# LazyLatte/vortex-raytracing

Measured on AMD Instinct MI355X. Metric: Mrays/s (primary+shadow) at 1920x1080, 1M-tri BVH, higher is better.
Workload: dtype f32; 1 GPU; configs[2]: Sponza-class 1048576 tris, 1920x1080, primary + 1 shadow ray per hit; frames_in_flight=2, frames_per_launch_group=5, parallelism=1 GPU: whole frames, 5 per set of launches (vxrt_render_batch), 2 sets in flight, world_size=1, bvh_nodes=726809, bvh_depth=13

## Files before the change

include/vortex_hip.h:

```cpp
#ifndef VORTEX_HIP_H
#define VORTEX_HIP_H

#include <stddef.h>
#include <stdint.h>

#ifdef __cplusplus
extern "C" {
#endif

typedef void* vx_device_h;
typedef void* vx_buffer_h;

typedef struct {
  int (*dev_open)(vx_device_h* hdevice);
  int (*dev_close)(vx_device_h hdevice);
  int (*dev_caps)(vx_device_h hdevice, uint32_t caps_id, uint64_t* value);
  int (*mem_alloc)(vx_device_h hdevice, uint64_t size, int flags, vx_buffer_h* hbuffer);
  int (*mem_reserve)(vx_device_h hdevice, uint64_t address, uint64_t size, int flags, vx_buffer_h* hbuffer);
  int (*mem_free)(vx_buffer_h hbuffer);
  int (*mem_access)(vx_buffer_h hbuffer, uint64_t offset, uint64_t size, int flags);
  int (*mem_address)(vx_buffer_h hbuffer, uint64_t* address);
  int (*mem_info)(vx_device_h hdevice, uint64_t* mem_free, uint64_t* mem_used);
  int (*copy_to_dev)(vx_buffer_h hbuffer, const void* host_ptr, uint64_t dst_offset, uint64_t size);
  int (*copy_from_dev)(void* host_ptr, vx_buffer_h hbuffer, uint64_t src_offset, uint64_t size);
// ... 84 lines not shown
  const void* triEx;
  const void* mat;
  const void* tex;
  uint32_t n_tlas_nodes;
  uint32_t n_blas;
  uint32_t n_bvh_nodes;
  uint32_t n_tris;
  uint32_t n_mats;
  uint32_t reserved;
  uint64_t tex_bytes;
} vxrt_scene_t;

typedef struct {
  float dist, bx, by, bz;
  uint32_t blasIdx, triIdx;
} vxrt_hit_t;

typedef struct {
  float ambient[3], light_color[3], light_pos[3], background[3];
  uint32_t max_depth;
} vxrt_shade_params_t;

#define VXRT_MODE_CLOSEST 0
#define VXRT_MODE_ANY 1

typedef struct vxrt_accel vxrt_accel_t;
int vxrt_accel_build(const vxrt_scene_t* scene, void* stream, vxrt_accel_t** out);
int vxrt_accel_destroy(vxrt_accel_t* accel);
uint64_t vxrt_accel_bytes(const vxrt_accel_t* accel);
int vxrt_accel_info(const vxrt_accel_t* accel, uint32_t which, uint64_t* value);

#define VXRT_REFIT_INSTANCES 1u
#define VXRT_REFIT_GEOMETRY 2u
int vxrt_accel_refit(vxrt_accel_t* accel, uint32_t what, void* stream);
int vxrt_accel_set_transforms(vxrt_accel_t* accel, uint32_t first, uint32_t count, const float* transforms, void* stream);

int vxrt_accel_frames_in_flight(vxrt_accel_t* accel, uint32_t n);

int vxrt_render(vxrt_accel_t* accel, uint32_t width, uint32_t height, uint32_t y0, uint32_t y1,
                const vxrt_shade_params_t* params, int shadow, uint32_t* dst,
                vxrt_hit_t* hits , float* colors ,
                unsigned long long* rays_traced, void* stream);

int vxrt_render_interleaved(vxrt_accel_t* accel, uint32_t width, uint32_t height, uint32_t phase, uint32_t stride,
                            const vxrt_shade_params_t* params, int shadow, uint32_t* dst, vxrt_hit_t* hits,
                            float* colors, unsigned long long* rays_traced, void* stream);

typedef struct vxrt_bvh_info {
  uint32_t n_nodes, n_leaves, max_leaf, max_depth;
  float bounds[6];
} vxrt_bvh_info_t;
int vxrt_bvh_build(void* tri, void* triEx, uint32_t n_tris, uint32_t tri_offset, uint32_t leaf_max,
                   void* nodes, uint32_t node_capacity, vxrt_bvh_info_t* info, void* stream);
int vxrt_tlas_build(const float* instance_boxes, uint32_t n_instances, void* nodes, uint32_t node_capacity,
                    vxrt_bvh_info_t* info, void* stream);
void vxrt_bvh_release_scratch(void);

#define VXRT_MAX_BATCH 32
int vxrt_render_interleaved_batch(vxrt_accel_t* accel, uint32_t width, uint32_t height, uint32_t phase, uint32_t stride, uint32_t n_frames,
                                  const vxrt_shade_params_t* params, int shadow, uint32_t* dst, uint64_t dst_frame_stride,
                                  unsigned long long* rays_traced, void* stream);

int vxrt_render_interleaved_batch_wave_log(vxrt_accel_t* accel, uint32_t width, uint32_t height, uint32_t phase, uint32_t stride, uint32_t n_frames,
                                           const vxrt_shade_params_t* params, int shadow, uint32_t* dst, uint64_t dst_frame_stride,
                                           unsigned long long* counters, unsigned long long* wave_log, void* stream);

int vxrt_wire_pack(const uint32_t* frames, uint64_t frame_stride, uint32_t width, uint32_t tile_rows_per_rank, uint32_t world, uint32_t rank,
                   uint32_t n_frames, uint8_t* wire, void* stream);
int vxrt_wire_unpack(const uint8_t* wire_all, uint64_t wire_stride_bytes, uint32_t width, uint32_t tile_rows_per_rank, uint32_t world,
                     uint32_t n_frames, uint32_t* frames, uint64_t frame_stride, void* stream);

int vxrt_render_rows_batch(vxrt_accel_t* accel, uint32_t width, uint32_t height, uint32_t y0, uint32_t y1, uint32_t n_frames,
                           const vxrt_shade_params_t* params, int shadow, uint32_t* dst, uint64_t dst_frame_stride,
                           unsigned long long* rays_traced, void* stream);

int vxrt_render_batch(vxrt_accel_t* accel, uint32_t width, uint32_t height, uint32_t n_frames, const vxrt_shade_params_t* params, int shadow,
                      uint32_t* dst, uint64_t dst_frame_stride, unsigned long long* rays_traced, void* stream);

typedef struct vxrt_camera {
  float pos[3], forward[3], right[3], up[3], viewplane[2];
} vxrt_camera_t;

int vxrt_render_camera(vxrt_accel_t* accel, const vxrt_camera_t* cam, uint32_t width, uint32_t height, uint32_t y0, uint32_t y1,
                       const vxrt_shade_params_t* params, int shadow, uint32_t* dst, vxrt_hit_t* hits , float* colors ,
                       unsigned long long* rays_traced, void* stream);

int vxrt_render_batch_camera(vxrt_accel_t* accel, uint32_t width, uint32_t height, uint32_t n_frames, const vxrt_camera_t* cams,
                             const vxrt_shade_params_t* params, int shadow, uint32_t* dst, uint64_t dst_frame_stride,
                             unsigned long long* rays_traced, void* stream);

int vxrt_render_stats(vxrt_accel_t* accel, uint32_t width, uint32_t height, uint32_t y0, uint32_t y1,
                      const vxrt_shade_params_t* params, int shadow, uint32_t* dst,
                      unsigned long long* counters, void* stream);

int vxrt_render_stats_timed(vxrt_accel_t* accel, uint32_t width, uint32_t height, uint32_t y0, uint32_t y1,
                            const vxrt_shade_params_t* params, int shadow, uint32_t* dst,
                            unsigned long long* counters, void* stream);

int vxrt_trace_stats(vxrt_accel_t* accel, const float* rays, uint64_t n, const float* tmax,
                     vxrt_hit_t* hits, int mode, unsigned long long* counters, void* stream);

typedef struct vxrt_ao_params {
  uint32_t spp;
  float radius;
  uint32_t seed;
  uint32_t reserved;
} vxrt_ao_params_t;
int vxrt_render_ao(vxrt_accel_t* accel, uint32_t width, uint32_t height, uint32_t y0, uint32_t y1,
                   const vxrt_shade_params_t* params, const vxrt_ao_params_t* ao, uint32_t* dst, float* colors,
                   uint32_t* unoccluded, unsigned long long* rays_traced, void* stream);

int vxrt_render_diffuse_bounce(vxrt_accel_t* accel, uint32_t width, uint32_t height, uint32_t y0, uint32_t y1,
                               const vxrt_shade_params_t* params, uint32_t seed, uint32_t* dst, float* colors,
                               unsigned long long* rays_traced, void* stream);

typedef struct vxrc_scene {
  const void* tlas; const void* blas; const void* bvh; const void* tri; const void* triEx; const void* triIdx; const void* tex;
  uint32_t n_tlas_nodes, n_blas, n_bvh_nodes, n_tris, n_tri_idx, tlas_root;
  uint64_t tex_bytes;
} vxrc_scene_t;
typedef struct vxrc_params {
  float camera_pos[3], camera_forward[3], camera_right[3], camera_up[3], viewplane[2];
  uint32_t samples_per_pixel, max_depth;
  float light_pos[3], light_color[3], ambient_color[3], background_color[3];
} vxrc_params_t;
typedef struct vxrc_accel vxrc_accel_t;
int vxrc_accel_build(const vxrc_scene_t* scene, void* stream, vxrc_accel_t** out);
int vxrc_accel_destroy(vxrc_accel_t* accel);
int vxrc_accel_info(const vxrc_accel_t* accel, uint32_t which, uint64_t* value);
int vxrc_render_accel(vxrc_accel_t* accel, uint32_t width, uint32_t height, uint32_t y0, uint32_t y1,
                      const vxrc_params_t* params, uint32_t* dst, float* colors, void* stream);

int vxrc_render(const vxrc_scene_t* scene, uint32_t width, uint32_t height, uint32_t y0, uint32_t y1,
                const vxrc_params_t* params, uint32_t* dst, float* colors, void* stream);

int vxrt_render_wave_log(vxrt_accel_t* accel, uint32_t width, uint32_t height, uint32_t y0, uint32_t y1,
                         const vxrt_shade_params_t* params, int shadow, uint32_t* dst,
                         unsigned long long* counters, unsigned long long* wave_log, void* stream);

int vxrt_trace(vxrt_accel_t* accel, const float* rays, uint64_t n, const float* tmax,
               vxrt_hit_t* hits, int mode, void* stream);

int vxrt_shade_rays(vxrt_accel_t* accel, const float* rays, const vxrt_hit_t* hits, uint64_t n, const vxrt_shade_params_t* params,
                    float* colors, uint32_t* rgb8, void* stream);

int vxrt_camera_rays(uint32_t width, uint32_t height, uint32_t y0, uint32_t y1, float* rays, void* stream);

int vxrt_pinhole_rays(const vxrt_camera_t* cam, uint32_t width, uint32_t height, uint32_t y0, uint32_t y1, float* rays, void* stream);

int vxrt_trace_reference_quirks(const void* image, uint64_t image_size, uint32_t tlas_off, uint32_t blas_off, uint32_t bvh_off, uint32_t tri_off,
                                const float* rays, uint64_t n, const float* tmax, vxrt_hit_t* hits, int mode, void* stream);

int vxrt_debug_read_control(vxrt_accel_t* accel, uint32_t ctx, uint32_t* out, uint32_t n_dwords, void* stream);
int vxrt_debug_end_log(vxrt_accel_t* accel, unsigned long long* log);
int vxrt_debug_trace_wave_log(vxrt_accel_t* accel, unsigned long long* log);
int vxrt_debug_read_lpt(vxrt_accel_t* accel, uint32_t ctx, uint32_t batch, uint32_t* cost, uint32_t cost_cap, uint32_t* order, uint32_t order_cap,
                        void* stream);

int vxrt_status(void* stream, uint32_t* status);
int vx_hip_buffer_device_ptr(vx_buffer_h hbuffer, void** dev_ptr);

int vx_hip_device_stat(vx_device_h hdevice, uint32_t which, uint64_t* value);

const char* vxrt_version(void);

#ifdef __cplusplus
}
#endif
#endif
```

vortex-raytracing_amd/csrc/rt_accel.hip:

```cpp
#include <algorithm>
#include <cmath>
#include <cstdio>
#include <cstdlib>
#include <cstring>
#include <utility>
#include "rt_internal.h"
#include "bvh_quant.h"

__global__ void accel_nodes_kernel(const uint32_t* __restrict__ ref, uint32_t n_nodes, uint4* __restrict__ out, int is_tlas,
                                   const uint32_t* __restrict__ bases, const uint32_t* __restrict__ ends, uint32_t nb,
                                   uint32_t n_tris, uint32_t n_blas, uint32_t bias, uint32_t* status) {
  const uint32_t i = blockIdx.x * blockDim.x + threadIdx.x;
  if (i >= n_nodes) return;
  const uint32_t* w = ref + (size_t)i * RT_NODE_DWORDS;
  const uint32_t imask = w[3] >> 24, leftFirst = w[4], leafData = w[5];
  uint32_t base = 0, end = n_nodes;
  if (!is_tlas) {
    bool in = false;
    for (uint32_t j = 0; j < nb; ++j) if (i >= bases[j] && i < ends[j]) { base = bases[j]; end = ends[j]; in = true; }
    if (!in) return;
  }
  if (imask != (is_tlas ? 1u : 0u)) return;
  const bool leaf = is_tlas ? (leafData != 0xffffffffu) : (leafData != 0u);
  if (leaf) return;
// ... 224 lines not shown
  bool fin = true;
  if (fbox_bvh) {
    for (int a = 0; a < 3; ++a) { olo[a] = fbox_bvh[(size_t)off * 6 + a]; ohi[a] = fbox_bvh[(size_t)off * 6 + 3 + a]; }
  } else if (r[5] != 0u) {
    fin = refit_tri_box(tri, r[4], r[5], olo, ohi);
  } else {
    const uint8_t* b = (const uint8_t*)r;
    olo[0] = olo[1] = olo[2] = __builtin_inff(); ohi[0] = ohi[1] = ohi[2] = -__builtin_inff();
    for (int k = 0; k < 4; ++k) {
      const uint8_t* c = b + 24 + 7 * k;
      if (c[0] == 0) continue;
      for (int a = 0; a < 3; ++a) {
        const int e = (int)(int8_t)b[12 + a];
        const float o = __uint_as_float(r[a]);
        olo[a] = fminf(olo[a], o + ldexpf((float)c[1 + a], e));
        ohi[a] = fmaxf(ohi[a], o + ldexpf((float)c[4 + a], e));
      }
    }
  }
  const float* m = (const float*)(rec + 17);
  for (int k = 0; k < 12; ++k) fin = fin && isfinite(m[k]);
  float lo[3] = {__builtin_inff(), __builtin_inff(), __builtin_inff()}, hi[3] = {-__builtin_inff(), -__builtin_inff(), -__builtin_inff()};
  for (int c = 0; c < 8; ++c) {
    const float x = (c & 1) ? ohi[0] : olo[0], y = (c & 2) ? ohi[1] : olo[1], z = (c & 4) ? ohi[2] : olo[2];
    for (int a = 0; a < 3; ++a) {
      const float p = refit_row(m + 4 * a, x, y, z);
      fin = fin && isfinite(p);
      lo[a] = fminf(lo[a], p); hi[a] = fmaxf(hi[a], p);
    }
  }
  if (!fin) atomicOr(res + 1, REFIT_ERR_NONFINITE);
  const int e[3] = {bb_pick_exp(hi[0] - lo[0]), bb_pick_exp(hi[1] - lo[1]), bb_pick_exp(hi[2] - lo[2])};
  refit_write_origin(w, lo, hi, e);
  refit_store_box(fbox, i, lo, hi);
}

__global__ __launch_bounds__(256) void refit_level_kernel(uint32_t* __restrict__ nodes, const uint2* __restrict__ items, uint32_t n,
                                                          float* __restrict__ fbox, uint32_t* __restrict__ res) {
  const uint32_t j = blockIdx.x * blockDim.x + threadIdx.x;
  if (j >= n) return;
  const uint2 it = items[j];
  uint32_t* w = nodes + (size_t)it.x * RT_NODE_DWORDS;
  uint32_t cw[7];
#pragma unroll
  for (int v = 0; v < 7; ++v) cw[v] = w[6 + v];
  uint8_t* cb = (uint8_t*)cw;
  uint32_t present = 0;
  float cmin[3][4], cmax[3][4];
  float lo[3] = {__builtin_inff(), __builtin_inff(), __builtin_inff()}, hi[3] = {-__builtin_inff(), -__builtin_inff(), -__builtin_inff()};
#pragma unroll
  for (int k = 0; k < 4; ++k) {
    const bool on = cb[7 * k] != 0;
    present |= on ? (1u << k) : 0u;
    const float* f = fbox + (size_t)(it.y + (on ? (uint32_t)k : 0u)) * 6;
#pragma unroll
    for (int a = 0; a < 3; ++a) {
      cmin[a][k] = on ? f[a] : 0.0f; cmax[a][k] = on ? f[3 + a] : 0.0f;
      if (on) { lo[a] = fminf(lo[a], cmin[a][k]); hi[a] = fmaxf(hi[a], cmax[a][k]); }
    }
  }
  if (!present) return;
  int e[3] = {bb_pick_exp(hi[0] - lo[0]), bb_pick_exp(hi[1] - lo[1]), bb_pick_exp(hi[2] - lo[2])};
  bool ok = true;
#pragma unroll
  for (int a = 0; a < 3; ++a) {
    uint32_t ql[4] = {0, 0, 0, 0}, qh[4] = {0, 0, 0, 0};
    ok = bb_quant_children(lo[a], e[a], cmin[a], cmax[a], present, ql, qh) && ok;
#pragma unroll
    for (int k = 0; k < 4; ++k)
      if ((present >> k) & 1u) { cb[7 * k + 1 + a] = (uint8_t)ql[k]; cb[7 * k + 4 + a] = (uint8_t)qh[k]; }
  }
  if (!ok) atomicOr(res + 1, REFIT_ERR_QUANT);
  refit_write_origin(w, lo, hi, e);
#pragma unroll
  for (int v = 0; v < 7; ++v) w[6 + v] = cw[v];
  refit_store_box(fbox, it.x, lo, hi);
}

__global__ void refit_finish_kernel(const uint32_t* __restrict__ blas, uint32_t troot, const uint32_t* __restrict__ top_roots, uint32_t* __restrict__ res) {
  if (threadIdx.x != 0 || blockIdx.x != 0) return;
  uint32_t id = 0u;
  if (is_inst_desc(troot)) {
    const float* m = (const float*)(blas + (size_t)(troot & PAYLOAD_MASK) * (RT_BLAS_STRIDE / 4) + 1);
    id = 1u;
    for (int i = 0; i < 12; ++i) id = (id && m[i] == ((i % 5 == 0) ? 1.0f : 0.0f)) ? 1u : 0u;
  }
  res[2] = id;
  if (top_roots) { res[3] = top_roots[0]; res[4] = top_roots[1]; }
}

__global__ __launch_bounds__(256) void refit_xform_kernel(const float* __restrict__ in, uint32_t n, float* __restrict__ out, uint32_t* __restrict__ res) {
#pragma clang fp contract(off)
  const uint32_t r = blockIdx.x * blockDim.x + threadIdx.x;
  if (r >= n) return;
  float c[16];
  bool fin = true;
  for (int k = 0; k < 16; ++k) { c[k] = in[(size_t)r * 16 + k]; fin = fin && isfinite(c[k]); }
  const float inv[16] = {
      c[5] * c[10] * c[15] - c[5] * c[11] * c[14] - c[9] * c[6] * c[15] + c[9] * c[7] * c[14] + c[13] * c[6] * c[11] - c[13] * c[7] * c[10],
      -c[1] * c[10] * c[15] + c[1] * c[11] * c[14] + c[9] * c[2] * c[15] - c[9] * c[3] * c[14] - c[13] * c[2] * c[11] + c[13] * c[3] * c[10],
      c[1] * c[6] * c[15] - c[1] * c[7] * c[14] - c[5] * c[2] * c[15] + c[5] * c[3] * c[14] + c[13] * c[2] * c[7] - c[13] * c[3] * c[6],
      -c[1] * c[6] * c[11] + c[1] * c[7] * c[10] + c[5] * c[2] * c[11] - c[5] * c[3] * c[10] - c[9] * c[2] * c[7] + c[9] * c[3] * c[6],
      -c[4] * c[10] * c[15] + c[4] * c[11] * c[14] + c[8] * c[6] * c[15] - c[8] * c[7] * c[14] - c[12] * c[6] * c[11] + c[12] * c[7] * c[10],
      c[0] * c[10] * c[15] - c[0] * c[11] * c[14] - c[8] * c[2] * c[15] + c[8] * c[3] * c[14] + c[12] * c[2] * c[11] - c[12] * c[3] * c[10],
      -c[0] * c[6] * c[15] + c[0] * c[7] * c[14] + c[4] * c[2] * c[15] - c[4] * c[3] * c[14] - c[12] * c[2] * c[7] + c[12] * c[3] * c[6],
      c[0] * c[6] * c[11] - c[0] * c[7] * c[10] - c[4] * c[2] * c[11] + c[4] * c[3] * c[10] + c[8] * c[2] * c[7] - c[8] * c[3] * c[6],
      c[4] * c[9] * c[15] - c[4] * c[11] * c[13] - c[8] * c[5] * c[15] + c[8] * c[7] * c[13] + c[12] * c[5] * c[11] - c[12] * c[7] * c[9],
      -c[0] * c[9] * c[15] + c[0] * c[11] * c[13] + c[8] * c[1] * c[15] - c[8] * c[3] * c[13] - c[12] * c[1] * c[11] + c[12] * c[3] * c[9],
      c[0] * c[5] * c[15] - c[0] * c[7] * c[13] - c[4] * c[1] * c[15] + c[4] * c[3] * c[13] + c[12] * c[1] * c[7] - c[12] * c[3] * c[5],
      -c[0] * c[5] * c[11] + c[0] * c[7] * c[9] + c[4] * c[1] * c[11] - c[4] * c[3] * c[9] - c[8] * c[1] * c[7] + c[8] * c[3] * c[5],
      -c[4] * c[9] * c[14] + c[4] * c[10] * c[13] + c[8] * c[5] * c[14] - c[8] * c[6] * c[13] - c[12] * c[5] * c[10] + c[12] * c[6] * c[9],
      c[0] * c[9] * c[14] - c[0] * c[10] * c[13] - c[8] * c[1] * c[14] + c[8] * c[2] * c[13] + c[12] * c[1] * c[10] - c[12] * c[2] * c[9],
      -c[0] * c[5] * c[14] + c[0] * c[6] * c[13] + c[4] * c[1] * c[14] - c[4] * c[2] * c[13] - c[12] * c[1] * c[6] + c[12] * c[2] * c[5],
      c[0] * c[5] * c[10] - c[0] * c[6] * c[9] - c[4] * c[1] * c[10] + c[4] * c[2] * c[9] + c[8] * c[1] * c[6] - c[8] * c[2] * c[5]};
  const float det = c[0] * inv[0] + c[1] * inv[4] + c[2] * inv[8] + c[3] * inv[12];
  uint32_t err = fin ? 0u : REFIT_ERR_NONFINITE;
  if (det == 0.0f) err |= REFIT_ERR_SINGULAR;
  const float invdet = 1.0f / det;
  float* o = out + (size_t)r * 32;
  for (int k = 0; k < 16; ++k) {
    const float v = inv[k] * invdet;
    if (!isfinite(v)) err |= REFIT_ERR_SINGULAR;
    o[k] = v;
    o[16 + k] = c[k];
  }
  if (err) atomicOr(res + 6, err);
}

__global__ __launch_bounds__(256) void refit_xform_commit_kernel(const float* __restrict__ xf, uint32_t first, uint32_t n, uint32_t* __restrict__ blas,
                                                                 const uint32_t* __restrict__ res) {
  const uint32_t t = blockIdx.x * blockDim.x + threadIdx.x;
  if (t >= n * 32u || res[6] != 0u) return;
  const uint32_t r = t / 32u, k = t % 32u;
  blas[(size_t)(first + r) * (RT_BLAS_STRIDE / 4) + 1 + k] = __float_as_uint(xf[(size_t)r * 32 + k]);
}

struct RefitPlan {
  uint32_t* blas_leaves = nullptr; uint32_t n_blas_leaves = 0;
  uint2* blas_items = nullptr; std::vector<uint32_t> blas_lv;
  uint32_t* tlas_leaves = nullptr; uint32_t n_tlas_leaves = 0;
  uint2* tlas_items = nullptr; std::vector<uint32_t> tlas_lv;
  float* fbox_bvh = nullptr; float* fbox_tlas = nullptr;
  uint32_t* ranges = nullptr; uint32_t nb = 0;
  uint32_t* res = nullptr;
  float* xf = nullptr; uint32_t xf_cap = 0;
};
static void refit_plan_free(RefitPlan* p) {
  if (!p) return;
  (void)hipFree(p->blas_leaves); (void)hipFree(p->blas_items); (void)hipFree(p->tlas_leaves); (void)hipFree(p->tlas_items);
  (void)hipFree(p->fbox_bvh); (void)hipFree(p->fbox_tlas); (void)hipFree(p->ranges); (void)hipFree(p->res); (void)hipFree(p->xf);
  delete p;
}

static void accel_free(vxrt_accel* a) {
  if (!a) return;
  (void)hipDeviceSynchronize();
  (void)hipFree(a->nodes_c); (void)hipFree(a->tri_w); (void)hipFree(a->blas_root);
  (void)hipFree(a->top_img); (void)hipFree(a->top_roots);
  refit_plan_free(a->refit);
  (void)hipFree(a->uvtab); (void)hipFree(a->apriori);
  for (uint32_t k = 0; k <= VXRT_MAX_BATCH; ++k) (void)hipFree(a->batch_order[k]);
  for (FrameCtx& c : a->ctx) {
    (void)hipFree(c.hitbuf); (void)hipFree(c.defer); (void)hipFree(c.ctl); (void)hipFree(c.bcount);
    for (FrameCtx::Lpt& l : c.lpt) { (void)hipFree(l.cost); (void)hipFree(l.order); }
    (void)hipFree(c.ao_geo); (void)hipFree(c.ao_nrm); (void)hipFree(c.ao_col); (void)hipFree(c.ao_cnt); (void)hipFree(c.ao_rays); (void)hipFree(c.ao_tmax); (void)hipFree(c.ao_hits); (void)hipFree(c.ao_list); (void)hipFree(c.ao_hdr);
    (void)hipFree(c.bin_hist); (void)hipFree(c.bin_keys); (void)hipFree(c.bin_order);
    for (FrameCtx::Level& l : c.lv) {
      (void)hipFree(l.rays); (void)hipFree(l.hits); (void)hipFree(l.parent); (void)hipFree(l.term); (void)hipFree(l.col);
      (void)hipFree(l.srays); (void)hipFree(l.stmax); (void)hipFree(l.shits);
    }
    (void)hipFree(c.pbatch); (void)hipFree(c.pool_spill); (void)hipFree(c.cam);
    if (c.side) (void)hipStreamDestroy(c.side);
    if (c.ev_in) (void)hipEventDestroy(c.ev_in);
    if (c.ev_side) (void)hipEventDestroy(c.ev_side);
    if (c.ev_done) (void)hipEventDestroy(c.ev_done);
  }
  delete a;
}

extern "C" {

int vxrt_accel_build(const vxrt_scene_t* s, void* stream, vxrt_accel_t** out) {
  if (!s || !out || !s->tlas || !s->blas || !s->bvh || !s->tri) return -1;
  if (s->n_tlas_nodes == 0 || s->n_blas == 0 || s->n_bvh_nodes == 0 || s->n_tris == 0) return -1;
  if ((uint64_t)s->n_tlas_nodes + s->n_bvh_nodes > PAYLOAD_MASK || s->n_tris >= 0x7fffffffu) return -1;
  hipStream_t st = (hipStream_t)stream;
  std::vector<uint32_t> recs((size_t)s->n_blas * (RT_BLAS_STRIDE / 4));
  if (hipStreamSynchronize(st) != hipSuccess) return -1;
  if (hipMemcpy(recs.data(), s->blas, recs.size() * 4, hipMemcpyDeviceToHost) != hipSuccess) return -1;
  std::vector<uint32_t> bases;
  float max_refl = 0.0f;
  for (uint32_t j = 0; j < s->n_blas; ++j) {
    const uint32_t off = recs[(size_t)j * (RT_BLAS_STRIDE / 4)];
    if (off >= s->n_bvh_nodes) return -1;
    bases.push_back(off);
    float refl;
    memcpy(&refl, &recs[(size_t)j * (RT_BLAS_STRIDE / 4) + 38], sizeof(float));
    if (refl > max_refl) max_refl = refl;
  }
  std::sort(bases.begin(), bases.end());
  bases.erase(std::unique(bases.begin(), bases.end()), bases.end());
  std::vector<uint32_t> ends(bases.size());
  for (size_t j = 0; j < bases.size(); ++j) ends[j] = j + 1 < bases.size() ? bases[j + 1] : s->n_bvh_nodes;

  auto a = new (std::nothrow) vxrt_accel();
  if (!a) return -1;
  a->ref = *s;
  a->max_reflectivity = max_refl;
  (void)hipGetDevice(&a->device);
  uint32_t* d_ranges = nullptr;
  uint32_t* d_status = nullptr;
  uint32_t* d_troot = nullptr;
  constexpr uint32_t TOP_CAP = RT_TOP_NODES;
  const bool stage_top = TOP_CAP > 0 && (uint64_t)s->n_tlas_nodes + s->n_bvh_nodes < DESC_TOP_FLAG;
  bool ok = hipMalloc(&a->nodes_c, ((size_t)s->n_tlas_nodes + s->n_bvh_nodes) * CNODE_VEC4 * 16) == hipSuccess &&
            (!stage_top || (hipMalloc(&a->top_img, (size_t)TOP_CAP * CNODE_VEC4 * 16) == hipSuccess &&
                            hipMalloc((void**)&a->top_roots, ((size_t)s->n_blas + 2) * sizeof(uint32_t)) == hipSuccess)) &&
            hipMalloc(&a->tri_w, (size_t)s->n_tris * WTRI_FLOATS * 4) == hipSuccess &&
            hipMalloc(&a->blas_root, (size_t)s->n_blas * sizeof(uint32_t)) == hipSuccess &&
            hipMalloc((void**)&d_ranges, bases.size() * 8) == hipSuccess &&
            hipMalloc((void**)&d_status, 8) == hipSuccess && hipMalloc((void**)&d_troot, 4) == hipSuccess;
  uint32_t hstatus = 0, troot = DESC_DONE, hstatus2[2] = {0, 0};
  if (ok) {
    ok = hipMemcpy(d_ranges, bases.data(), bases.size() * 4, hipMemcpyHostToDevice) == hipSuccess &&
         hipMemcpy(d_ranges + bases.size(), ends.data(), ends.size() * 4, hipMemcpyHostToDevice) == hipSuccess &&
         hipMemset(d_status, 0, 8) == hipSuccess;
  }
  if (ok) {
    const uint32_t nb = (uint32_t)bases.size();
    hipLaunchKernelGGL(accel_nodes_kernel, dim3((s->n_tlas_nodes + 255) / 256), dim3(256), 0, st, (const uint32_t*)s->tlas, s->n_tlas_nodes,
                       (uint4*)a->nodes_c, 1, (const uint32_t*)nullptr, (const uint32_t*)nullptr, 0u, s->n_tris, s->n_blas, 0u, d_status);
    hipLaunchKernelGGL(accel_nodes_kernel, dim3((s->n_bvh_nodes + 255) / 256), dim3(256), 0, st, (const uint32_t*)s->bvh, s->n_bvh_nodes,
                       (uint4*)a->nodes_c + (size_t)s->n_tlas_nodes * CNODE_VEC4, 0, d_ranges, d_ranges + nb, nb, s->n_tris, s->n_blas, s->n_tlas_nodes, d_status + 1);
    hipLaunchKernelGGL(accel_tris_kernel, dim3((s->n_tris + 255) / 256), dim3(256), 0, st, (const float*)s->tri, s->n_tris, (float4*)a->tri_w);
    hipLaunchKernelGGL(accel_roots_kernel, dim3((s->n_blas + 1 + 255) / 256), dim3(256), 0, st, (const uint32_t*)s->tlas, (const uint32_t*)s->bvh,
                       (const uint32_t*)s->blas, s->n_tlas_nodes, s->n_bvh_nodes, s->n_blas, s->n_tris, d_troot, (uint32_t*)a->blas_root, d_status);
    if (s->triEx && s->mat && s->n_mats) {
      const uint32_t nchk = std::max(s->n_tris, s->n_mats);
      hipLaunchKernelGGL(accel_check_shading_kernel, dim3((nchk + 255) / 256), dim3(256), 0, st, (const rt_triex_t*)s->triEx, s->n_tris,
                         (const rt_material_t*)s->mat, s->n_mats, (uint64_t)s->tex_bytes, s->tex ? 1 : 0, d_status);
    }
    ok = hipGetLastError() == hipSuccess && hipStreamSynchronize(st) == hipSuccess &&
         hipMemcpy(hstatus2, d_status, 8, hipMemcpyDeviceToHost) == hipSuccess &&
         hipMemcpy(&troot, d_troot, 4, hipMemcpyDeviceToHost) == hipSuccess;
    hstatus = hstatus2[0] | hstatus2[1];
    a->blas_status = hstatus2[1] & STATUS_FMA_DECODE_DIFFERS;
  }
  uint32_t n_top = 0, troot_top = troot;
  if (ok && stage_top && (hstatus & (STATUS_BAD_SCENE | STATUS_FMA_DECODE_DIFFERS)) == 0) {
    ok = hipMemsetAsync(a->top_img, 0, (size_t)TOP_CAP * CNODE_VEC4 * 16, st) == hipSuccess;
    hipLaunchKernelGGL(accel_top_kernel, dim3(1), dim3(64), 0, st, (const uint4*)a->nodes_c, troot, (const uint32_t*)a->blas_root, s->n_blas, TOP_CAP,
                       (uint4*)a->top_img, a->top_roots, a->top_roots + 1, a->top_roots + 2);
    uint32_t hdr[2] = {0, DESC_DONE};
    ok = ok && hipGetLastError() == hipSuccess && hipStreamSynchronize(st) == hipSuccess &&
         hipMemcpy(hdr, a->top_roots, sizeof hdr, hipMemcpyDeviceToHost) == hipSuccess;
    n_top = hdr[0]; troot_top = hdr[1];
  }
  uint32_t levels = 0;
  if (ok && (hstatus & STATUS_BAD_SCENE) == 0) {
    const uint32_t nc = s->n_tlas_nodes + s->n_bvh_nodes;
    uint32_t* d_depth = nullptr;
    ok = hipMalloc((void**)&d_depth, ((size_t)nc + 1) * 4) == hipSuccess && hipMemsetAsync(d_depth, 0, ((size_t)nc + 1) * 4, st) == hipSuccess;
    if (ok) {
      for (uint32_t level = 1; level <= RT_SHALLOW_LEVELS + 1u; ++level)
        hipLaunchKernelGGL(accel_depth_kernel, dim3(level == 1u ? 1u : (nc + 255) / 256), dim3(256), 0, st, (const uint4*)a->nodes_c, nc, troot,
                           (const uint32_t*)a->blas_root, level, d_depth, d_depth + nc);
      ok = hipGetLastError() == hipSuccess && hipStreamSynchronize(st) == hipSuccess &&
           hipMemcpy(&levels, d_depth + nc, 4, hipMemcpyDeviceToHost) == hipSuccess;
    }
    (void)hipFree(d_depth);
  }
  (void)hipFree(d_ranges); (void)hipFree(d_status); (void)hipFree(d_troot);
  if (!ok || (hstatus & STATUS_BAD_SCENE) != 0) { accel_free(a); return -1; }
  static const int shallow_env = [] { const char* e = getenv("VXRT_SHALLOW"); return e ? atoi(e) : -1; }();
  a->levels = levels;
  a->shallow = levels <= RT_SHALLOW_LEVELS && shallow_env != 0;
  a->dev.nodes_c = (const uint4*)a->nodes_c; a->dev.ref_tlas = (const uint32_t*)s->tlas; a->dev.n_tlas = s->n_tlas_nodes; a->dev.tri_w = (const float4*)a->tri_w;
  a->dev.blas_root = (const uint32_t*)a->blas_root; a->dev.tlas_root = troot;
  a->dev.ident_root = 0u;
  if (troot >= 0xC0000000u && troot < DESC_IDLE) {
    float m[12];
    static const bool ident_off = [] { const char* e = getenv("VXRT_IDENT_ROOT"); return e && e[0] == '0'; }();
    if (!ident_off && hipMemcpy(m, (const uint32_t*)s->blas + (size_t)(troot & PAYLOAD_MASK) * (RT_BLAS_STRIDE / 4) + 1, sizeof m, hipMemcpyDeviceToHost) == hipSuccess) {
      bool id = true;
      for (int i = 0; i < 12; ++i) id = id && m[i] == ((i % 5 == 0) ? 1.0f : 0.0f);
      a->dev.ident_root = id ? 1u : 0u;
    }
  }
  a->dev.exact_decode = (hstatus & STATUS_FMA_DECODE_DIFFERS) ? 1u : 0u;
  a->dev.ref_bvh = (const uint32_t*)s->bvh;
  a->dev.blas = (const uint32_t*)s->blas; a->dev.triEx = (const rt_triex_t*)s->triEx;
  a->dev.mat = (const rt_material_t*)s->mat; a->dev.tex = (const uint8_t*)s->tex;
  a->dev.top_img = (const uint4*)a->top_img; a->dev.n_top = n_top; a->dev.tlas_root_top = troot_top;
  a->dev.blas_root_top = n_top ? a->top_roots + 2 : (const uint32_t*)a->blas_root;
  if (getenv("VXRT_DEBUG")) fprintf(stderr, "[vxrt] accel: %u top-of-tree nodes staged for LDS (cap %u)\n", n_top, TOP_CAP);
  *out = a;
  return 0;
}

int vxrt_accel_destroy(vxrt_accel_t* a) {
  if (!a) return 0;
  accel_free(a);
  return 0;
}

uint64_t vxrt_accel_bytes(const vxrt_accel_t* a) {
  if (!a) return 0;
  return (uint64_t)a->ref.n_tlas_nodes * CNODE_VEC4 * 16 + (uint64_t)a->ref.n_bvh_nodes * CNODE_VEC4 * 16 +
         (uint64_t)a->ref.n_tris * WTRI_FLOATS * 4 + (uint64_t)a->ref.n_blas * 4;
}

int vxrt_accel_info(const vxrt_accel_t* a, uint32_t which, uint64_t* value) {
  if (!a || !value) return -1;
  switch (which) {
  case 0: *value = a->levels; return 0;
  case 1: *value = a->shallow ? 1u : 0u; return 0;
  case 2: *value = a->dev.ident_root; return 0;
  case 3: *value = a->dev.exact_decode; return 0;
  }
  return -1;
}

int vxrt_accel_frames_in_flight(vxrt_accel_t* a, uint32_t n) {
  if (!a || n < 1 || n > MAX_FRAMES_IN_FLIGHT) return -1;
  if (hipDeviceSynchronize() != hipSuccess) return -1;
  a->n_ctx = n; a->next_ctx = 0;
  return 0;
}

static int refit_fail(const char* where) {
  const hipError_t e = hipGetLastError();
  if (getenv("VXRT_DEBUG")) fprintf(stderr, "[vxrt] refit failed: %s (%s)\n", where, hipGetErrorString(e));
  return -1;
}

static RefitPlan* refit_plan_build(vxrt_accel* a, hipStream_t st) {
  const vxrt_scene_t& s = a->ref;
  std::vector<uint32_t> tl((size_t)s.n_tlas_nodes * RT_NODE_DWORDS), bv((size_t)s.n_bvh_nodes * RT_NODE_DWORDS), recs((size_t)s.n_blas * (RT_BLAS_STRIDE / 4));
  if (hipStreamSynchronize(st) != hipSuccess ||
      hipMemcpy(tl.data(), s.tlas, tl.size() * 4, hipMemcpyDeviceToHost) != hipSuccess ||
      hipMemcpy(bv.data(), s.bvh, bv.size() * 4, hipMemcpyDeviceToHost) != hipSuccess ||
      hipMemcpy(recs.data(), s.blas, recs.size() * 4, hipMemcpyDeviceToHost) != hipSuccess) { refit_fail("plan: node copy"); return nullptr; }
  std::vector<uint32_t> bases;
  for (uint32_t j = 0; j < s.n_blas; ++j) bases.push_back(recs[(size_t)j * (RT_BLAS_STRIDE / 4)]);
  std::sort(bases.begin(), bases.end());
  bases.erase(std::unique(bases.begin(), bases.end()), bases.end());
  std::vector<uint32_t> ends(bases.size());
  for (size_t j = 0; j < bases.size(); ++j) ends[j] = j + 1 < bases.size() ? bases[j + 1] : s.n_bvh_nodes;
  auto walk = [](const std::vector<uint32_t>& w, uint32_t root, uint32_t base, uint32_t end, bool tlas, std::vector<uint32_t>& leaves,
                 std::vector<std::pair<uint32_t, uint2>>& items) -> bool {
    std::vector<std::pair<uint32_t, uint32_t>> q{{root, 0u}};
    for (size_t h = 0; h < q.size(); ++h) {
      const uint32_t i = q[h].first, L = q[h].second;
      const uint32_t* n = w.data() + (size_t)i * RT_NODE_DWORDS;
      if (tlas ? n[5] != 0xffffffffu : n[5] != 0u) { leaves.push_back(i); continue; }
      const uint64_t c0 = (uint64_t)base + n[4];
      items.push_back({L, make_uint2(i, (uint32_t)c0)});
      const uint8_t* b = (const uint8_t*)n;
      bool any = false;
      for (uint32_t k = 0; k < 4; ++k) {
        if (b[24 + 7 * k] == 0) continue;
        if (c0 + k >= end || c0 + k <= i) return false;
        q.push_back({(uint32_t)(c0 + k), L + 1u});
        any = true;
      }
      if (!any) return false;
    }
    return true;
  };
  std::vector<uint32_t> bl, tlv;
  std::vector<std::pair<uint32_t, uint2>> bi, ti;
  for (size_t j = 0; j < bases.size(); ++j)
    if (!walk(bv, bases[j], bases[j], ends[j], false, bl, bi)) { refit_fail("plan: BLAS walk"); return nullptr; }
  if (!walk(tl, 0u, 0u, s.n_tlas_nodes, true, tlv, ti)) { refit_fail("plan: TLAS walk"); return nullptr; }
  for (uint32_t i : tlv) if (tl[(size_t)i * RT_NODE_DWORDS + 5] >= s.n_blas) { refit_fail("plan: instance index"); return nullptr; }
  auto bucket = [](const std::vector<std::pair<uint32_t, uint2>>& it, std::vector<uint2>& out, std::vector<uint32_t>& lv) {
    uint32_t depth = 0;
    for (const auto& x : it) depth = std::max(depth, x.first + 1u);
    lv.assign(depth + 1u, 0u);
    for (const auto& x : it) ++lv[x.first + 1u];
    for (uint32_t L = 0; L < depth; ++L) lv[L + 1u] += lv[L];
    std::vector<uint32_t> pos(lv.begin(), lv.end() - 1);
    out.resize(it.size());
    for (const auto& x : it) out[pos[x.first]++] = x.second;
  };
  std::vector<uint32_t> ranges(bases);
  ranges.insert(ranges.end(), ends.begin(), ends.end());
  std::vector<uint2> bitems, titems;
  auto p = new (std::nothrow) RefitPlan();
  if (!p) return nullptr;
  bucket(bi, bitems, p->blas_lv);
  bucket(ti, titems, p->tlas_lv);
  p->n_blas_leaves = (uint32_t)bl.size(); p->n_tlas_leaves = (uint32_t)tlv.size(); p->nb = (uint32_t)bases.size();
  auto up = [](void** d, const void* h, size_t bytes) {
    return hipMalloc(d, std::max<size_t>(bytes, 16)) == hipSuccess && (bytes == 0 || hipMemcpy(*d, h, bytes, hipMemcpyHostToDevice) == hipSuccess);
  };
  const bool ok = up((void**)&p->blas_leaves, bl.data(), bl.size() * 4) && up((void**)&p->blas_items, bitems.data(), bitems.size() * 8) &&
                  up((void**)&p->tlas_leaves, tlv.data(), tlv.size() * 4) && up((void**)&p->tlas_items, titems.data(), titems.size() * 8) &&
                  up((void**)&p->ranges, ranges.data(), ranges.size() * 4) &&
                  hipMalloc((void**)&p->fbox_bvh, (size_t)s.n_bvh_nodes * 24) == hipSuccess &&
                  hipMalloc((void**)&p->fbox_tlas, (size_t)s.n_tlas_nodes * 24) == hipSuccess &&
                  hipMalloc((void**)&p->res, REFIT_RES_WORDS * 4) == hipSuccess;
  if (!ok) { refit_fail("plan: upload"); refit_plan_free(p); return nullptr; }
  return p;
}

static int refit_run(vxrt_accel* a, uint32_t what, hipStream_t st, const float* xf_in, uint32_t xf_first, uint32_t xf_count) {
  RefitPlan* p = a->refit;
  const vxrt_scene_t& s = a->ref;
  for (uint32_t k = 0; k < MAX_FRAMES_IN_FLIGHT; ++k) {
    FrameCtx& c = a->ctx[k];
    if (!c.busy || c.last_stream == st) continue;
    if (c.done_recorded) { if (hipStreamWaitEvent(st, c.ev_done, 0) != hipSuccess) return refit_fail("ordering"); }
    else if (hipDeviceSynchronize() != hipSuccess) return refit_fail("ordering");
  }
  const bool geom = (what & VXRT_REFIT_GEOMETRY) != 0u;
  auto grid = [](uint64_t n) { return dim3((uint32_t)((n + 255) / 256)); };
  bool ok = hipMemsetAsync(p->res, 0, REFIT_RES_WORDS * 4, st) == hipSuccess;
  if (ok && xf_count) {
    hipLaunchKernelGGL(refit_xform_kernel, grid(xf_count), dim3(256), 0, st, xf_in, xf_count, p->xf, p->res);
    hipLaunchKernelGGL(refit_xform_commit_kernel, grid((uint64_t)xf_count * 32u), dim3(256), 0, st, (const float*)p->xf, xf_first, xf_count,
                       (uint32_t*)s.blas, (const uint32_t*)p->res);
  }
  if (ok && geom) {
    if (p->n_blas_leaves)
      hipLaunchKernelGGL(refit_blas_leaf_kernel, grid(p->n_blas_leaves), dim3(256), 0, st, (uint32_t*)s.bvh, (const float*)s.tri, p->blas_leaves,
                         p->n_blas_leaves, p->fbox_bvh, p->res);
    for (size_t L = p->blas_lv.size() - 1; L-- > 0;) {
      const uint32_t n = p->blas_lv[L + 1] - p->blas_lv[L];
      if (n) hipLaunchKernelGGL(refit_level_kernel, grid(n), dim3(256), 0, st, (uint32_t*)s.bvh, p->blas_items + p->blas_lv[L], n, p->fbox_bvh, p->res);
    }
  }
  if (ok) {
    if (p->n_tlas_leaves)
      hipLaunchKernelGGL(refit_instance_kernel, grid(p->n_tlas_leaves), dim3(256), 0, st, (uint32_t*)s.tlas, p->tlas_leaves, p->n_tlas_leaves,
                         (const uint32_t*)s.blas, (const uint32_t*)s.bvh, (const float*)s.tri, geom ? (const float*)p->fbox_bvh : (const float*)nullptr,
                         p->fbox_tlas, p->res);
    for (size_t L = p->tlas_lv.size() - 1; L-- > 0;) {
      const uint32_t n = p->tlas_lv[L + 1] - p->tlas_lv[L];
      if (n) hipLaunchKernelGGL(refit_level_kernel, grid(n), dim3(256), 0, st, (uint32_t*)s.tlas, p->tlas_items + p->tlas_lv[L], n, p->fbox_tlas, p->res);
    }
    hipLaunchKernelGGL(accel_nodes_kernel, grid(s.n_tlas_nodes), dim3(256), 0, st, (const uint32_t*)s.tlas, s.n_tlas_nodes,
                       (uint4*)a->nodes_c, 1, (const uint32_t*)nullptr, (const uint32_t*)nullptr, 0u, s.n_tris, s.n_blas, 0u, p->res);
    if (geom) {
      hipLaunchKernelGGL(accel_nodes_kernel, grid(s.n_bvh_nodes), dim3(256), 0, st, (const uint32_t*)s.bvh, s.n_bvh_nodes,
                         (uint4*)a->nodes_c + (size_t)s.n_tlas_nodes * CNODE_VEC4, 0, p->ranges, p->ranges + p->nb, p->nb, s.n_tris, s.n_blas, s.n_tlas_nodes,
                         p->res + 5);
      hipLaunchKernelGGL(accel_tris_kernel, grid(s.n_tris), dim3(256), 0, st, (const float*)s.tri, s.n_tris, (float4*)a->tri_w);
    }
    if (a->top_img) {
      ok = hipMemsetAsync(a->top_img, 0, (size_t)RT_TOP_NODES * CNODE_VEC4 * 16, st) == hipSuccess;
      hipLaunchKernelGGL(accel_top_kernel, dim3(1), dim3(64), 0, st, (const uint4*)a->nodes_c, a->dev.tlas_root, (const uint32_t*)a->blas_root, s.n_blas,
                         (uint32_t)RT_TOP_NODES, (uint4*)a->top_img, a->top_roots, a->top_roots + 1, a->top_roots + 2);
    }
    hipLaunchKernelGGL(refit_finish_kernel, dim3(1), dim3(64), 0, st, (const uint32_t*)s.blas, a->dev.tlas_root, (const uint32_t*)a->top_roots, p->res);
  }
  uint32_t res[REFIT_RES_WORDS] = {0};
  ok = ok && hipGetLastError() == hipSuccess && hipStreamSynchronize(st) == hipSuccess &&
       hipMemcpy(res, p->res, sizeof res, hipMemcpyDeviceToHost) == hipSuccess;
  if (!ok || res[1] != 0u || ((res[0] | res[5]) & STATUS_BAD_SCENE) != 0u) {
    a->stale = true;
    if (getenv("VXRT_DEBUG")) fprintf(stderr, "[vxrt] refit: ok %d, errors %u, status %u / %u\n", (int)ok, res[1], res[0], res[5]);
    return refit_fail("boxes");
  }
  if (geom) a->blas_status = res[5] & STATUS_FMA_DECODE_DIFFERS;
  const uint32_t st_all = (res[0] & STATUS_FMA_DECODE_DIFFERS) | a->blas_status;
  a->dev.exact_decode = st_all ? 1u : 0u;
  static const bool ident_off = [] { const char* e = getenv("VXRT_IDENT_ROOT"); return e && e[0] == '0'; }();
  a->dev.ident_root = ident_off ? 0u : res[2];
  if (a->top_img && !st_all) {
    a->dev.n_top = res[3]; a->dev.tlas_root_top = res[4]; a->dev.blas_root_top = a->top_roots + 2;
  } else {
    a->dev.n_top = 0; a->dev.tlas_root_top = a->dev.tlas_root; a->dev.blas_root_top = (const uint32_t*)a->blas_root;
// ... 35 lines not shown
```

vortex-raytracing_amd/csrc/rt_internal.h:

```cpp
#pragma once
#include <hip/hip_runtime.h>
#include <stdint.h>
#include <vector>
#include "rt_types.h"
#include "../../include/vortex_hip.h"

#define STATUS_STACK_OVERFLOW 1u
#define STATUS_ITER_LIMIT 2u
#define STATUS_BAD_SCENE 4u
#define STATUS_FMA_DECODE_DIFFERS 8u

struct SceneDev {
  const uint4* nodes_c;
  const uint32_t* ref_tlas;
  uint32_t n_tlas;
  const float4* tri_w;
  const uint32_t* blas_root;
  uint32_t tlas_root;
  uint32_t exact_decode;
  const uint32_t* ref_bvh;
  const uint32_t* blas;
  const rt_triex_t* triEx;
  const rt_material_t* mat;
  const uint8_t* tex;
  const uint4* top_img;
  uint32_t n_top;
  uint32_t tlas_root_top;
  const uint32_t* blas_root_top;
  uint32_t ident_root;
};

struct HitRec { float dist, bx, by, bz; uint32_t blasIdx, triIdx; };

struct ShadeParams { float amb[3], lcol[3], lpos[3], bg[3]; uint32_t max_depth; };

#define MAX_FRAMES_IN_FLIGHT 8
struct FrameCtx {
  void* hitbuf = nullptr;
  uint64_t hitbuf_pixels = 0;
  uint32_t* defer = nullptr;
  uint64_t defer_cap = 0;
  uint32_t* ctl = nullptr;
  ShadeParams* pbatch = nullptr;
  float* cam = nullptr; uint64_t cam_floats = 0;
  bool ctl_dirty = false;
  struct Level {
    float* rays = nullptr; HitRec* hits = nullptr; uint32_t* parent = nullptr; float4* term = nullptr; float* col = nullptr;
    float* srays = nullptr; float* stmax = nullptr; HitRec* shits = nullptr;
    uint64_t cap = 0; uint32_t n = 0;
  };
  std::vector<Level> lv;
  uint32_t* bcount = nullptr;
  struct Lpt { uint32_t* cost = nullptr; uint32_t* order = nullptr; uint32_t cap = 0; uint32_t key[6] = {0, 0, 0, 0, 0, 0}; bool valid = false; };
  Lpt lpt[VXRT_MAX_BATCH + 1];
  float4* ao_geo = nullptr; float4* ao_nrm = nullptr; float4* ao_col = nullptr; uint32_t* ao_cnt = nullptr;
  uint32_t* ao_list = nullptr; uint32_t* ao_hdr = nullptr;
  float* ao_rays = nullptr; float* ao_tmax = nullptr; HitRec* ao_hits = nullptr; uint64_t ao_cap = 0, ao_ray_cap = 0;
  uint32_t* bin_hist = nullptr; uint32_t* bin_keys = nullptr; uint32_t* bin_order = nullptr; uint64_t bin_cap = 0, bin_ray_cap = 0;
  void* pool_spill = nullptr; uint64_t pool_spill_bytes = 0;
  hipStream_t side = nullptr;
  hipEvent_t ev_in = nullptr, ev_side = nullptr, ev_done = nullptr;
  bool busy = false, inited = false, done_recorded = false;
  hipStream_t last_stream = nullptr;
};

struct vxrt_accel {
  SceneDev dev{};
  vxrt_scene_t ref{};
  void* nodes_c = nullptr; void* tri_w = nullptr; void* blas_root = nullptr;
  void* top_img = nullptr; uint32_t* top_roots = nullptr;
  FrameCtx ctx[MAX_FRAMES_IN_FLIGHT];
  uint32_t n_ctx = 1, next_ctx = 0;
  bool stream_seen = false, multi_stream = false; hipStream_t first_stream = nullptr;
  float* uvtab = nullptr;
  uint32_t uv_w = 0, uv_h = 0;
  uint32_t* apriori = nullptr;
  uint32_t* batch_order[VXRT_MAX_BATCH + 1] = {}; uint32_t bo_tiles = 0;
  uint32_t ap_count = 0, ap_key[6] = {0, 0, 0, 0, 0, 0};
  uint64_t ap_cap = 0;
  float max_reflectivity = 0.0f;
  unsigned long long* trace_wave_log = nullptr;
  unsigned long long* end_log = nullptr;
  uint32_t levels = 0;
  bool shallow = false;
  int device = 0;
  struct RefitPlan* refit = nullptr;
  uint32_t blas_status = 0;
  bool stale = false;
};
```

vortex-raytracing_amd/csrc/rt_kernels.hip:

```cpp
#include <hip/hip_runtime.h>
#include <stdint.h>
#include "rt_internal.h"
#include "pinhole.h"

__device__ __forceinline__ float std_min(float a, float b) { return (b < a) ? b : a; }
__device__ __forceinline__ float std_max(float a, float b) { return (a < b) ? b : a; }

template <bool EXACT>
__device__ __forceinline__ float slab_interval(float tx1, float tx2, float ty1, float ty2, float tz1, float tz2) {
  float tmin, tmax;
  if (EXACT) {
    tmin = std_min(tx1, tx2);
    tmax = std_max(tx1, tx2);
    tmin = std_max(tmin, std_min(ty1, ty2));
    tmax = std_min(tmax, std_max(ty1, ty2));
    tmin = std_max(tmin, std_min(tz1, tz2));
    tmax = std_min(tmax, std_max(tz1, tz2));
  } else {
    tmin = fmaxf(fmaxf(fminf(tx1, tx2), fminf(ty1, ty2)), fminf(tz1, tz2));
    tmax = fminf(fminf(fmaxf(tx1, tx2), fmaxf(ty1, ty2)), fmaxf(tz1, tz2));
  }
  return (tmax < tmin || tmax <= 0) ? RT_LARGE_FLOAT : tmin;
}

// ... 253 lines not shown
__device__ __forceinline__ float random_float(uint32_t& s) {
  s ^= s << 13; s ^= s >> 17; s ^= s << 5;
  return (float)s * 2.3283064365387e-10f;
}

__device__ __forceinline__ void ao_sample_ray(uint32_t x, uint32_t y, uint32_t W, uint32_t spp, uint32_t smp, uint32_t user_seed,
                                              float Ix, float Iy, float Iz, float nx, float ny, float nz, float vdx, float vdy, float vdz, float* o6) {
  uint32_t seed = wang_hash((x + y * W) * spp + smp + 1u + user_seed * 0x9E3779B9u);
  if (seed == 0u) seed = 1u;
  float u = 0.0f, v = 0.0f, r2 = 0.0f;
  bool ok = false;
  for (int k = 0; k < 8 && !ok; ++k) {
    const float a = 2.0f * random_float(seed) - 1.0f;
    const float b = 2.0f * random_float(seed) - 1.0f;
    const float q = a * a + b * b;
    if (q < 1.0f) { u = a; v = b; r2 = q; ok = true; }
  }
  const float z = sqrtf(1.0f - r2);
  if (nx * vdx + ny * vdy + nz * vdz > 0.0f) { nx = -nx; ny = -ny; nz = -nz; }
  const float sign = nz >= 0.0f ? 1.0f : -1.0f;
  const float a = -1.0f / (sign + nz);
  const float b = nx * ny * a;
  const float tx = 1.0f + sign * nx * nx * a, ty = sign * b, tz = -sign * nx;
  const float bx = b, by = sign + ny * ny * a, bz = -ny;
  o6[0] = Ix + nx * 0.001f; o6[1] = Iy + ny * 0.001f; o6[2] = Iz + nz * 0.001f;
  o6[3] = tx * u + bx * v + nx * z;
  o6[4] = ty * u + by * v + ny * z;
  o6[5] = tz * u + bz * v + nz * z;
}

#ifndef RT_TRI_PREFETCH
#define RT_TRI_PREFETCH 1
#endif
#ifndef RT_WAVES_PER_EU
#define RT_WAVES_PER_EU 6
#endif

#ifndef RT_DEAD_MAX
#define RT_DEAD_MAX 64
#endif
#ifndef RT_LEAF_MIN
#define RT_LEAF_MIN 1
#endif
#ifndef RT_TRACE_LEAF_MIN
#define RT_TRACE_LEAF_MIN 24
#endif
#ifndef RT_TRI_LDS
#define RT_TRI_LDS 0
#endif
#ifndef RT_TRI_LDS_MIN
#define RT_TRI_LDS_MIN 8
#endif
#ifndef RT_UNORDERED_OCCLUSION
#define RT_UNORDERED_OCCLUSION 1
#endif
#ifndef RT_SHADOW_FINISH_MIN
#define RT_SHADOW_FINISH_MIN 65
#endif
#ifndef RT_TRACE_DEAD_MAX
#define RT_TRACE_DEAD_MAX 16
#endif
#ifndef RT_CHUNK
#define RT_CHUNK 64
#endif
#ifndef RT_TRACE_NT
#define RT_TRACE_NT 0
#endif
#ifndef RT_TRACE_CHUNK
#define RT_TRACE_CHUNK 64
#endif
#ifndef RT_XCC_HOME
#define RT_XCC_HOME 1
#endif
#ifndef RT_QUEUE_DRY_MASK
#define RT_QUEUE_DRY_MASK 1
#endif
#ifndef RT_STEAL_SPREAD
#define RT_STEAL_SPREAD 0
#endif
#ifndef QUEUE_SHARDS
#define QUEUE_SHARDS 8u
#endif
#define QUEUE_STRIDE 32u
#define CTL_QUEUE_DWORDS (QUEUE_SHARDS * QUEUE_STRIDE)
#define CTL_DWORDS (32u + 3u * CTL_QUEUE_DWORDS)
#ifndef RT_WAVES_TRACE
#define RT_WAVES_TRACE 7
#endif
#ifndef RT_LDS_STACK_TRACE
#define RT_LDS_STACK_TRACE 7
#endif
#ifndef RT_WAVES_RENDER
#define RT_WAVES_RENDER 7
#endif
#ifndef RT_LDS_STACK_RENDER
#define RT_LDS_STACK_RENDER 6
#endif
#ifndef RT_WAVES_RENDER_PACKED
#define RT_WAVES_RENDER_PACKED 8
#endif
#ifndef RT_LDS_STACK_RENDER_PACKED
#define RT_LDS_STACK_RENDER_PACKED 5
#endif
#ifndef LDS_STACK
#define LDS_STACK 8
#endif
#ifndef RT_WG_WAVES
#define RT_WG_WAVES 4
#endif
#define RT_WG_THREADS (64 * RT_WG_WAVES)

enum { JOB_RENDER = 0, JOB_RENDER_SHADOW = 1, JOB_TRACE = 2, JOB_RENDER_GI = 3, JOB_TRACE_UNORDERED = 4 };
__host__ __device__ constexpr bool is_trace_job(int job) { return job == JOB_TRACE || job == JOB_TRACE_UNORDERED; }
enum { JOB_CAM = 8 };
__host__ __device__ constexpr int job_base(int job) { return job & ~JOB_CAM; }
__host__ __device__ constexpr bool is_cam_job(int job) { return (job & JOB_CAM) != 0; }
#ifndef RT_WAVES_GI
#define RT_WAVES_GI 7
#endif
#ifndef RT_LDS_STACK_GI
#define RT_LDS_STACK_GI 6
#endif
#ifndef RT_GI_DEAD_MAX
#define RT_GI_DEAD_MAX 64
#endif

#ifdef RT_ISA_MARKS
#define RT_MARK(name) asm volatile("; RTMARK " name)
#else
#define RT_MARK(name)
#endif

__device__ __forceinline__ size_t hit_index(uint32_t x, uint32_t lr, uint32_t tiles_x) {
  return ((size_t)(lr >> 3) * tiles_x + (x >> 3)) * 64u + ((lr & 7u) << 3) + (x & 7u);
}
__device__ __forceinline__ uint32_t frame_row(uint32_t lr, uint32_t y0, uint32_t row_step) { return y0 + (lr >> 3) * row_step + (lr & 7u); }

struct FastDiv { uint32_t d, m, s; };
static FastDiv fast_div_make(uint32_t d) {
  FastDiv f{d ? d : 1u, 1u, 0u};
  while ((1ull << f.s) < f.d) ++f.s;
  f.m = (uint32_t)((((1ull << f.s) - f.d) << 32) / f.d) + 1u;
  return f;
}
__device__ __forceinline__ uint32_t fast_div(uint32_t x, const FastDiv& f) { return (__umulhi(x, f.m) + x) >> f.s; }

struct PersistArgs {
  uint32_t W, H, y0, y1, tiles_x;
  FastDiv div_tiles_x, div_frame_tiles;
  uint32_t row_step;
  uint32_t total;
  const uint32_t* total_dev;
  HitRec* hits;
  const float* rays; const float* tmax; int any_hit;
  const uint32_t* order;
  unsigned long long* counters;
  uint32_t* status;
  uint32_t* queue;
  uint32_t per_shard;
  const float* utab; const float* vtab;
  uint32_t* defer_count; uint32_t* defer_list; uint32_t defer_cap;
  const uint32_t* tile_order; uint32_t* tile_cost;
  uint32_t shard_rot;
  unsigned long long* wave_log;
  unsigned long long* end_log;
  const ShadeParams* pbatch; uint32_t frame_tiles;
  uint32_t* dst; float* colors; uint32_t gi_seed;
};

#define RT_FAST_INV_MAX 0x1p+64f
#define RT_FAST_POS_MAX 0x1p+60f
__device__ __forceinline__ bool ray_in_fast_domain(float ox, float oy, float oz, float ix, float iy, float iz) {
  return fabsf(ix) <= RT_FAST_INV_MAX && fabsf(iy) <= RT_FAST_INV_MAX && fabsf(iz) <= RT_FAST_INV_MAX && ix != 0.0f && iy != 0.0f && iz != 0.0f &&
         fabsf(ox) <= RT_FAST_POS_MAX && fabsf(oy) <= RT_FAST_POS_MAX && fabsf(oz) <= RT_FAST_POS_MAX;
}

__device__ __forceinline__ float vmax_nonan(float a, float b) { float r; asm("v_max_f32 %0, %1, %2" : "=v"(r) : "v"(a), "v"(b)); return r; }

#define F_FOUND 1u
#define F_ANYHIT 2u
#define F_SHADOW 8u
#define F_WORLD 16u
#define F_RESUMED 32u

template <int JOB, int STATS, bool LDEXP, bool EXACT, bool PACKED = false, bool SHALLOW = false>
__global__ __launch_bounds__(EXACT ? 256 : RT_WG_THREADS, EXACT ? 4 : (is_trace_job(JOB) ? RT_WAVES_TRACE : (JOB == JOB_RENDER_GI ? RT_WAVES_GI : (PACKED ? RT_WAVES_RENDER_PACKED : RT_WAVES_RENDER)))) void rt_persistent_kernel(SceneDev sc, ShadeParams p, PersistArgs A) {
  constexpr int LSTK = EXACT ? LDS_STACK : (is_trace_job(JOB) ? RT_LDS_STACK_TRACE : (JOB == JOB_RENDER_GI ? RT_LDS_STACK_GI : (PACKED ? RT_LDS_STACK_RENDER_PACKED : RT_LDS_STACK_RENDER)));
  constexpr int WG_WAVES = EXACT ? 4 : RT_WG_WAVES;
  constexpr bool USE_TOP = RT_TOP_NODES > 0 && !EXACT && !LDEXP;
  constexpr uint32_t DEAD_MAX = is_trace_job(JOB) ? RT_TRACE_DEAD_MAX : (JOB == JOB_RENDER_GI ? RT_GI_DEAD_MAX : RT_DEAD_MAX);
  constexpr uint32_t FINISH_MIN = job_base(JOB) == JOB_RENDER_SHADOW ? RT_SHADOW_FINISH_MIN : 65u;
  const uint32_t lane = threadIdx.x & 63u;
  const uint32_t n_jobs = EXACT ? min(*A.defer_count, A.defer_cap) : (A.total_dev ? min(*A.total_dev, A.total) : A.total);
  const uint32_t per_shard = (EXACT || A.total_dev) ? (((n_jobs + QUEUE_SHARDS - 1) / QUEUE_SHARDS + 63u) & ~63u) : A.per_shard;

  __shared__ uint2 s_stk[WG_WAVES][LSTK][64];
  constexpr int NCTX = (!EXACT && is_trace_job(JOB)) ? 8 : 9;
  __shared__ uint32_t s_ctx[WG_WAVES][NCTX][64];
  __shared__ uint32_t s_dry;
  if (threadIdx.x == 0) s_dry = 0u;
  float* s_cam = nullptr;
  if constexpr (is_cam_job(JOB)) {
    s_cam = cam_lds<CAM_TAB>();
    for (uint32_t i = threadIdx.x; i < (uint32_t)CAM_TAB; i += blockDim.x) s_cam[i] = A.utab[i];
  }
  __syncthreads();
  uint2* const lstk = &s_stk[threadIdx.x >> 6][0][lane];
  uint32_t* const ctx = &s_ctx[threadIdx.x >> 6][0][lane];
#define CTX(i) ctx[((NCTX == 8 && (i) > 5) ? (i) - 1 : (i)) * 64]
  __shared__ uint4 s_top[USE_TOP ? 4 : 1][USE_TOP ? RT_TOP_NODES : 1];
  constexpr bool TRI_LDS = RT_TRI_LDS > 0 && !EXACT && !is_trace_job(JOB);
  __shared__ float4 s_tri[TRI_LDS ? WG_WAVES : 1][TRI_LDS ? 3 * RT_TRI_LDS : 1];
  const uint32_t n_top = USE_TOP ? min(sc.n_top, (uint32_t)RT_TOP_NODES) : 0u;
  if (USE_TOP && n_top) {
    for (uint32_t i = threadIdx.x; i < 4u * n_top; i += (uint32_t)(64 * WG_WAVES)) s_top[i / n_top][i % n_top] = sc.top_img[(size_t)(i / n_top) * RT_TOP_NODES + (i % n_top)];
    __syncthreads();
  }
  const uint32_t root_desc = (USE_TOP && n_top) ? sc.tlas_root_top : sc.tlas_root;
  const uint32_t* const blas_roots = (USE_TOP && n_top) ? sc.blas_root_top : sc.blas_root;
  const uint32_t root_blas_desc = is_inst_desc(root_desc) ? blas_roots[root_desc & PAYLOAD_MASK] : DESC_DONE;

  float arx = 0, ary = 0, arz = 0, aix = 0, aiy = 0, aiz = 0;
  float hitd = 0, path_m = 0, tos_m = 0;
  uint32_t cur = DESC_IDLE, tos_d = DESC_DONE, job = 0, flags = 0;
  float g_col[3] = {0.f, 0.f, 0.f}, g_alb[3] = {0.f, 0.f, 0.f}, g_ray[6] = {0.f, 0.f, 0.f, 0.f, 0.f, 0.f};
  int sp = 0;
  constexpr int STACK_CAP = SHALLOW ? 3 * RT_SHALLOW_LEVELS : LSTK + RT_STACK_ENTRIES;
  static_assert(STACK_CAP > LSTK, "stack");
  uint32_t ovf_d[STACK_CAP - LSTK];
  float ovf_m[STACK_CAP - LSTK];
  bool queue_empty = false;
  const uint32_t xcc_id = RT_XCC_HOME ? (uint32_t)__builtin_amdgcn_s_getreg((3 << 11) | (0 << 6) | 20) : blockIdx.x;
  const uint32_t shard = (xcc_id + A.shard_rot) % QUEUE_SHARDS;
  uint32_t tries = 0, loc_next = 0, loc_end = 0;
  uint32_t loc_off = 0;
  uint32_t lpt_tile = 0xFFFFFFFFu, lpt_work = 0; unsigned long long lpt_t0 = 0;
  Fetches fx;
  unsigned nrays = 0, nhit = 0;
  unsigned long long t_first = 0;
  unsigned long long wl_tn = 0, wl_tl = 0, wl_t0 = 0;
  unsigned wl_no23 = 0, wl_no3 = 0, wl_iter = 0, wl_node_x = 0, wl_node_l = 0, wl_leaf_x = 0, wl_leaf_l = 0;
  unsigned long long wl_tstart = 0, wl_tf = 0, wl_tfin = 0, wl_tmark = 0;
  unsigned long long wl_tq = 0;
  if (STATS && A.wave_log) { t_first = wall_clock64(); wl_tstart = __builtin_readcyclecounter(); }

  auto pixel_of = [&](uint32_t r, uint32_t& x, uint32_t& y) {
    asm volatile("" : "+v"(r));
    uint32_t tile = r >> 6;
    const uint32_t l = r & 63u;
    if (A.pbatch) tile -= fast_div(tile, A.div_frame_tiles) * A.frame_tiles;
    const uint32_t ty = fast_div(tile, A.div_tiles_x);
    x = (tile - ty * A.tiles_x) * 8u + (l & 7u);
    y = A.y0 + ty * A.row_step + (l >> 3);
  };
  auto hit_slot = [&]() -> HitRec* {
    uint32_t j = job;
    asm volatile("" : "+v"(j));
    return A.hits + j;
  };
  auto pixel_ray = [&](uint32_t x, uint32_t y, float& ox, float& oy, float& oz, float& dx, float& dy, float& dz) {
    if constexpr (is_cam_job(JOB)) {
      const uint32_t f = A.pbatch ? fast_div(job >> 6, A.div_frame_tiles) : 0u;
      camera_ray(s_cam + f * CAM_HDR, A.vtab + (size_t)f * (A.W + A.H), A.W, x, y, ox, oy, oz, dx, dy, dz);
    } else generate_ray(A.utab[x], A.vtab[y], ox, oy, oz, dx, dy, dz);
  };
  auto world_ray = [&](float& ox, float& oy, float& oz, float& dx, float& dy, float& dz, float& tmax_) {
    tmax_ = RT_LARGE_FLOAT;
    if (is_trace_job(JOB)) {
      const float* rp = A.rays + (size_t)job * 6;
      if (RT_TRACE_NT) {
        ox = __builtin_nontemporal_load(rp); oy = __builtin_nontemporal_load(rp + 1); oz = __builtin_nontemporal_load(rp + 2);
        dx = __builtin_nontemporal_load(rp + 3); dy = __builtin_nontemporal_load(rp + 4); dz = __builtin_nontemporal_load(rp + 5);
      } else { ox = rp[0]; oy = rp[1]; oz = rp[2]; dx = rp[3]; dy = rp[4]; dz = rp[5]; }
      if (A.tmax) tmax_ = A.tmax[job];
    } else {
      uint32_t x, y;
      pixel_of(job, x, y);
      pixel_ray(x, y, ox, oy, oz, dx, dy, dz);
      if (JOB == JOB_RENDER_GI && (flags & F_SHADOW)) {
        ox = g_ray[0]; oy = g_ray[1]; oz = g_ray[2]; dx = g_ray[3]; dy = g_ray[4]; dz = g_ray[5];
      }
      if (job_base(JOB) == JOB_RENDER_SHADOW && (flags & F_SHADOW)) {
        const float pd = __uint_as_float(CTX(5));
        float sox, soy, soz, sdx, sdy, sdz, sdist;
        float lpx = p.lpos[0], lpy = p.lpos[1], lpz = p.lpos[2];
        if (A.pbatch) { const ShadeParams* q = A.pbatch + fast_div(job >> 6, A.div_frame_tiles); lpx = q->lpos[0]; lpy = q->lpos[1]; lpz = q->lpos[2]; }
        shadow_ray(lpx, lpy, lpz, ox, oy, oz, dx, dy, dz, pd, sox, soy, soz, sdx, sdy, sdz, sdist);
        ox = sox; oy = soy; oz = soz; dx = sdx; dy = sdy; dz = sdz;
        tmax_ = sdist;
      }
    }
  };
  auto defer = [&](bool counted) {
    const uint32_t slot = atomicAdd(A.defer_count, 1u);
    if (JOB == JOB_RENDER_GI && (flags & F_SHADOW)) nrays--;
    if (slot < A.defer_cap) A.defer_list[slot] = job | ((flags & F_SHADOW) && JOB != JOB_RENDER_GI ? 0x80000000u : 0u);
    if (job_base(JOB) == JOB_RENDER_SHADOW && (flags & F_SHADOW)) {
      HitRec h;
      h.bx = __uint_as_float(CTX(3)); h.by = __uint_as_float(CTX(4)); h.bz = 1 - h.bx - h.by;
      h.dist = __uint_as_float(CTX(5)); h.blasIdx = CTX(6); h.triIdx = CTX(7);
      *hit_slot() = h;
    }
    if (counted) nrays--;
    cur = DESC_IDLE;
  };
  auto enter_instance = [&](uint32_t blasIdx, float ox, float oy, float oz, float dx, float dy, float dz) {
    const uint32_t* bp = sc.blas + (size_t)blasIdx * (RT_BLAS_STRIDE / 4);
    uint32_t bw[13];
#pragma unroll
    for (int i = 0; i < 13; ++i) bw[i] = bp[i];
    if (STATS) { fx.node++; fx.inst++; }
    const float m00 = __uint_as_float(bw[1]), m01 = __uint_as_float(bw[2]), m02 = __uint_as_float(bw[3]), m03 = __uint_as_float(bw[4]);
    const float m10 = __uint_as_float(bw[5]), m11 = __uint_as_float(bw[6]), m12 = __uint_as_float(bw[7]), m13 = __uint_as_float(bw[8]);
    const float m20 = __uint_as_float(bw[9]), m21 = __uint_as_float(bw[10]), m22 = __uint_as_float(bw[11]), m23 = __uint_as_float(bw[12]);
    arx = m00 * ox + m01 * oy + m02 * oz + m03;
    ary = m10 * ox + m11 * oy + m12 * oz + m13;
    arz = m20 * ox + m21 * oy + m22 * oz + m23;
    const float cdx = m00 * dx + m01 * dy + m02 * dz;
    const float cdy = m10 * dx + m11 * dy + m12 * dz;
    const float cdz = m20 * dx + m21 * dy + m22 * dz;
    aix = 1.0f / cdx; aiy = 1.0f / cdy; aiz = 1.0f / cdz;
    const bool s2 = ray_in_fast_domain(arx, ary, arz, aix, aiy, aiz);
    if (!EXACT && !s2) { defer(true); return; }
    flags &= ~F_WORLD;
    CTX(0) = __float_as_uint(cdx); CTX(1) = __float_as_uint(cdy); CTX(2) = __float_as_uint(cdz);
    CTX(8) = blasIdx;
    cur = blas_roots[blasIdx];
  };
  auto start_ray = [&](float ox, float oy, float oz, float dx, float dy, float dz, float tmax_, bool any_) {
    arx = ox; ary = oy; arz = oz;
    aix = 1.0f / dx; aiy = 1.0f / dy; aiz = 1.0f / dz;
    const bool safe = ray_in_fast_domain(ox, oy, oz, aix, aiy, aiz);
    flags = (flags & (F_SHADOW | F_RESUMED)) | F_WORLD | (any_ ? F_ANYHIT : 0u);
    if (!EXACT && !safe) {
      if (!is_trace_job(JOB) && !is_cam_job(JOB) && !(flags & F_SHADOW)) cur = DESC_IDLE; else defer(false);
      return;
    }
    hitd = tmax_ > RT_LARGE_FLOAT ? RT_LARGE_FLOAT : tmax_;
    path_m = -__builtin_inff(); sp = 0; tos_d = DESC_DONE;
    cur = root_desc;
    nrays++;
    if (is_inst_desc(root_desc)) {
      const bool no_neg_zero = __float_as_uint(ox) != 0x80000000u && __float_as_uint(oy) != 0x80000000u && __float_as_uint(oz) != 0x80000000u;
      if (sc.ident_root && safe && no_neg_zero) {
        if (STATS) { fx.node++; fx.inst++; }
        flags &= ~F_WORLD;
        CTX(0) = __float_as_uint(dx); CTX(1) = __float_as_uint(dy); CTX(2) = __float_as_uint(dz);
        CTX(8) = root_desc & PAYLOAD_MASK;
        cur = root_blas_desc;
      } else enter_instance(root_desc & PAYLOAD_MASK, ox, oy, oz, dx, dy, dz);
    }
  };
  volatile uint32_t* const vovf_d = ovf_d;
  volatile float* const vovf_m = ovf_m;
  auto push = [&](uint32_t d, float m) {
    if (tos_d != DESC_DONE) {
      if (sp < LSTK) lstk[sp * 64] = make_uint2(tos_d, __float_as_uint(tos_m));
      else { ovf_d[sp - LSTK] = tos_d; ovf_m[sp - LSTK] = tos_m; }
      ++sp;
    }
    tos_d = d; tos_m = m;
  };
  auto pop_next = [&]() {
    cur = DESC_DONE;
    while (tos_d != DESC_DONE) {
      const uint32_t d = tos_d;
      const float m = tos_m;
      if (sp > 0) {
        --sp;
        if (sp < LSTK) { const uint2 e = lstk[sp * 64]; tos_d = e.x; tos_m = __uint_as_float(e.y); }
        else { tos_d = ovf_d[sp - LSTK]; tos_m = ovf_m[sp - LSTK]; }
      } else {
        tos_d = DESC_DONE;
      }
      if (m < hitd) { cur = d; path_m = m; break; }
    }
  };

  for (;;) {
    RT_MARK("fetch");
    if (STATS && A.wave_log) wl_tmark = __builtin_readcyclecounter();
    {
      const unsigned long long idle = __ballot(cur == DESC_IDLE);
      if (!queue_empty && idle != 0ull && (is_trace_job(JOB) || FINISH_MIN > 64u || idle == ~0ull || RT_DEAD_MAX < 64)) {
        const uint32_t wl_tries0 = tries; const unsigned long long wl_tpoll0 = (STATS && A.wave_log) ? __builtin_readcyclecounter() : 0ull;
        if (loc_next == loc_end) {
          uint32_t dry = RT_QUEUE_DRY_MASK ? *(volatile uint32_t*)&s_dry : 0u;
          while (tries < QUEUE_SHARDS) {
            const uint32_t step = RT_STEAL_SPREAD ? (((tries & 1u) << 2) | (tries & 2u) | ((tries >> 2) & 1u)) : tries;
            const uint32_t sid = (shard + step) % QUEUE_SHARDS;
            if (RT_QUEUE_DRY_MASK && ((dry >> sid) & 1u)) { ++tries; continue; }
            const uint32_t s_lo = sid * per_shard;
            uint32_t in_range;
            asm volatile("s_cmp_lt_u32 %1, %2\n\ts_cselect_b32 %0, 1, 0 ; RTGUARD shard_range" : "=s"(in_range)
                         : "s"(__builtin_amdgcn_readfirstlane(s_lo)), "s"(__builtin_amdgcn_readfirstlane(n_jobs)) : "scc");
            if (!in_range) { ++tries; continue; }
            const uint32_t s_n = min(per_shard, n_jobs - s_lo);
            uint32_t base = 0;
            constexpr uint32_t CHUNK = (is_trace_job(JOB) && !EXACT) ? (uint32_t)RT_TRACE_CHUNK : (uint32_t)RT_CHUNK;
            if (lane == 0) base = atomicAdd(A.queue + sid * QUEUE_STRIDE, CHUNK);
            base = __shfl(base, 0);
            if (base < s_n) {
              loc_next = s_lo + base; loc_end = s_lo + min(base + CHUNK, s_n);
              break;
            }
            if (RT_QUEUE_DRY_MASK) {
              if (lane == 0) atomicOr(&s_dry, 1u << sid);
              dry |= 1u << sid;
            }
            ++tries;
          }
          if (tries >= QUEUE_SHARDS) { queue_empty = true; if (STATS && A.wave_log && !wl_tq) wl_tq = wall_clock64(); }
          if (STATS && A.wave_log && !USE_TOP && tries != wl_tries0 && lane == 0) wl_no23 += (unsigned)(__builtin_readcyclecounter() - wl_tpoll0);
        }
        uint32_t avail = loc_end - loc_next;
        if (!is_trace_job(JOB) && !EXACT) {
          avail = min(avail, 64u - (loc_next & 63u));
          if (avail != 0u && (A.tile_order || A.tile_cost)) {
            const uint32_t pos = loc_next >> 6;
            const uint32_t tile = A.tile_order ? A.tile_order[pos] : pos;
            loc_off = __builtin_amdgcn_readfirstlane((tile << 6) - (loc_next & ~63u));
            if (A.tile_cost && tile != lpt_tile) {
              if (lane == 0 && lpt_tile != 0xFFFFFFFFu) A.tile_cost[lpt_tile] = lpt_work;
              if (STATS && A.wave_log) {
                const unsigned long long now = wall_clock64();
                if (lane == 0) {
                  if (lpt_tile != 0xFFFFFFFFu) A.tile_cost[2u * (A.total >> 6) + lpt_tile] = (uint32_t)min(now - lpt_t0, 0xFFFFFFFFull);
                  A.tile_cost[(A.total >> 6) + tile] = (uint32_t)now;
                  A.tile_cost[3u * (A.total >> 6) + tile] = tries;
                }
                lpt_t0 = now;
              }
              lpt_tile = tile; lpt_work = 0;
            }
          }
        }
        if (avail != 0u && cur == DESC_IDLE) {
          const uint32_t rank = (uint32_t)__popcll(idle & ((1ull << lane) - 1ull));
          if (rank < avail) {
            job = loc_next + rank + loc_off;
            flags = 0;
            if (!EXACT && is_trace_job(JOB) && A.order) job = A.order[job];
            if (EXACT) {
              const uint32_t wd = A.defer_list[job];
              job = wd & 0x7fffffffu;
              if (wd >> 31) { flags = F_SHADOW | F_RESUMED; if (job_base(JOB) == JOB_RENDER_SHADOW) CTX(5) = __float_as_uint(hit_slot()->dist); }
            }
            float ox, oy, oz, dx, dy, dz, tm;
            if (is_trace_job(JOB)) {
              world_ray(ox, oy, oz, dx, dy, dz, tm);
              start_ray(ox, oy, oz, dx, dy, dz, tm, A.any_hit != 0);
            } else {
              uint32_t x, y;
              pixel_of(job, x, y);
              if (x < A.W && y < A.y1) {
                world_ray(ox, oy, oz, dx, dy, dz, tm);
                start_ray(ox, oy, oz, dx, dy, dz, tm, (flags & F_SHADOW) != 0u);
              }
            }
          }
        }
        loc_next += min(avail, (uint32_t)__popcll(idle));
      }
      if (__ballot(cur != DESC_IDLE) == 0ull) {
        if (queue_empty && loc_next == loc_end) {
          if (!is_trace_job(JOB) && !EXACT && A.tile_cost && lane == 0 && lpt_tile != 0xFFFFFFFFu) {
            A.tile_cost[lpt_tile] = lpt_work;
            if (STATS && A.wave_log) A.tile_cost[2u * (A.total >> 6) + lpt_tile] = (uint32_t)min(wall_clock64() - lpt_t0, 0xFFFFFFFFull);
          }
          break;
        }
        if (STATS && A.wave_log) wl_tf += __builtin_readcyclecounter() - wl_tmark;
        continue;
      }
    }
    if (STATS && A.wave_log) wl_tf += __builtin_readcyclecounter() - wl_tmark;

    for (;;) {
      RT_MARK("loop_top");
      if (!is_trace_job(JOB) && !EXACT) ++lpt_work;
      if (STATS && A.wave_log) {
        const unsigned long long nm = __ballot(is_node_desc(cur));
        ++wl_iter;
        if (nm) {
          ++wl_node_x; wl_node_l += (unsigned)__popcll(nm);
          const uint32_t c0 = __shfl(cur, __ffsll((long long)nm) - 1);
          if (__ballot(is_node_desc(cur) && cur == c0) == nm) ++wl_no3;
        }
      }
      if (STATS && A.wave_log) wl_t0 = __builtin_readcyclecounter();
      RT_MARK("node");
      if (is_node_desc(cur)) {
        const bool top = (cur >> 30) == DK_TLAS;
        if (top && !(flags & F_WORLD)) {
          float ox, oy, oz, dx, dy, dz, tm;
          world_ray(ox, oy, oz, dx, dy, dz, tm);
          arx = ox; ary = oy; arz = oz; aix = 1.0f / dx; aiy = 1.0f / dy; aiz = 1.0f / dz;
          flags |= F_WORLD;
        }
        const uint32_t ni = cur & PAYLOAD_MASK;
        uint4 q0, q1, q2, q3;
        if (USE_TOP && (cur & DESC_TOP_FLAG)) {
          typedef uint32_t u32x4_t __attribute__((ext_vector_type(4)));
          typedef __attribute__((address_space(3))) const volatile u32x4_t lds_u32x4_t;
          lds_u32x4_t* tp = (lds_u32x4_t*)&s_top[0][0] + (cur & DESC_TOP_SLOT);
          const u32x4_t t0 = tp[0], t1 = tp[RT_TOP_NODES], t2 = tp[2 * RT_TOP_NODES], t3 = tp[3 * RT_TOP_NODES];
          q0 = make_uint4(t0.x, t0.y, t0.z, t0.w); q1 = make_uint4(t1.x, t1.y, t1.z, t1.w);
          q2 = make_uint4(t2.x, t2.y, t2.z, t2.w); q3 = make_uint4(t3.x, t3.y, t3.z, t3.w);
          if (STATS && A.wave_log) ++wl_no23;
        } else {
          const uint4* np = sc.nodes_c + (size_t)ni * CNODE_VEC4;
          q0 = np[0]; q1 = np[1]; q2 = np[2]; q3 = np[3];
        }
        const uint32_t* ref_node = nullptr;
        if (LDEXP) ref_node = top ? sc.ref_tlas + (size_t)ni * RT_NODE_DWORDS : sc.ref_bvh + (size_t)(ni - sc.n_tlas) * RT_NODE_DWORDS;
        if (STATS) fx.node++;
        Cand c[4];
        eval_children<EXACT, LDEXP>(q0, q1, q2, q3, ref_node, arx, ary, arz, aix, aiy, aiz, hitd, c);
        if (((job_base(JOB) == JOB_RENDER_SHADOW && RT_UNORDERED_OCCLUSION) || JOB == JOB_TRACE_UNORDERED) && STATS != 1 && __all((flags & F_ANYHIT) != 0u)) {
          const bool v0 = c[0].d < __builtin_inff(), v1 = c[1].d < __builtin_inff(), v2 = c[2].d < __builtin_inff(), v3 = c[3].d < __builtin_inff();
          if (v0 || v1 || v2 || v3) {
            bool more = true;
            if (sp + 4 > STACK_CAP) { atomicOr(A.status, STATUS_STACK_OVERFLOW); more = false; }
            cur = v0 ? c[0].desc : (v1 ? c[1].desc : (v2 ? c[2].desc : c[3].desc));
            if (more) {
              if (v1 && v0) push(c[1].desc, c[1].d);
              if (v2 && (v0 || v1)) push(c[2].desc, c[2].d);
              if (v3 && (v0 || v1 || v2)) push(c[3].desc, c[3].d);
            }
          } else {
            pop_next();
          }
        } else {
          order_children(c);
          if (c[0].d < __builtin_inff()) {
            bool more = true;
            if (sp + 4 > STACK_CAP) { atomicOr(A.status, STATUS_STACK_OVERFLOW); more = false; }
            if (more && c[3].d < __builtin_inff()) push(c[3].desc, vmax_nonan(path_m, c[3].d));
            if (more && c[2].d < __builtin_inff()) push(c[2].desc, vmax_nonan(path_m, c[2].d));
            if (more && c[1].d < __builtin_inff()) push(c[1].desc, vmax_nonan(path_m, c[1].d));
            cur = c[0].desc;
            path_m = vmax_nonan(path_m, c[0].d);
          } else {
            pop_next();
          }
        }
      }
      if (STATS && A.wave_log) { const unsigned long long t1 = __builtin_readcyclecounter(); wl_tn += t1 - wl_t0; wl_t0 = t1; }
      RT_MARK("inst");
      if (__any(is_inst_desc(cur))) {
        if (is_inst_desc(cur)) {
          float ox, oy, oz, dx, dy, dz, tm;
          world_ray(ox, oy, oz, dx, dy, dz, tm);
          enter_instance(cur & PAYLOAD_MASK, ox, oy, oz, dx, dy, dz);
        }
      }
      RT_MARK("leaf");
      const unsigned long long leafm = __ballot(is_leaf_desc(cur));
      if (leafm != 0ull && ((uint32_t)__popcll(leafm) >= (is_trace_job(JOB) ? RT_TRACE_LEAF_MIN : RT_LEAF_MIN) || __ballot(is_node_desc(cur) || is_inst_desc(cur)) == 0ull)) {
        if (STATS && A.wave_log) { ++wl_leaf_x; wl_leaf_l += (unsigned)__popcll(leafm); }
        if (!is_trace_job(JOB) && !EXACT) lpt_work += 2u;
        {
          bool tri_from_lds = false;
          if (TRI_LDS) {
            const uint32_t L0 = __shfl(cur, __ffsll((long long)leafm) - 1);
            const uint32_t c0 = (L0 >> LEAF_FIRST_BITS) & LEAF_MAX_INLINE;
            const unsigned long long same = __ballot(cur == L0);
            if (c0 != 0u && c0 <= (uint32_t)RT_TRI_LDS && (uint32_t)__popcll(same) >= (uint32_t)RT_TRI_LDS_MIN) {
              if (lane < 3u * c0) s_tri[threadIdx.x >> 6][lane] = sc.tri_w[(size_t)(L0 & LEAF_FIRST_MASK) * 3 + lane];
              tri_from_lds = cur == L0;
              if (STATS && A.wave_log) wl_no23 += (unsigned)__popcll(same);
            }
          }
          if (is_leaf_desc(cur)) {
            if (STATS) fx.node++;
            uint32_t leftFirst = cur & LEAF_FIRST_MASK, triCount = (cur >> LEAF_FIRST_BITS) & LEAF_MAX_INLINE;
            if (triCount == 0u) {
              const uint32_t* rn = sc.ref_bvh + (size_t)leftFirst * RT_NODE_DWORDS;
              leftFirst = rn[4]; triCount = rn[5];
            }
            const float cdx = __uint_as_float(CTX(0)), cdy = __uint_as_float(CTX(1)), cdz = __uint_as_float(CTX(2));
            bool stop = false;
            constexpr bool PREFETCH = is_trace_job(JOB) && RT_TRI_PREFETCH;
            float4 n0 = make_float4(0.f, 0.f, 0.f, 0.f), n1 = n0, n2 = n0;
            if (PREFETCH) { const float4* tp0 = sc.tri_w + (size_t)leftFirst * 3; n0 = tp0[0]; n1 = tp0[1]; n2 = tp0[2]; }
            for (uint32_t i = 0; i < triCount; ++i) {
              const uint32_t triIdx = leftFirst + i;
              float4 t0, t1, t2;
              if (TRI_LDS && tri_from_lds) {
                typedef float f32x4_t __attribute__((ext_vector_type(4)));
                typedef __attribute__((address_space(3))) const volatile f32x4_t lds_f32x4_t;
                lds_f32x4_t* lp = (lds_f32x4_t*)&s_tri[threadIdx.x >> 6][0] + 3u * i;
                const f32x4_t a0 = lp[0], a1 = lp[1], a2 = lp[2];
                t0 = make_float4(a0.x, a0.y, a0.z, a0.w); t1 = make_float4(a1.x, a1.y, a1.z, a1.w); t2 = make_float4(a2.x, a2.y, a2.z, a2.w);
              } else
              if (PREFETCH) {
                t0 = n0; t1 = n1; t2 = n2;
                if (i + 1u < triCount) { const float4* tn = sc.tri_w + (size_t)(triIdx + 1u) * 3; n0 = tn[0]; n1 = tn[1]; n2 = tn[2]; }
              } else {
                const float4* tp = sc.tri_w + (size_t)triIdx * 3;
                t0 = tp[0]; t1 = tp[1]; t2 = tp[2];
              }
              if (STATS) fx.tri++;
              float bx, by, bz;
              const float d = ray_tri(arx, ary, arz, cdx, cdy, cdz, t0, t1, t2, bx, by, bz);
              if (d < hitd) {
                hitd = d;
                flags |= F_FOUND;
                if (!(job_base(JOB) == JOB_RENDER_SHADOW && (flags & F_SHADOW))) { CTX(3) = __float_as_uint(bx); CTX(4) = __float_as_uint(by); CTX(6) = CTX(8); CTX(7) = triIdx; }
                if (flags & F_ANYHIT) { stop = true; break; }
                if (!(path_m < hitd)) break;
              }
            }
            if (stop) { sp = 0; tos_d = DESC_DONE; cur = DESC_DONE; }
            else pop_next();
          }
        }
      }
      if (STATS && A.wave_log) { const unsigned long long t1 = __builtin_readcyclecounter(); wl_tl += t1 - wl_t0; }
      RT_MARK("loop_exit");
      const unsigned long long work = __ballot(is_work_desc(cur));
      if (work == 0ull) break;
      const unsigned long long done = __ballot(cur == DESC_DONE);
      const uint32_t n_done = (uint32_t)__popcll(done);
      const uint32_t n_idle = queue_empty && loc_next == loc_end ? 0u : 64u - (uint32_t)__popcll(work | done);
      if (n_done + n_idle >= DEAD_MAX || n_done >= FINISH_MIN) break;
    }

    RT_MARK("finish");
    if (STATS && A.wave_log) wl_tmark = __builtin_readcyclecounter();
    if (cur == DESC_DONE) {
      const bool found = (flags & F_FOUND) != 0u;
      HitRec h; h.dist = RT_LARGE_FLOAT; h.bx = 0; h.by = 0; h.bz = 0; h.blasIdx = 0; h.triIdx = 0;
      if (is_trace_job(JOB)) {
        if (found) {
          h.dist = hitd; h.bx = __uint_as_float(CTX(3)); h.by = __uint_as_float(CTX(4)); h.bz = 1 - h.bx - h.by;
          h.blasIdx = CTX(6); h.triIdx = CTX(7);
        }
        if (RT_TRACE_NT) {
          uint32_t* hp = (uint32_t*)hit_slot();
          __builtin_nontemporal_store(__float_as_uint(h.dist), hp); __builtin_nontemporal_store(__float_as_uint(h.bx), hp + 1);
          __builtin_nontemporal_store(__float_as_uint(h.by), hp + 2); __builtin_nontemporal_store(__float_as_uint(h.bz), hp + 3);
          __builtin_nontemporal_store(h.blasIdx, hp + 4); __builtin_nontemporal_store(h.triIdx, hp + 5);
        } else *hit_slot() = h;
        cur = DESC_IDLE;
      } else if (JOB == JOB_RENDER_GI) {
        uint32_t x, y;
        pixel_of(job, x, y);
        const size_t e = (size_t)x + (size_t)y * A.W;
        bool write = false;
        float cr = 0.f, cg = 0.f, cb = 0.f;
        if (found) {
          h.dist = hitd; h.bx = __uint_as_float(CTX(3)); h.by = __uint_as_float(CTX(4)); h.bz = 1 - h.bx - h.by;
          h.blasIdx = CTX(6); h.triIdx = CTX(7);
        }
        if (!(flags & F_SHADOW)) {
          float ox, oy, oz, dx, dy, dz;
          generate_ray(A.utab[x], A.vtab[y], ox, oy, oz, dx, dy, dz);
          if (!found) {
            cr = p.bg[0]; cg = p.bg[1]; cb = p.bg[2];
            write = true;
          } else {
            float r, g, b, refl, Ix, Iy, Iz, Nx, Ny, Nz, a3[3];
            shade_terms<false>(sc, p, ox, oy, oz, dx, dy, dz, h, false, r, g, b, refl, Ix, Iy, Iz, Nx, Ny, Nz, nullptr, a3);
            float thr = 1.0f;
            thr *= refl;
            g_col[0] = r + p.bg[0] * thr; g_col[1] = g + p.bg[1] * thr; g_col[2] = b + p.bg[2] * thr;
            g_alb[0] = a3[0]; g_alb[1] = a3[1]; g_alb[2] = a3[2];
            ao_sample_ray(x, y, A.W, 1u, 0u, A.gi_seed, Ix, Iy, Iz, Nx, Ny, Nz, dx, dy, dz, g_ray);
            flags = F_SHADOW;
            start_ray(g_ray[0], g_ray[1], g_ray[2], g_ray[3], g_ray[4], g_ray[5], RT_LARGE_FLOAT, false);
          }
        } else {
          float r, g, b;
          shade_eval<false>(sc, p, g_ray[0], g_ray[1], g_ray[2], g_ray[3], g_ray[4], g_ray[5], h, found, false, r, g, b);
          cr = g_col[0] + g_alb[0] * r; cg = g_col[1] + g_alb[1] * g; cb = g_col[2] + g_alb[2] * b;
          write = true;
        }
        if (write) {
          A.dst[e] = pack_rgb8(cr, cg, cb);
          if (A.colors) { A.colors[3 * e] = cr; A.colors[3 * e + 1] = cg; A.colors[3 * e + 2] = cb; }
          cur = DESC_IDLE;
        }
      } else if (!(flags & F_SHADOW)) {
        if (STATS && found) nhit++;
        if (job_base(JOB) == JOB_RENDER_SHADOW && found) {
          uint32_t x, y;
          pixel_of(job, x, y);
          float ox, oy, oz, dx, dy, dz, sox, soy, soz, sdx, sdy, sdz, sdist;
          pixel_ray(x, y, ox, oy, oz, dx, dy, dz);
          float lpx = p.lpos[0], lpy = p.lpos[1], lpz = p.lpos[2];
          if (A.pbatch) { const ShadeParams* q = A.pbatch + fast_div(job >> 6, A.div_frame_tiles); lpx = q->lpos[0]; lpy = q->lpos[1]; lpz = q->lpos[2]; }
          shadow_ray(lpx, lpy, lpz, ox, oy, oz, dx, dy, dz, hitd, sox, soy, soz, sdx, sdy, sdz, sdist);
          CTX(5) = __float_as_uint(hitd);
          flags = F_SHADOW;
          start_ray(sox, soy, soz, sdx, sdy, sdz, sdist, true);
        } else {
          if (found) {
            h.dist = hitd; h.bx = __uint_as_float(CTX(3)); h.by = __uint_as_float(CTX(4)); h.bz = 1 - h.bx - h.by;
            h.blasIdx = CTX(6); h.triIdx = CTX(7);
          }
          *hit_slot() = h;
          cur = DESC_IDLE;
        }
      } else if (EXACT && (flags & F_RESUMED)) {
        if (found) hit_slot()->blasIdx |= 0x80000000u;
        cur = DESC_IDLE;
      } else {
        h.bx = __uint_as_float(CTX(3)); h.by = __uint_as_float(CTX(4)); h.bz = 1 - h.bx - h.by;
        h.dist = __uint_as_float(CTX(5)); h.blasIdx = CTX(6) | (found ? 0x80000000u : 0u); h.triIdx = CTX(7);
        *hit_slot() = h;
        cur = DESC_IDLE;
      }
    }
    if (STATS && A.wave_log) wl_tfin += __builtin_readcyclecounter() - wl_tmark;
  }
#undef CTX

  if (STATS && A.wave_log && !EXACT) {
    unsigned s = nrays;
    for (int o = 32; o > 0; o >>= 1) s += __shfl_down(s, o);
    for (int o = 32; o > 0; o >>= 1) wl_no23 += __shfl_down(wl_no23, o);
    if (lane == 0) {
      unsigned long long* w = A.wave_log + 16ull * (blockIdx.x * (uint32_t)WG_WAVES + (threadIdx.x >> 6));
      w[13] = wl_tf; w[14] = wl_tfin; w[15] = wl_tq;
      w[0] = t_first; w[1] = wall_clock64(); w[2] = s; w[8] = wl_no23;
      w[9] = (unsigned long long)wl_no3 | ((unsigned long long)(uint32_t)__builtin_amdgcn_s_getreg((3 << 11) | (0 << 6) | 20) << 56);
      w[10] = wl_tn; w[11] = wl_tl; w[12] = __builtin_readcyclecounter() - wl_tstart;
      w[3] = wl_iter; w[4] = wl_node_x; w[5] = wl_node_l; w[6] = wl_leaf_x; w[7] = wl_leaf_l;
    }
  }
  if (!EXACT && A.end_log) {
    unsigned s = nrays;
    for (int o = 32; o > 0; o >>= 1) s += __shfl_down(s, o);
    if (lane == 0) {
      unsigned long long* w = A.end_log + 2ull * (blockIdx.x * (uint32_t)WG_WAVES + (threadIdx.x >> 6));
      w[0] = wall_clock64();
      w[1] = (unsigned long long)s | ((unsigned long long)(uint32_t)__builtin_amdgcn_s_getreg((3 << 11) | (0 << 6) | 20) << 56);
    }
  }
  if (A.counters) {
    __shared__ unsigned s_cnt[5];
    if (threadIdx.x < 5u) s_cnt[threadIdx.x] = 0u;
    __syncthreads();
    unsigned v[5] = {nrays, fx.node, fx.inst, fx.tri, nhit};
#pragma unroll
    for (int k = 0; k < (STATS ? 5 : 1); ++k) {
      unsigned s = v[k];
      for (int o = 32; o > 0; o >>= 1) s += __shfl_down(s, o);
      if (lane == 0 && s) atomicAdd(&s_cnt[k], s);
    }
    __syncthreads();
    if (threadIdx.x < (STATS ? 5u : 1u) && s_cnt[threadIdx.x]) atomicAdd(A.counters + threadIdx.x, (unsigned long long)s_cnt[threadIdx.x]);
  }
}

__device__ __forceinline__ uint32_t lpt_cls(uint32_t c) {
  if (c < 64u) return c;
  const uint32_t e = 31u - (uint32_t)__clz((int)c);
  return ((e - 5u) << 6) | ((c >> (e - 6u)) & 63u);
}
__device__ void lpt_order_block(uint32_t shard, const uint32_t* __restrict__ cost, uint32_t* __restrict__ order,
                                uint32_t n_tiles, uint32_t tiles_per_shard, uint32_t* hist ,
                                const uint32_t* __restrict__ base_order = nullptr) {
  const uint32_t lo = shard * tiles_per_shard;
  const uint32_t hi = min(lo + tiles_per_shard, n_tiles);
  if (lo >= hi) return;
  const uint32_t lane = threadIdx.x & 63u, wave = threadIdx.x >> 6;
  for (uint32_t i = threadIdx.x; i < 2048u; i += 256u) hist[i] = 0u;
  __syncthreads();
  for (uint32_t t = lo + threadIdx.x; t < hi; t += 256u) atomicAdd(&hist[2047u - lpt_cls(cost[base_order ? base_order[t] : t])], 1u);
  __syncthreads();
  uint32_t v[8], sum = 0;
#pragma unroll
  for (int k = 0; k < 8; ++k) { v[k] = hist[threadIdx.x * 8u + k]; sum += v[k]; }
  uint32_t inc = sum;
  for (int o = 1; o < 64; o <<= 1) { const uint32_t y = __shfl_up(inc, o); if (lane >= (uint32_t)o) inc += y; }
  if (lane == 63u) hist[2048u + wave] = inc;
  __syncthreads();
  uint32_t base = inc - sum;
  for (uint32_t w = 0; w < wave; ++w) base += hist[2048u + w];
#pragma unroll
  for (int k = 0; k < 8; ++k) { hist[threadIdx.x * 8u + k] = base; base += v[k]; }
  __syncthreads();
  for (uint32_t t = lo + threadIdx.x; t < hi; t += 256u) {
    const uint32_t tile = base_order ? base_order[t] : t;
    order[lo + atomicAdd(&hist[2047u - lpt_cls(cost[tile])], 1u)] = tile;
  }
}

template <bool STATS, bool CAM>
__device__ __forceinline__ void shade_pass(SceneDev sc, ShadeParams p, uint32_t W, uint32_t H, uint32_t y0, uint32_t y1, uint32_t row_step,
                                           uint32_t n_rows, const float* __restrict__ utab, const float* __restrict__ vtab,
                                           const HitRec* __restrict__ hb, uint32_t* __restrict__ dst,
                                           HitRec* __restrict__ hits, float* __restrict__ colors,
                                           unsigned long long* counters, uint32_t* __restrict__ ctl_reset,
                                           uint32_t lpt_blocks, const uint32_t* __restrict__ lpt_cost, uint32_t* __restrict__ lpt_order,
                                           uint32_t lpt_tiles, uint32_t lpt_per_shard,
                                           uint32_t batch, const ShadeParams* __restrict__ pbatch, uint64_t dst_frame_stride,
                                           const uint32_t* __restrict__ lpt_base) {
  __shared__ uint32_t s_hist[2048 + 8];
  if (blockIdx.x < lpt_blocks) { lpt_order_block(blockIdx.x, lpt_cost, lpt_order, lpt_tiles, lpt_per_shard, s_hist, lpt_base); return; }
  const uint32_t blk = blockIdx.x - lpt_blocks;
  if (ctl_reset && blk == 0)
    for (uint32_t i = threadIdx.x; i < CTL_DWORDS; i += 256u) ctl_reset[i] = 0u;
  const uint64_t t = (uint64_t)blk * 256u + threadIdx.x;
  const uint64_t n = (uint64_t)W * n_rows * batch;
  unsigned ntex = 0, npix = 0;
  const uint32_t x = (uint32_t)(t % W), vr = (uint32_t)(t / W);
  const uint32_t frame = batch > 1 ? vr / n_rows : 0u, lr = vr - frame * n_rows, y = frame_row(lr, y0, row_step);
  if (batch > 1 && t < n) { p = pbatch[frame]; dst += (size_t)frame * dst_frame_stride; }
  if (t < n && y < y1) {
    const size_t idx = (size_t)x + (size_t)y * W;
    HitRec h = hb[hit_index(x, vr, (W + 7u) >> 3)];
    const uint32_t occ_bit = h.blasIdx & 0x80000000u;
    const bool occ = occ_bit != 0u;
    h.blasIdx &= 0x7fffffffu;
    const bool found = h.dist != RT_LARGE_FLOAT;
    float ox, oy, oz, dx, dy, dz;
    frame_pixel_ray<CAM>(utab, vtab, W, H, frame, x, y, ox, oy, oz, dx, dy, dz);
    float r, g, b;
    shade_eval<STATS>(sc, p, ox, oy, oz, dx, dy, dz, h, found, occ, r, g, b, &ntex);
    dst[idx] = pack_rgb8(r, g, b);
    if (hits) { HitRec o = h; o.blasIdx |= occ_bit; hits[idx] = o; }
    if (colors) { colors[3 * idx] = r; colors[3 * idx + 1] = g; colors[3 * idx + 2] = b; }
    npix = 1;
  }
  if (STATS && counters) {
    const uint32_t lane = threadIdx.x & 63u;
    unsigned v[2] = {ntex, npix};
#pragma unroll
    for (int k = 0; k < 2; ++k) {
      unsigned s = v[k];
      for (int o = 32; o > 0; o >>= 1) s += __shfl_down(s, o);
      if (lane == 0 && s) atomicAdd(counters + 5 + k, (unsigned long long)s);
    }
  }
}
template <bool STATS>
__global__ __launch_bounds__(256) void rt_shade_kernel(SceneDev sc, ShadeParams p, uint32_t W, uint32_t H, uint32_t y0, uint32_t y1, uint32_t row_step,
                                                      uint32_t n_rows, const float* __restrict__ utab, const float* __restrict__ vtab,
                                                      const HitRec* __restrict__ hb, uint32_t* __restrict__ dst,
                                                      HitRec* __restrict__ hits, float* __restrict__ colors,
                                                      unsigned long long* counters, uint32_t* __restrict__ ctl_reset,
                                                      uint32_t lpt_blocks, const uint32_t* __restrict__ lpt_cost, uint32_t* __restrict__ lpt_order,
                                                      uint32_t lpt_tiles, uint32_t lpt_per_shard,
                                                      uint32_t batch = 1, const ShadeParams* __restrict__ pbatch = nullptr, uint64_t dst_frame_stride = 0,
                                                      const uint32_t* __restrict__ lpt_base = nullptr) {
  shade_pass<STATS, false>(sc, p, W, H, y0, y1, row_step, n_rows, utab, vtab, hb, dst, hits, colors, counters, ctl_reset, lpt_blocks, lpt_cost, lpt_order,
                           lpt_tiles, lpt_per_shard, batch, pbatch, dst_frame_stride, lpt_base);
}
template <bool BATCH>
__global__ __launch_bounds__(256) void rt_shade_camera_kernel(SceneDev sc, ShadeParams p, uint32_t W, uint32_t H, uint32_t y0, uint32_t y1, uint32_t row_step,
                                                             uint32_t n_rows, const float* __restrict__ cam,
                                                             const HitRec* __restrict__ hb, uint32_t* __restrict__ dst,
                                                             HitRec* __restrict__ hits, float* __restrict__ colors, uint32_t* __restrict__ ctl_reset,
                                                             uint32_t lpt_blocks, const uint32_t* __restrict__ lpt_cost, uint32_t* __restrict__ lpt_order,
                                                             uint32_t lpt_tiles, uint32_t lpt_per_shard,
                                                             uint32_t batch, const ShadeParams* __restrict__ pbatch, uint64_t dst_frame_stride,
                                                             const uint32_t* __restrict__ lpt_base) {
  shade_pass<false, true>(sc, p, W, H, y0, y1, row_step, n_rows, cam, cam + CAM_TAB, hb, dst, hits, colors, nullptr, ctl_reset, lpt_blocks, lpt_cost, lpt_order,
                          lpt_tiles, lpt_per_shard, BATCH ? batch : 1u, pbatch, dst_frame_stride, lpt_base);
}

__global__ __launch_bounds__(256) void rt_shade_rays_kernel(SceneDev sc, ShadeParams p, uint64_t n, const float* __restrict__ rays,
                                                           const HitRec* __restrict__ hits, float* __restrict__ colors, uint32_t* __restrict__ rgb8) {
  const uint64_t i = (uint64_t)blockIdx.x * 256u + threadIdx.x;
  if (i >= n) return;
  const float* rp = rays + i * 6;
  HitRec h = hits[i];
  h.blasIdx &= 0x7fffffffu;
  float r, g, b;
  shade_eval<false>(sc, p, rp[0], rp[1], rp[2], rp[3], rp[4], rp[5], h, h.dist != RT_LARGE_FLOAT, false, r, g, b);
  if (colors) { colors[3 * i] = r; colors[3 * i + 1] = g; colors[3 * i + 2] = b; }
  if (rgb8) rgb8[i] = pack_rgb8(r, g, b);
}

template <bool LEVEL0, bool CAM>
__device__ __forceinline__ void shade_bounce_pass(SceneDev sc, ShadeParams p, uint32_t level, uint64_t n,
    uint32_t W, uint32_t H, uint32_t y0, const float* __restrict__ utab, const float* __restrict__ vtab,
    const HitRec* __restrict__ hb, const float* __restrict__ rays, const HitRec* __restrict__ shits,
    float4* __restrict__ term, float* __restrict__ col, uint32_t* __restrict__ dst, HitRec* __restrict__ hits_out,
    float* __restrict__ colors_out, uint32_t* next_count, float* __restrict__ next_rays, uint32_t* __restrict__ next_parent,
    uint32_t* __restrict__ ctl_reset) {
  if (ctl_reset && blockIdx.x == 0)
    for (uint32_t i = threadIdx.x; i < CTL_DWORDS; i += 256u) ctl_reset[i] = 0u;
  const uint64_t t = (uint64_t)blockIdx.x * 256u + threadIdx.x;
  if (t >= n) return;
  size_t e = (size_t)t;
  float ox, oy, oz, dx, dy, dz;
  HitRec h;
  bool occ;
  if (LEVEL0) {
    const uint32_t x = (uint32_t)(t % W), y = y0 + (uint32_t)(t / W);
    e = (size_t)x + (size_t)y * W;
    h = hb[hit_index(x, y - y0, (W + 7u) >> 3)];
    occ = (h.blasIdx & 0x80000000u) != 0u;
    if (hits_out) hits_out[e] = h;
    h.blasIdx &= 0x7fffffffu;
    frame_pixel_ray<CAM>(utab, vtab, W, H, 0u, x, y, ox, oy, oz, dx, dy, dz);
  } else {
    const float* rp = rays + e * 6;
    ox = rp[0]; oy = rp[1]; oz = rp[2]; dx = rp[3]; dy = rp[4]; dz = rp[5];
    h = hb[e];
    occ = shits != nullptr && shits[e].dist != RT_LARGE_FLOAT;
  }
  float r, g, b;
  bool final_ = true;
  if (h.dist == RT_LARGE_FLOAT) {
    r = p.bg[0]; g = p.bg[1]; b = p.bg[2];
  } else {
    float refl, Ix, Iy, Iz, Nx, Ny, Nz;
    shade_terms<false>(sc, p, ox, oy, oz, dx, dy, dz, h, occ, r, g, b, refl, Ix, Iy, Iz, Nx, Ny, Nz);
    if (refl > 0.0f && level + 1u < p.max_depth) {
      final_ = false;
      term[e] = make_float4(r, g, b, refl);
      const uint32_t slot = atomicAdd(next_count, 1u);
      mirror_ray(dx, dy, dz, Ix, Iy, Iz, Nx, Ny, Nz, next_rays + (size_t)slot * 6);
      next_parent[slot] = (uint32_t)e;
    } else {
      float thr = 1.0f;
      thr *= refl;
      r = r + p.bg[0] * thr;
      g = g + p.bg[1] * thr;
      b = b + p.bg[2] * thr;
    }
  }
  if (final_) {
    if (LEVEL0) {
      dst[e] = pack_rgb8(r, g, b);
      if (colors_out) { colors_out[3 * e] = r; colors_out[3 * e + 1] = g; colors_out[3 * e + 2] = b; }
    } else {
      col[3 * e] = r; col[3 * e + 1] = g; col[3 * e + 2] = b;
    }
  }
}
template <bool LEVEL0>
__global__ __launch_bounds__(256) void rt_shade_bounce_kernel(SceneDev sc, ShadeParams p, uint32_t level, uint64_t n,
    uint32_t W, uint32_t y0, const float* __restrict__ utab, const float* __restrict__ vtab,
    const HitRec* __restrict__ hb, const float* __restrict__ rays, const HitRec* __restrict__ shits,
    float4* __restrict__ term, float* __restrict__ col, uint32_t* __restrict__ dst, HitRec* __restrict__ hits_out,
    float* __restrict__ colors_out, uint32_t* next_count, float* __restrict__ next_rays, uint32_t* __restrict__ next_parent,
    uint32_t* __restrict__ ctl_reset) {
  shade_bounce_pass<LEVEL0, false>(sc, p, level, n, W, 0u, y0, utab, vtab, hb, rays, shits, term, col, dst, hits_out, colors_out, next_count, next_rays,
                                   next_parent, ctl_reset);
}
__global__ __launch_bounds__(256) void rt_shade_bounce_camera_kernel(SceneDev sc, ShadeParams p, uint64_t n, uint32_t W, uint32_t H, uint32_t y0,
    const float* __restrict__ cam, const HitRec* __restrict__ hb, float4* __restrict__ term, uint32_t* __restrict__ dst, HitRec* __restrict__ hits_out,
    float* __restrict__ colors_out, uint32_t* next_count, float* __restrict__ next_rays, uint32_t* __restrict__ next_parent, uint32_t* __restrict__ ctl_reset) {
  shade_bounce_pass<true, true>(sc, p, 0u, n, W, H, y0, cam, cam + CAM_TAB, hb, nullptr, nullptr, term, nullptr, dst, hits_out, colors_out, next_count,
                                next_rays, next_parent, ctl_reset);
}

__global__ __launch_bounds__(256) void rt_bounce_shadow_rays_kernel(ShadeParams p, uint32_t n, const float* __restrict__ rays,
    const HitRec* __restrict__ hits, float* __restrict__ srays, float* __restrict__ stmax, unsigned long long* rays_traced) {
  const uint32_t i = blockIdx.x * 256u + threadIdx.x;
  bool real = false;
  if (i < n) {
    const float* rp = rays + (size_t)i * 6;
    float* sp = srays + (size_t)i * 6;
    const float d = hits[i].dist;
    if (d == RT_LARGE_FLOAT) {
      sp[0] = 0.f; sp[1] = 0.f; sp[2] = 0.f; sp[3] = 1.f; sp[4] = 1.f; sp[5] = 1.f;
      stmax[i] = -1.0f;
    } else {
      float sdist;
      shadow_ray(p, rp[0], rp[1], rp[2], rp[3], rp[4], rp[5], d, sp[0], sp[1], sp[2], sp[3], sp[4], sp[5], sdist);
      stmax[i] = sdist;
      real = true;
    }
  }
  const unsigned long long m = __ballot(real);
  if (rays_traced && (threadIdx.x & 63u) == 0u && m) atomicAdd(rays_traced, (unsigned long long)__popcll(m));
}

template <bool TO_PIXELS>
__global__ __launch_bounds__(256) void rt_bounce_unwind_kernel(uint32_t n, const uint32_t* __restrict__ parent, const float* __restrict__ col_k,
    const float4* __restrict__ term_prev, float* __restrict__ col_prev, uint32_t* __restrict__ dst, float* __restrict__ colors_out) {
  const uint32_t i = blockIdx.x * 256u + threadIdx.x;
  if (i >= n) return;
  const size_t q = parent[i];
  const float4 t = term_prev[q];
  float thr = 1.0f;
  thr *= t.w;
  const float r = t.x + col_k[3 * (size_t)i] * thr, g = t.y + col_k[3 * (size_t)i + 1] * thr, b = t.z + col_k[3 * (size_t)i + 2] * thr;
  if (TO_PIXELS) {
    dst[q] = pack_rgb8(r, g, b);
    if (colors_out) { colors_out[3 * q] = r; colors_out[3 * q + 1] = g; colors_out[3 * q + 2] = b; }
  } else {
    col_prev[3 * q] = r; col_prev[3 * q + 1] = g; col_prev[3 * q + 2] = b;
  }
}

#define AO_PREP_CHUNKS 4
__global__ __launch_bounds__(256) void rt_ao_prepare_kernel(SceneDev sc, ShadeParams p, uint64_t n, uint32_t W, uint32_t y0,
    const float* __restrict__ utab, const float* __restrict__ vtab, const HitRec* __restrict__ hb,
    float4* __restrict__ geo, float4* __restrict__ nrm, float4* __restrict__ col, uint32_t* __restrict__ cnt,
    uint32_t* __restrict__ list, uint32_t* hdr, uint32_t* ctl_reset, float4* __restrict__ alb ) {
  if (ctl_reset && blockIdx.x == 0)
    for (uint32_t i = threadIdx.x; i < CTL_DWORDS; i += 256u) ctl_reset[i] = 0u;
  __shared__ uint32_t s_cnt[AO_PREP_CHUNKS][4];
  const uint32_t lane = threadIdx.x & 63u, wv = threadIdx.x >> 6;
  bool hit_c[AO_PREP_CHUNKS];
  uint32_t off_c[AO_PREP_CHUNKS];
#pragma unroll
  for (int c = 0; c < AO_PREP_CHUNKS; ++c) {
    const uint64_t t = ((uint64_t)blockIdx.x * AO_PREP_CHUNKS + c) * 256u + threadIdx.x;
    bool hit = false;
    if (t < n) {
      const uint32_t x = (uint32_t)(t % W), y = y0 + (uint32_t)(t / W);
      HitRec h = hb[hit_index(x, y - y0, (W + 7u) >> 3)];
      h.blasIdx &= 0x7fffffffu;
      float ox, oy, oz, dx, dy, dz;
      generate_ray(utab[x], vtab[y], ox, oy, oz, dx, dy, dz);
      float r, g, b;
// ... 585 lines not shown
  uint32_t batch = 1;
  int shadow = 0;
  uint32_t* dst = nullptr; uint64_t dst_frame_stride = 0;
  vxrt_hit_t* hits = nullptr; float* colors = nullptr;
  unsigned long long* counters = nullptr;
  uint32_t* unoccluded = nullptr;
  unsigned long long* wave_log = nullptr;
  const vxrt_ao_params_t* ao = nullptr;
  const vxrt_camera_t* cams = nullptr;
  void* stream = nullptr;
  Counting counting = Counting::TIMED;
};

static int render_bounce_tail(vxrt_accel_t* a, FrameCtx* c, const RenderRequest& r, const ShadeParams& p, const float* utab, const float* vtab) {
  const SceneDev& sc = a->dev;
  const uint32_t width = r.width, y0 = r.y0, y1 = r.y1;
  const bool shadow = r.shadow != 0;
  uint32_t* dst = r.dst; float* colors = r.colors;
  unsigned long long* rays_traced = r.counters;
  hipStream_t s = (hipStream_t)r.stream;
  const uint64_t npix = (uint64_t)width * (y1 - y0);
  const uint64_t pix_span = (uint64_t)width * y1;
  if (npix > 0x7fffffffull) return -1;
  if (!c->bcount && hipMalloc((void**)&c->bcount, sizeof(uint32_t)) != hipSuccess) return -1;
  if (c->lv.size() < 2) c->lv.resize(2);
  if (!level_reserve(c->lv[0], pix_span, false, true)) return -1;
  if (!level_reserve(c->lv[1], npix, shadow, false)) return -1;
  dim3 block(256);
  if (hipMemsetAsync(c->bcount, 0, sizeof(uint32_t), s) != hipSuccess) return -1;
  if (r.cams) hipLaunchKernelGGL(rt_shade_bounce_camera_kernel, dim3((uint32_t)((npix + 255) / 256)), block, 0, s, sc, p, npix, width, r.height, y0, utab,
                                 (const HitRec*)c->hitbuf, c->lv[0].term, dst, (HitRec*)r.hits, colors, c->bcount, c->lv[1].rays, c->lv[1].parent, c->ctl);
  else hipLaunchKernelGGL(rt_shade_bounce_kernel<true>, dim3((uint32_t)((npix + 255) / 256)), block, 0, s, sc, p, 0u, npix, width, y0, utab, vtab,
                          (const HitRec*)c->hitbuf, (const float*)nullptr, (const HitRec*)nullptr, c->lv[0].term, (float*)nullptr, dst, (HitRec*)r.hits, colors,
                          c->bcount, c->lv[1].rays, c->lv[1].parent, c->ctl);
  if (hipGetLastError() != hipSuccess) return -1;
  c->ctl_dirty = false;
  uint32_t depth = 0;
  for (uint32_t k = 1; k < p.max_depth; ++k) {
    uint32_t n = 0;
    if (hipMemcpyAsync(&n, c->bcount, sizeof(uint32_t), hipMemcpyDeviceToHost, s) != hipSuccess) return -1;
    if (hipStreamSynchronize(s) != hipSuccess) return -1;
    if (n == 0) break;
    FrameCtx::Level& L = c->lv[k];
    L.n = n;
    depth = k;
    if (rays_traced) hipLaunchKernelGGL(add_counter_kernel, dim3(1), dim3(64), 0, s, rays_traced, (unsigned long long)n);
    if (trace_on_ctx(a, c, L.rays, n, nullptr, L.hits, VXRT_MODE_CLOSEST, s) != 0) return -1;
    const dim3 grid((n + 255u) / 256u);
    if (shadow) {
      hipLaunchKernelGGL(rt_bounce_shadow_rays_kernel, grid, block, 0, s, p, n, (const float*)L.rays, (const HitRec*)L.hits, L.srays, L.stmax, rays_traced);
      if (trace_on_ctx(a, c, L.srays, n, L.stmax, L.shits, MODE_ANY_UNORDERED, s) != 0) return -1;
    }
    if (c->lv.size() < (size_t)k + 2) c->lv.resize((size_t)k + 2);
    FrameCtx::Level& Nx = c->lv[k + 1];
    const bool more = k + 1 < p.max_depth;
    if (more && !level_reserve(Nx, n, shadow, false)) return -1;
    FrameCtx::Level& Lk = c->lv[k];
    if (hipMemsetAsync(c->bcount, 0, sizeof(uint32_t), s) != hipSuccess) return -1;
    hipLaunchKernelGGL(rt_shade_bounce_kernel<false>, grid, block, 0, s, sc, p, k, (uint64_t)n, width, y0, utab, vtab,
                       (const HitRec*)Lk.hits, (const float*)Lk.rays, shadow ? (const HitRec*)Lk.shits : (const HitRec*)nullptr, Lk.term, Lk.col,
                       (uint32_t*)nullptr, (HitRec*)nullptr, (float*)nullptr, c->bcount, more ? Nx.rays : (float*)nullptr, more ? Nx.parent : (uint32_t*)nullptr,
                       (uint32_t*)nullptr);
    if (hipGetLastError() != hipSuccess) return -1;
    if (!more) break;
  }
  for (uint32_t k = depth; k >= 1; --k) {
    FrameCtx::Level& L = c->lv[k];
    const dim3 grid((L.n + 255u) / 256u);
    if (k == 1) hipLaunchKernelGGL(rt_bounce_unwind_kernel<true>, grid, block, 0, s, L.n, (const uint32_t*)L.parent, (const float*)L.col, (const float4*)c->lv[0].term, (float*)nullptr, dst, colors);
    else        hipLaunchKernelGGL(rt_bounce_unwind_kernel<false>, grid, block, 0, s, L.n, (const uint32_t*)L.parent, (const float*)L.col, (const float4*)c->lv[k - 1].term, c->lv[k - 1].col, (uint32_t*)nullptr, (float*)nullptr);
  }
  return hipGetLastError() == hipSuccess ? 0 : -1;
}

#define AO_BATCH_RAYS (32ull << 20)
#define VXRT_AO_MODE_DIFFUSE_BOUNCE 1u
static int render_ao_tail(vxrt_accel_t* a, FrameCtx* c, const RenderRequest& r, const ShadeParams& p, const float* utab, const float* vtab) {
  const SceneDev& sc = a->dev;
  const vxrt_ao_params_t* ao = r.ao;
  const uint32_t width = r.width, y0 = r.y0, y1 = r.y1;
  hipStream_t s = (hipStream_t)r.stream;
  const uint64_t n = (uint64_t)width * (y1 - y0);
  if (ao->reserved == VXRT_AO_MODE_DIFFUSE_BOUNCE) return -1;
  if (n > 0x7fffffffull || ao->spp == 0) return -1;
  uint32_t ns = (uint32_t)std::min<uint64_t>(ao->spp, std::max<uint64_t>(1, AO_BATCH_RAYS / n));
  const uint64_t ray_cap = n * ns;
  if (ray_cap > 0x7fffffffull) return -1;
  if (c->ao_cap < n || c->ao_ray_cap < ray_cap) {
    if (hipStreamSynchronize(s) != hipSuccess) return -1;
    const uint64_t have = c->ao_cap, rhave = c->ao_ray_cap;
    bool ok = grow_buf((void**)&c->ao_geo, have, n, 16) && grow_buf((void**)&c->ao_nrm, have, n, 16) && grow_buf((void**)&c->ao_col, have, n, 16) &&
              grow_buf((void**)&c->ao_cnt, have, n, 4) && grow_buf((void**)&c->ao_list, have, n, 4) && grow_buf((void**)&c->ao_hdr, c->ao_hdr ? 1 : 0, 1, 8) &&
              grow_buf((void**)&c->ao_rays, rhave, ray_cap, 24) && grow_buf((void**)&c->ao_tmax, rhave, ray_cap, 4) &&
              grow_buf((void**)&c->ao_hits, rhave, ray_cap, sizeof(HitRec));
    if (!ok) return -1;
    c->ao_cap = std::max(have, n); c->ao_ray_cap = std::max(rhave, ray_cap);
  }
  const dim3 block(256), grid((uint32_t)((n + 255) / 256)), rgrid((uint32_t)((ray_cap + 255) / 256));
  static const bool sort_on = [] { const char* e = getenv("VXRT_SORT_SECONDARY"); return e && e[0] == '1'; }();
  const uint32_t cells_x = (width + (1u << BIN_CELL_SHIFT) - 1) >> BIN_CELL_SHIFT, cells_y = (y1 - y0 + (1u << BIN_CELL_SHIFT) - 1) >> BIN_CELL_SHIFT;
  const uint32_t n_cells = cells_x * cells_y, n_bins = 8u * n_cells;
  if (sort_on && (c->bin_cap < n_bins || c->bin_ray_cap < ray_cap)) {
    if (hipStreamSynchronize(s) != hipSuccess) return -1;
    bool ok = grow_buf((void**)&c->bin_hist, c->bin_cap, n_bins, 4) && grow_buf((void**)&c->bin_keys, c->bin_ray_cap, ray_cap, 4) &&
              grow_buf((void**)&c->bin_order, c->bin_ray_cap, ray_cap, 4);
    if (!ok) return -1;
    c->bin_cap = std::max<uint64_t>(c->bin_cap, n_bins); c->bin_ray_cap = std::max(c->bin_ray_cap, ray_cap);
  }
  auto bin_rays = [&](uint32_t ns_batch) -> const uint32_t* {
    if (!sort_on) return nullptr;
    if (hipMemsetAsync(c->bin_hist, 0, (size_t)n_bins * 4, s) != hipSuccess) return nullptr;
    hipLaunchKernelGGL(rt_bin_count_kernel, rgrid, block, 0, s, ray_cap, (const uint32_t*)c->ao_hdr, (const float*)c->ao_rays, (const uint32_t*)c->ao_list, ns_batch,
                       width, cells_x, n_cells, c->bin_hist, c->bin_keys);
    hipLaunchKernelGGL(rt_bin_scan_kernel, dim3(1), dim3(1024), 0, s, c->bin_hist, n_bins, (n_bins + 1023u) / 1024u);
    hipLaunchKernelGGL(rt_bin_scatter_kernel, rgrid, block, 0, s, ray_cap, (const uint32_t*)c->ao_hdr, (const uint32_t*)c->bin_keys, c->bin_hist, c->bin_order);
    return c->bin_order;
  };
  if (hipMemsetAsync(c->ao_hdr, 0, 8, s) != hipSuccess) return -1;
  hipLaunchKernelGGL(rt_ao_prepare_kernel, dim3((uint32_t)((n + 256u * AO_PREP_CHUNKS - 1u) / (256u * AO_PREP_CHUNKS))), block, 0, s, sc, p, n, width, y0, utab, vtab, (const HitRec*)c->hitbuf,
                     c->ao_geo, c->ao_nrm, c->ao_col, c->ao_cnt, c->ao_list, c->ao_hdr, c->ctl, (float4*)nullptr);
  if (hipGetLastError() != hipSuccess) return -1;
  c->ctl_dirty = false;
  for (uint32_t s0 = 0; s0 < ao->spp; s0 += ns) {
    const uint32_t k = std::min(ns, ao->spp - s0);
    hipLaunchKernelGGL(rt_ao_rays_kernel, rgrid, block, 0, s, ray_cap, width, y0, utab, vtab, (const float4*)c->ao_geo, (const float4*)c->ao_nrm,
                       (const uint32_t*)c->ao_list, c->ao_hdr, ao->spp, s0, k, ao->seed, ao->radius, c->ao_rays, c->ao_tmax);
    if (trace_on_ctx(a, c, c->ao_rays, n * k, c->ao_tmax, c->ao_hits, MODE_ANY_UNORDERED, s, c->ao_hdr + 1, nullptr, bin_rays(k)) != 0) return -1;
    hipLaunchKernelGGL(rt_ao_accumulate_kernel, rgrid, block, 0, s, ray_cap, (const uint32_t*)c->ao_list, (const uint32_t*)c->ao_hdr, k,
                       (const HitRec*)c->ao_hits, c->ao_cnt);
  }
  hipLaunchKernelGGL(rt_ao_final_kernel, grid, block, 0, s, n, width, y0, (const float4*)c->ao_geo, (const float4*)c->ao_col, (const uint32_t*)c->ao_cnt,
                     ao->spp, r.dst, r.colors, r.unoccluded, r.counters);
  return hipGetLastError() == hipSuccess ? 0 : -1;
}


struct Tiles {
  uint32_t x, y;
  uint32_t row_step;
  uint32_t per_frame;
  uint64_t total;
};
static Tiles window_tiles(const RenderRequest& r) {
  Tiles t;
  t.x = (r.width + 7) / 8; t.y = ((r.y1 - r.y0 + 7) / 8 + r.stride - 1) / r.stride;
  t.row_step = 8u * r.stride;
  t.per_frame = t.x * t.y;
  t.total = (uint64_t)t.x * t.y * r.batch;
  return t;
}

static bool mirror_frame(const vxrt_accel* a, const vxrt_shade_params_t& params) { return params.max_depth > 1 && a->max_reflectivity > 0.0f; }
static bool gi_fused_frame(const RenderRequest& r) { return r.ao && r.ao->reserved == VXRT_AO_MODE_DIFFUSE_BOUNCE; }

static int check_request(const vxrt_accel* a, const RenderRequest& r) {
  const bool stats = r.counting != Counting::TIMED;
  if (!a || a->stale || !r.params || !r.dst) return -1;
  if (r.cams && (r.stride != 1 || r.ao || stats || r.wave_log || r.unoccluded)) return -1;
  if (r.batch == 0 || r.batch > VXRT_MAX_BATCH) return -1;
  if (r.batch > 1 && (r.hits || r.colors || r.ao || ((stats || r.wave_log) && !(r.counting == Counting::TIMED_TRAVERSAL && r.wave_log)))) return -1;
  if (r.ao && (stats || r.shadow)) return -1;
  if (r.stride == 0 || (r.stride > 1 && ((r.y0 & 7u) != 0 || r.ao))) return -1;
  if (!a->ref.triEx || !a->ref.mat || a->ref.n_mats == 0) return -1;
  if (r.width == 0 || r.height == 0 || r.y0 > r.y1 || r.y1 > r.height) return -1;
  if (stats && !r.counters) return -1;
  if (r.y0 == r.y1) return 0;
  if (window_tiles(r).total > 0x1ffffffull) return -1;
  if (mirror_frame(a, r.params[0]) && (stats || r.stride > 1 || r.batch > 1)) return -1;
  if (r.batch > 1)
    for (uint32_t f = 0; f < r.batch; ++f)
      if (mirror_frame(a, r.params[f])) return -1;
  if (gi_fused_frame(r) && (stats || r.shadow || r.unoccluded)) return -1;
  return 1;
}

static bool lpt_wanted(const vxrt_accel* a, const RenderRequest& r, uint32_t n_tiles) {
  const HostKnobs& k = host_knobs();
  if (!k.lpt || !(r.counting == Counting::TIMED || r.wave_log)) return false;
  if (n_tiles < LPT_MIN_TILES) return false;
  if (r.batch == 1) return a->n_ctx == 1;
  if (!k.lpt_batch) return false;
  if (n_tiles <= k.lpt_batch_max) return true;
  return k.lpt_batch_alone && a->n_ctx == 1;
}

static bool ensure_uv_tables(vxrt_accel* a, uint32_t width, uint32_t height, hipStream_t s) {
  if (a->uv_w == width && a->uv_h == height) return true;
  std::vector<float> tab((size_t)width + height);
  for (uint32_t x = 0; x < width; ++x) tab[x] = (float)(((double)x * 2.0 - (double)width) / (double)height);
  for (uint32_t y = 0; y < height; ++y) tab[width + y] = (float)(((double)y * 2.0 - (double)height) / (double)height);
  a->uv_w = a->uv_h = 0;
  uint64_t none = 0;
  if (!grow_device({{(void**)&a->uvtab, sizeof(float)}}, &none, tab.size(), GrowSync::DEVICE, s)) return false;
  if (hipMemcpy(a->uvtab, tab.data(), tab.size() * sizeof(float), hipMemcpyHostToDevice) != hipSuccess) return false;
  a->uv_w = width; a->uv_h = height;
  return true;
}

static bool upload_cameras(FrameCtx* c, const RenderRequest& r, hipStream_t s) {
  const uint64_t need = CAM_TAB + (uint64_t)r.batch * (r.width + r.height);
  if (!grow_device({{(void**)&c->cam, sizeof(float)}}, &c->cam_floats, need, GrowSync::STREAM, s)) return false;
  CamBatch cb;
  for (uint32_t f = 0; f < VXRT_MAX_BATCH; ++f) cb.c[f] = r.cams[f < r.batch ? f : 0];
  const uint32_t g = (uint32_t)std::min<uint64_t>((need + 255) / 256, 1024);
  hipLaunchKernelGGL(rt_camera_prep_kernel, dim3(g), dim3(256), 0, s, cb, r.batch, r.width, r.height, c->cam);
  return hipGetLastError() == hipSuccess;
}

static bool upload_batch(vxrt_accel* a, FrameCtx* c, const RenderRequest& r, const Tiles& t, hipStream_t s) {
  if (!c->pbatch && hipMalloc((void**)&c->pbatch, VXRT_MAX_BATCH * sizeof(ShadeParams)) != hipSuccess) return false;
  ShadeBatch sb;
  for (uint32_t f = 0; f < VXRT_MAX_BATCH; ++f) sb.p[f] = shade_params(r.params[f < r.batch ? f : 0]);
  hipLaunchKernelGGL(set_batch_params_kernel, dim3(1), dim3(64), 0, s, sb, r.batch, c->pbatch);
  if (a->bo_tiles != t.per_frame) {
    if (hipDeviceSynchronize() != hipSuccess) return false;
    for (uint32_t k = 0; k <= VXRT_MAX_BATCH; ++k) { (void)hipFree(a->batch_order[k]); a->batch_order[k] = nullptr; }
    a->bo_tiles = t.per_frame;
  }
  if (!a->batch_order[r.batch]) {
    std::vector<uint32_t> ord;
    ord.reserve(t.total);
    const uint32_t band = (t.per_frame + QUEUE_SHARDS - 1) / QUEUE_SHARDS;
    for (uint32_t sh = 0; sh < QUEUE_SHARDS; ++sh)
      for (uint32_t f = 0; f < r.batch; ++f)
        for (uint32_t k = sh * band; k < std::min(t.per_frame, (sh + 1) * band); ++k) ord.push_back(f * t.per_frame + k);
    if (hipMalloc((void**)&a->batch_order[r.batch], ord.size() * sizeof(uint32_t)) != hipSuccess) return false;
    if (hipMemcpy(a->batch_order[r.batch], ord.data(), ord.size() * sizeof(uint32_t), hipMemcpyHostToDevice) != hipSuccess) return false;
  }
  return true;
}

static bool ensure_lpt_tables(FrameCtx* c, const RenderRequest& r, uint32_t n_tiles, PersistArgs& A, hipStream_t s) {
  FrameCtx::Lpt& L = c->lpt[r.batch];
  const bool grows = L.cap < n_tiles;
  if (!grow_device({{(void**)&L.cost, 4 * 4}, {(void**)&L.order, 4}}, &L.cap, n_tiles, GrowSync::STREAM, s)) return false;
  if (grows) L.valid = false;
  const uint32_t key[6] = {r.width, r.height, r.y0, r.y1, (uint32_t)r.shadow | (r.stride << 1), (r.ao ? 1u : 0u) | (r.batch << 1) | (r.cams ? 0x80000000u : 0u)};
  if (memcmp(key, L.key, sizeof key) != 0) { L.valid = false; memcpy(L.key, key, sizeof key); }
  if (!L.cost || !L.order) return false;
  A.tile_cost = L.cost;
  if (L.valid) A.tile_order = L.order;
  else if (r.batch == 1) A.tile_order = nullptr;
  return true;
}

static bool ensure_apriori(vxrt_accel* a, const RenderRequest& r, const Tiles& t, hipStream_t s) {
  if (a->ap_key[0] == r.width && a->ap_key[1] == r.height && a->ap_key[2] == r.y0 && a->ap_key[3] == r.y1 && a->ap_key[4] == r.stride && a->ap_key[5] >= r.batch && a->apriori) return true;
  std::vector<uint32_t> list(1, 0u);
  for (uint32_t k = 0; k < t.per_frame; ++k)
    for (uint32_t l = 0; l < 64; ++l) {
      const uint32_t x = (k % t.x) * 8u + (l & 7u), y = r.y0 + (k / t.x) * t.row_step + (l >> 3);
      if (x >= r.width || y >= r.y1) continue;
      const float u = (float)(((double)x * 2.0 - (double)r.width) / (double)r.height);
      const float v = (float)(((double)y * 2.0 - (double)r.height) / (double)r.height);
      if (u == 0.0f || v == 0.0f) list.push_back(k * 64u + l);
    }
  const size_t per_frame = list.size() - 1;
  for (uint32_t f = 1; f < r.batch; ++f)
    for (size_t i = 0; i < per_frame; ++i) list.push_back(list[1 + i] + f * t.per_frame * 64u);
  list[0] = (uint32_t)(list.size() - 1);
  if (hipDeviceSynchronize() != hipSuccess) return false;
  if (!grow_device({{(void**)&a->apriori, sizeof(uint32_t)}}, &a->ap_cap, list.size(), GrowSync::NONE, s)) return false;
  if (hipMemcpy(a->apriori, list.data(), list.size() * sizeof(uint32_t), hipMemcpyHostToDevice) != hipSuccess) return false;
  a->ap_count = (uint32_t)per_frame;
  a->ap_key[0] = r.width; a->ap_key[1] = r.height; a->ap_key[2] = r.y0; a->ap_key[3] = r.y1; a->ap_key[4] = r.stride; a->ap_key[5] = r.batch;
  return true;
}

static bool frame_resources(vxrt_accel* a, FrameCtx* c, const RenderRequest& r, const Tiles& t, bool lpt, PersistArgs& A, hipStream_t s) {
  const uint32_t n_tiles = (uint32_t)t.total;
  const uint64_t pixels = r.batch > 1 ? (uint64_t)n_tiles * 64u : (uint64_t)t.x * ((r.height + 7) / 8 + 1) * 64u;
  if (!grow_device({{&c->hitbuf, sizeof(HitRec)}}, &c->hitbuf_pixels, pixels, GrowSync::STREAM, s)) return false;
  if (!r.cams && !ensure_uv_tables(a, r.width, r.height, s)) return false;
  A.W = r.width; A.H = r.height; A.y0 = r.y0; A.y1 = r.y1; A.tiles_x = t.x; A.row_step = t.row_step; A.total = n_tiles * 64u;
  A.div_tiles_x = fast_div_make(t.x); A.div_frame_tiles = fast_div_make(t.per_frame); A.frame_tiles = t.per_frame;
  A.hits = (HitRec*)c->hitbuf; A.counters = r.counters; A.wave_log = r.wave_log; A.end_log = a->end_log;
  A.utab = a->uvtab; A.vtab = a->uvtab + r.width;
  if (r.cams) {
    if (!upload_cameras(c, r, s)) return false;
    A.utab = c->cam; A.vtab = c->cam + CAM_TAB;
  }
  if (r.batch > 1) {
    if (!upload_batch(a, c, r, t, s)) return false;
    A.pbatch = c->pbatch; A.tile_order = a->batch_order[r.batch];
  }
  if (!grow_device({{(void**)&c->defer, sizeof(uint32_t)}}, &c->defer_cap, A.total, GrowSync::STREAM, s)) return false;
  A.defer_count = c->ctl; A.defer_list = c->defer; A.defer_cap = A.total;
  A.queue = c->ctl + 32;
  A.per_shard = ((A.total + QUEUE_SHARDS - 1) / QUEUE_SHARDS + 63u) & ~63u;
  A.shard_rot = host_knobs().shard_rot;
  if (lpt && !ensure_lpt_tables(c, r, n_tiles, A, s)) return false;
  return r.cams || ensure_apriori(a, r, t, s);
}

struct LaunchPlan {
  bool lpt;
  bool packed;
  bool side_launch;
  uint32_t side_wgs;
  bool side_reserve;
  uint32_t grid_div;
  bool grid_div_small;
};
static LaunchPlan launch_plan(const vxrt_accel* a, const RenderRequest& r, uint32_t n_tiles, bool lpt, uint32_t ap_count) {
  const HostKnobs& k = host_knobs();
  LaunchPlan plan;
  plan.lpt = lpt;
  plan.packed = k.packed >= 0 ? k.packed != 0 : ((a->n_ctx > 1 || (k.packed_batch && r.batch > 1)) && n_tiles >= LPT_MIN_TILES);
  plan.side_launch = ap_count != 0;
  plan.side_wgs = plan.side_launch ? std::min<uint32_t>(EXACT_GRID, (ap_count + 255u) / 256u) : 0u;
  plan.side_reserve = k.side_reserve >= 0 ? k.side_reserve != 0 : a->n_ctx == 1;
  plan.grid_div = k.grid_div > 0 ? (uint32_t)k.grid_div : ((k.grid_div == 0 && a->n_ctx > 1) ? a->n_ctx : 1u);
  plan.grid_div_small = k.grid_div == 0;
  return plan;
}

template <class K>
static uint32_t main_grid(K kernel, const LaunchPlan& plan, uint32_t total) {
  const uint32_t side_wgs_r = plan.side_reserve ? plan.side_wgs : 0u;
  uint32_t g = persistent_grid(kernel, total + (uint64_t)side_wgs_r * RT_WG_THREADS);
  const uint32_t cap = persistent_grid(kernel, ~0ull >> 8);
  const uint32_t div = (plan.grid_div_small && (uint64_t)total >= 2ull * 64ull * RT_WG_WAVES * cap) ? 1u : plan.grid_div;
  if (div > 1u) g = std::min<uint32_t>(g, std::max<uint32_t>(cap / div, 1u));
  return std::max<uint32_t>(1u, g > side_wgs_r ? g - side_wgs_r : 1u);
}

struct FrameLaunch {
  const vxrt_accel* a; FrameCtx* c; const LaunchPlan& plan; const ShadeParams& p; hipStream_t s;
  PersistArgs A, X, X0;
};

template <int JOB, int STATS, bool PACKED>
static void launch_traversal(const FrameLaunch& l) {
  static_assert(!(PACKED && (JOB == JOB_RENDER_GI || STATS != 0)), "only the timed render jobs have a packed form");
  with_decode_and_depth<STATS == 0>(l.a, [&](auto ld, auto sh) {
    const auto k_main = rt_persistent_kernel<JOB, STATS, decltype(ld)::value, false, PACKED, decltype(sh)::value>;
    const auto k_exact = rt_persistent_kernel<JOB, STATS, decltype(ld)::value, true>;
    if (l.plan.side_launch) hipLaunchKernelGGL(k_exact, dim3(l.plan.side_wgs), dim3(256), 0, l.c->side, l.a->dev, l.p, l.X0);
    hipLaunchKernelGGL(k_main, dim3(main_grid(k_main, l.plan, l.A.total)), dim3(RT_WG_THREADS), 0, l.s, l.a->dev, l.p, l.A);
    hipLaunchKernelGGL(k_exact, dim3(EXACT_GRID), dim3(256), 0, l.s, l.a->dev, l.p, l.X);
  });
}
template <int STATS, bool PACKED, int CAM = 0>
static void launch_render(bool shadow, const FrameLaunch& l) {
  if (shadow) launch_traversal<JOB_RENDER_SHADOW | CAM, STATS, PACKED>(l); else launch_traversal<JOB_RENDER | CAM, STATS, PACKED>(l);
}

static bool traverse_frame(vxrt_accel* a, FrameCtx* c, const RenderRequest& r, const LaunchPlan& plan, const ShadeParams& p, const PersistArgs& A, hipStream_t s) {
  FrameLaunch l{a, c, plan, p, s, A, A, A};
  l.X.queue = c->ctl + 32 + CTL_QUEUE_DWORDS;
  c->ctl_dirty = true;
  if (plan.side_launch) {
    const bool drained = hipStreamQuery(s) == hipSuccess;
    if (!drained && (hipEventRecord(c->ev_in, s) != hipSuccess || hipStreamWaitEvent(c->side, c->ev_in, 0) != hipSuccess)) return false;
    const uint32_t ap_count = a->ap_count * r.batch;
    l.X0.queue = c->ctl + 32 + 2 * CTL_QUEUE_DWORDS;
    l.X0.defer_count = a->apriori; l.X0.defer_list = a->apriori + 1; l.X0.defer_cap = ap_count;
  }
  if (gi_fused_frame(r)) {
    for (PersistArgs* g : {&l.A, &l.X, &l.X0}) { g->dst = r.dst; g->colors = r.colors; g->gi_seed = r.ao->seed; }
    launch_traversal<JOB_RENDER_GI, 0, false>(l);
  }
  else if (r.counting == Counting::TIMED_TRAVERSAL) launch_render<2, false>(r.shadow != 0, l);
  else if (r.counting == Counting::REFERENCE_ORDER) launch_render<1, false>(r.shadow != 0, l);
  else if (r.cams)      launch_render<0, false, JOB_CAM>(r.shadow != 0, l);
  else if (plan.packed) launch_render<0, true>(r.shadow != 0, l);
  else                  launch_render<0, false>(r.shadow != 0, l);
  return !plan.side_launch || (hipEventRecord(c->ev_side, c->side) == hipSuccess && hipStreamWaitEvent(s, c->ev_side, 0) == hipSuccess);
}

static bool shade_frame(vxrt_accel* a, FrameCtx* c, const RenderRequest& r, const Tiles& t, bool lpt_sort, const ShadeParams& p, const PersistArgs& A, hipStream_t s) {
  const FrameCtx::Lpt& L = c->lpt[r.batch];
  const uint32_t n_tiles = (uint32_t)t.total, n_rows = t.y * 8u;
  const uint64_t npx = (uint64_t)r.width * n_rows * r.batch;
  const uint32_t lpt_blocks = lpt_sort ? QUEUE_SHARDS : 0u;
  const dim3 sgrid((uint32_t)((npx + 255) / 256) + lpt_blocks), block(256);
  const uint32_t* base_order = r.batch > 1 ? (const uint32_t*)a->batch_order[r.batch] : (const uint32_t*)nullptr;
  if (r.cams) {
    hipLaunchKernelGGL(r.batch > 1 ? rt_shade_camera_kernel<true> : rt_shade_camera_kernel<false>, sgrid, block, 0, s, a->dev, p, r.width, r.height, r.y0, r.y1, t.row_step,
                       n_rows, (const float*)A.utab, (const HitRec*)c->hitbuf, r.dst, (HitRec*)r.hits, r.colors, c->ctl, lpt_blocks, (const uint32_t*)L.cost,
                       L.order, n_tiles, A.per_shard >> 6, r.batch, (const ShadeParams*)c->pbatch, r.dst_frame_stride, base_order);
  } else {
    const bool stats = r.counting != Counting::TIMED;
    hipLaunchKernelGGL(stats ? rt_shade_kernel<true> : rt_shade_kernel<false>, sgrid, block, 0, s, a->dev, p, r.width, r.height, r.y0, r.y1, t.row_step,
                       n_rows, A.utab, A.vtab, (const HitRec*)c->hitbuf, r.dst, (HitRec*)r.hits, r.colors, r.counters, c->ctl, lpt_blocks, (const uint32_t*)L.cost,
                       L.order, n_tiles, A.per_shard >> 6, stats ? 1u : r.batch, stats ? (const ShadeParams*)nullptr : (const ShadeParams*)c->pbatch,
                       stats ? (uint64_t)0 : r.dst_frame_stride, base_order);
  }
  return hipGetLastError() == hipSuccess;
}

static int render_common(vxrt_accel_t* a, const RenderRequest& r) {
  const int go = check_request(a, r);
  if (go <= 0) return go;
  uint32_t* st = status_word();
  if (!st) return -1;
  const ShadeParams p = shade_params(r.params[0]);
  const Tiles t = window_tiles(r);
  hipStream_t s = (hipStream_t)r.stream;
  FrameCtx* c = acquire_ctx(a, s);
  if (!c) return -1;
  auto fail = [&]() -> int { c->ctl_dirty = true; (void)release_ctx(a, c, s); return -1; };
  const bool lpt = lpt_wanted(a, r, (uint32_t)t.total);
  PersistArgs A{};
  A.status = st;
  if (!frame_resources(a, c, r, t, lpt, A, s)) return fail();
  const LaunchPlan plan = launch_plan(a, r, (uint32_t)t.total, lpt, r.cams ? 0u : a->ap_count * r.batch);
  if (!traverse_frame(a, c, r, plan, p, A, s)) return fail();
  const bool mirror = mirror_frame(a, r.params[0]);
  const bool lpt_sort = plan.lpt && !r.ao && !mirror;
  if (plan.lpt && !lpt_sort) c->lpt[r.batch].valid = false;
  if (gi_fused_frame(r)) {
    if (hipGetLastError() != hipSuccess) return fail();
  } else if (r.ao) {
    if (render_ao_tail(a, c, r, p, A.utab, A.vtab) != 0) return fail();
  } else if (mirror) {
    if (render_bounce_tail(a, c, r, p, A.utab, A.vtab) != 0) return fail();
  } else {
    if (!shade_frame(a, c, r, t, lpt_sort, p, A, s)) return fail();
    if (lpt_sort) c->lpt[r.batch].valid = true;
    c->ctl_dirty = false;
  }
  return release_ctx(a, c, s);
}

extern "C" {

const char* vxrt_version(void) { return "vortex-rt-mi355x 0.3 (gfx950, compact 64-byte nodes, persistent wavefronts)"; }

int vxrt_render(vxrt_accel_t* accel, uint32_t width, uint32_t height, uint32_t y0, uint32_t y1,
                const vxrt_shade_params_t* params, int shadow, uint32_t* dst, vxrt_hit_t* hits,
                float* colors, unsigned long long* rays_traced, void* stream) {
  RenderRequest r;
  r.width = width; r.height = height; r.y0 = y0; r.y1 = y1; r.params = params; r.shadow = shadow;
  r.dst = dst; r.hits = hits; r.colors = colors; r.counters = rays_traced; r.stream = stream;
  return render_common(accel, r);
}

int vxrt_render_interleaved(vxrt_accel_t* accel, uint32_t width, uint32_t height, uint32_t phase, uint32_t stride,
                            const vxrt_shade_params_t* params, int shadow, uint32_t* dst, vxrt_hit_t* hits,
                            float* colors, unsigned long long* rays_traced, void* stream) {
  if (stride == 0 || phase >= stride) return -1;
  if ((uint64_t)phase * 8u >= height) return 0;
  RenderRequest r;
  r.width = width; r.height = height; r.y0 = phase * 8u; r.y1 = height; r.stride = stride; r.params = params; r.shadow = shadow;
  r.dst = dst; r.hits = hits; r.colors = colors; r.counters = rays_traced; r.stream = stream;
  return render_common(accel, r);
}

int vxrt_render_interleaved_batch(vxrt_accel_t* accel, uint32_t width, uint32_t height, uint32_t phase, uint32_t stride, uint32_t n_frames,
                                  const vxrt_shade_params_t* params, int shadow, uint32_t* dst, uint64_t dst_frame_stride,
                                  unsigned long long* rays_traced, void* stream) {
  if (stride == 0 || phase >= stride || n_frames == 0) return -1;
  if ((uint64_t)phase * 8u >= height) return 0;
  RenderRequest r;
  r.width = width; r.height = height; r.y0 = phase * 8u; r.y1 = height; r.stride = stride; r.params = params; r.batch = n_frames; r.shadow = shadow;
  r.dst = dst; r.dst_frame_stride = dst_frame_stride; r.counters = rays_traced; r.stream = stream;
  return render_common(accel, r);
}

int vxrt_render_rows_batch(vxrt_accel_t* accel, uint32_t width, uint32_t height, uint32_t y0, uint32_t y1, uint32_t n_frames,
                           const vxrt_shade_params_t* params, int shadow, uint32_t* dst, uint64_t dst_frame_stride,
                           unsigned long long* rays_traced, void* stream) {
  if (n_frames == 0) return -1;
  RenderRequest r;
  r.width = width; r.height = height; r.y0 = y0; r.y1 = y1; r.params = params; r.batch = n_frames; r.shadow = shadow;
  r.dst = dst; r.dst_frame_stride = dst_frame_stride; r.counters = rays_traced; r.stream = stream;
  return render_common(accel, r);
}

int vxrt_render_interleaved_batch_wave_log(vxrt_accel_t* accel, uint32_t width, uint32_t height, uint32_t phase, uint32_t stride, uint32_t n_frames,
                                           const vxrt_shade_params_t* params, int shadow, uint32_t* dst, uint64_t dst_frame_stride,
                                           unsigned long long* counters, unsigned long long* wave_log, void* stream) {
  if (stride == 0 || phase >= stride || n_frames == 0 || !wave_log || !counters) return -1;
  RenderRequest r;
  r.width = width; r.height = height; r.y0 = phase * 8u; r.y1 = height; r.stride = stride; r.params = params; r.batch = n_frames; r.shadow = shadow;
  r.dst = dst; r.dst_frame_stride = dst_frame_stride; r.counters = counters; r.wave_log = wave_log; r.stream = stream;
  r.counting = Counting::TIMED_TRAVERSAL;
  return render_common(accel, r);
}

int vxrt_render_batch(vxrt_accel_t* accel, uint32_t width, uint32_t height, uint32_t n_frames, const vxrt_shade_params_t* params, int shadow,
                      uint32_t* dst, uint64_t dst_frame_stride, unsigned long long* rays_traced, void* stream) {
  return vxrt_render_interleaved_batch(accel, width, height, 0, 1, n_frames, params, shadow, dst, dst_frame_stride, rays_traced, stream);
}

static bool camera_ok(const vxrt_camera_t* c) {
  if (!c) return false;
  const float* f = &c->pos[0];
  for (int i = 0; i < 14; ++i) if (!std::isfinite(f[i])) return false;
  return true;
}

int vxrt_render_camera(vxrt_accel_t* accel, const vxrt_camera_t* cam, uint32_t width, uint32_t height, uint32_t y0, uint32_t y1,
                       const vxrt_shade_params_t* params, int shadow, uint32_t* dst, vxrt_hit_t* hits, float* colors,
                       unsigned long long* rays_traced, void* stream) {
  if (!camera_ok(cam)) return -1;
  RenderRequest r;
  r.width = width; r.height = height; r.y0 = y0; r.y1 = y1; r.params = params; r.shadow = shadow; r.cams = cam;
  r.dst = dst; r.hits = hits; r.colors = colors; r.counters = rays_traced; r.stream = stream;
  return render_common(accel, r);
}

int vxrt_render_batch_camera(vxrt_accel_t* accel, uint32_t width, uint32_t height, uint32_t n_frames, const vxrt_camera_t* cams,
                             const vxrt_shade_params_t* params, int shadow, uint32_t* dst, uint64_t dst_frame_stride,
                             unsigned long long* rays_traced, void* stream) {
  if (!cams || n_frames == 0 || n_frames > VXRT_MAX_BATCH) return -1;
  for (uint32_t f = 0; f < n_frames; ++f) if (!camera_ok(cams + f)) return -1;
  if (!accel || accel->stale || !params || !dst) return -1;
  if (height == 0) return 0;
  RenderRequest r;
  r.width = width; r.height = height; r.y0 = 0; r.y1 = height; r.params = params; r.batch = n_frames; r.shadow = shadow; r.cams = cams;
  r.dst = dst; r.dst_frame_stride = dst_frame_stride; r.counters = rays_traced; r.stream = stream;
  return render_common(accel, r);
}

int vxrt_render_stats(vxrt_accel_t* accel, uint32_t width, uint32_t height, uint32_t y0, uint32_t y1,
                      const vxrt_shade_params_t* params, int shadow, uint32_t* dst,
                      unsigned long long* counters, void* stream) {
  RenderRequest r;
  r.width = width; r.height = height; r.y0 = y0; r.y1 = y1; r.params = params; r.shadow = shadow;
  r.dst = dst; r.counters = counters; r.stream = stream; r.counting = Counting::REFERENCE_ORDER;
  return render_common(accel, r);
}

int vxrt_render_stats_timed(vxrt_accel_t* accel, uint32_t width, uint32_t height, uint32_t y0, uint32_t y1,
                            const vxrt_shade_params_t* params, int shadow, uint32_t* dst,
                            unsigned long long* counters, void* stream) {
  RenderRequest r;
  r.width = width; r.height = height; r.y0 = y0; r.y1 = y1; r.params = params; r.shadow = shadow;
  r.dst = dst; r.counters = counters; r.stream = stream; r.counting = Counting::TIMED_TRAVERSAL;
  return render_common(accel, r);
}

int vxrt_render_wave_log(vxrt_accel_t* accel, uint32_t width, uint32_t height, uint32_t y0, uint32_t y1,
                         const vxrt_shade_params_t* params, int shadow, uint32_t* dst,
                         unsigned long long* counters, unsigned long long* wave_log, void* stream) {
  RenderRequest r;
  r.width = width; r.height = height; r.y0 = y0; r.y1 = y1; r.params = params; r.shadow = shadow;
  r.dst = dst; r.counters = counters; r.wave_log = wave_log; r.stream = stream; r.counting = Counting::TIMED_TRAVERSAL;
// ... 154 lines not shown
```

vortex-raytracing_amd/csrc/rt_types.h:

```cpp
#pragma once
#include <stdint.h>

#define RT_LARGE_FLOAT 1e30f
#define RT_EPSILON 1e-6f
#define RT_BVH_WIDTH 4
#define RT_NODE_BYTES 52
#define RT_NODE_DWORDS 13
#define RT_BLAS_STRIDE 160
#define RT_TRI_BYTES 36
#define RT_MAX_TRAIL 32
#define RT_TRIEX_BYTES 64
#define RT_MAT_BYTES 88
#define RT_MAX_LEVELS 32
#define RT_STACK_ENTRIES (3 * RT_MAX_LEVELS)

#pragma pack(push, 1)
struct rt_child_t { uint8_t meta; uint8_t qaabb[6]; };
#pragma pack(pop)

struct rt_qnode_t {
  float origin[3];
  int8_t ex, ey, ez;
  uint8_t imask;
  uint32_t leftFirst;
  uint32_t leafData;
  rt_child_t children[RT_BVH_WIDTH];
};
static_assert(sizeof(rt_qnode_t) == RT_NODE_BYTES, "node layout");

struct rt_blas_t {
  uint32_t bvh_offset;
  float invTransform[16];
  float transform[16];
  uint64_t mat_offset;
  uint32_t tex_width, tex_height;
  float reflectivity;
  uint32_t _pad;
};
static_assert(sizeof(rt_blas_t) == RT_BLAS_STRIDE, "blas layout");

struct rt_tri_t { float v0[3], v1[3], v2[3]; };
static_assert(sizeof(rt_tri_t) == RT_TRI_BYTES, "tri layout");

struct rt_triex_t {
  float N0[3], N1[3], N2[3];
  float uv0[2], uv1[2], uv2[2];
  uint32_t texId;
};
static_assert(sizeof(rt_triex_t) == RT_TRIEX_BYTES, "triEx layout");

struct rt_material_t {
  float ambient[3], diffuse[3], specular[3], emissive[3];
  float shininess, ior, dissolve, reflectivity;
  int32_t diffuse_tex_id, illum;
  uint32_t tex_width, tex_height;
  uint64_t tex_offset;
};
static_assert(sizeof(rt_material_t) == RT_MAT_BYTES, "material layout");

#define DK_TLAS 0u
#define DK_BLAS 1u
#define DK_LEAF 2u
#define DK_INST 3u
#define DESC(kind, payload) (((kind) << 30) | (payload))
#define DESC_DONE 0xFFFFFFFEu
#define DESC_IDLE 0xFFFFFFFDu
#define DESC_NONE 0xFFFFFFFFu
#define PAYLOAD_MASK 0x3FFFFFFFu
#define DESC_TOP_FLAG 0x20000000u
#define DESC_TOP_SLOT 0x0000FFFFu
#define LEAF_FIRST_BITS 26
#define LEAF_FIRST_MASK 0x03FFFFFFu
#define LEAF_MAX_INLINE 15u
#define CNODE_VEC4 4
#define WTRI_FLOATS 12
#ifndef RT_SHALLOW_LEVELS
#define RT_SHALLOW_LEVELS 16
#endif
#ifndef RT_TOP_NODES
#define RT_TOP_NODES 0
#endif
#define RT_TOP_MAX 1024
static_assert(RT_TOP_NODES <= RT_TOP_MAX, "top-of-tree image");
#ifdef __HIPCC__
__device__ __forceinline__ bool is_node_desc(uint32_t d) { return d < 0x80000000u; }
__device__ __forceinline__ bool is_leaf_desc(uint32_t d) { return (d >> 30) == DK_LEAF; }
__device__ __forceinline__ bool is_inst_desc(uint32_t d) { return d >= 0xC0000000u && d < DESC_IDLE; }
__device__ __forceinline__ bool is_work_desc(uint32_t d) { return d < DESC_IDLE; }
#endif
```

vortex-raytracing_amd/rtapi.py:

```python
import ctypes as C

from .runtime import hip_lib, check

MODE_CLOSEST, MODE_ANY = 0, 1


class VxrtScene(C.Structure):
    _fields_ = [("tlas", C.c_void_p), ("blas", C.c_void_p), ("bvh", C.c_void_p), ("tri", C.c_void_p),
                ("triEx", C.c_void_p), ("mat", C.c_void_p), ("tex", C.c_void_p),
                ("n_tlas_nodes", C.c_uint32), ("n_blas", C.c_uint32), ("n_bvh_nodes", C.c_uint32),
                ("n_tris", C.c_uint32), ("n_mats", C.c_uint32), ("reserved", C.c_uint32), ("tex_bytes", C.c_uint64)]


class ShadeParams(C.Structure):
    _fields_ = [("ambient", C.c_float * 3), ("light_color", C.c_float * 3), ("light_pos", C.c_float * 3),
                ("background", C.c_float * 3), ("max_depth", C.c_uint32)]


def default_shade_params():
    p = ShadeParams()
    p.ambient[:] = (0.4, 0.4, 0.4)
    p.light_color[:] = (1.0, 1.0, 1.0)
    p.light_pos[:] = (0.0, 10.0, -10.0)
    p.background[:] = (0.4, 0.35, 0.25)
# ... 64 lines not shown
def tlas_build(boxes_ptr, n_instances, nodes_ptr, node_capacity, stream=None):
    L = _lib()
    L.vxrt_tlas_build.restype = C.c_int
    L.vxrt_tlas_build.argtypes = [C.c_void_p, C.c_uint32, C.c_void_p, C.c_uint32, C.POINTER(BvhInfo), C.c_void_p]
    info = BvhInfo()
    rc = L.vxrt_tlas_build(boxes_ptr, n_instances, nodes_ptr, node_capacity, C.byref(info), stream)
    if rc == -2:
        raise BvhTooDeep("vxrt_tlas_build: tree depth %d exceeds the reference's 32 levels" % info.max_depth)
    check(rc, "vxrt_tlas_build")
    return info


REFIT_INSTANCES, REFIT_GEOMETRY = 1, 2


def accel_refit(accel, what, stream=None):
    L = _lib()
    L.vxrt_accel_refit.restype = C.c_int
    L.vxrt_accel_refit.argtypes = [C.c_void_p, C.c_uint32, C.c_void_p]
    check(L.vxrt_accel_refit(accel, int(what), stream), "vxrt_accel_refit")


def accel_set_transforms(accel, first, count, ptr, stream=None):
    L = _lib()
    L.vxrt_accel_set_transforms.restype = C.c_int
    L.vxrt_accel_set_transforms.argtypes = [C.c_void_p, C.c_uint32, C.c_uint32, C.c_void_p, C.c_void_p]
    check(L.vxrt_accel_set_transforms(accel, int(first), int(count), ptr, stream), "vxrt_accel_set_transforms")


def accel_destroy(accel):
    if accel:
        check(_lib().vxrt_accel_destroy(accel), "vxrt_accel_destroy")


def accel_frames_in_flight(accel, n):
    if _lib().vxrt_accel_frames_in_flight(accel, int(n)) != 0:
        raise RuntimeError("vxrt_accel_frames_in_flight(%r) failed" % (n,))


def trace_reference_quirks(image_ptr, image_size, offsets, rays_ptr, n, hits_ptr, mode=MODE_CLOSEST, tmax_ptr=None, stream=None):
    L = _lib()
    L.vxrt_trace_reference_quirks.restype = C.c_int
    L.vxrt_trace_reference_quirks.argtypes = [C.c_void_p, C.c_uint64, C.c_uint32, C.c_uint32, C.c_uint32, C.c_uint32, C.c_void_p, C.c_uint64,
                                              C.c_void_p, C.c_void_p, C.c_int, C.c_void_p]
    check(L.vxrt_trace_reference_quirks(image_ptr, image_size, offsets[0], offsets[1], offsets[2], offsets[3], rays_ptr, n, tmax_ptr, hits_ptr, mode, stream),
          "vxrt_trace_reference_quirks")


def debug_read_control(accel, ctx=0, n_dwords=800, stream=None):
    import numpy as np
    L = _lib()
    L.vxrt_debug_read_control.restype = C.c_int
    L.vxrt_debug_read_control.argtypes = [C.c_void_p, C.c_uint32, C.c_void_p, C.c_uint32, C.c_void_p]
    out = np.zeros(n_dwords, np.uint32)
    check(L.vxrt_debug_read_control(accel, ctx, out.ctypes.data, n_dwords, stream), "vxrt_debug_read_control")
    return out


def accel_bytes(accel):
    return int(_lib().vxrt_accel_bytes(accel))


def render(accel, width, height, y0, y1, params, dst_ptr, shadow=0, hits_ptr=None, colors_ptr=None, rays_ptr=None, stream=None):
    check(_lib().vxrt_render(accel, width, height, y0, y1, C.byref(params), int(shadow), dst_ptr, hits_ptr,
                             colors_ptr, rays_ptr, stream), "vxrt_render")


def render_interleaved(accel, width, height, phase, stride, params, dst_ptr, shadow=0, hits_ptr=None, colors_ptr=None, rays_ptr=None, stream=None):
    L = _lib()
    L.vxrt_render_interleaved.restype = C.c_int
    L.vxrt_render_interleaved.argtypes = [C.c_void_p, C.c_uint32, C.c_uint32, C.c_uint32, C.c_uint32, C.POINTER(ShadeParams), C.c_int,
                                          C.c_void_p, C.c_void_p, C.c_void_p, C.c_void_p, C.c_void_p]
    check(L.vxrt_render_interleaved(accel, width, height, int(phase), int(stride), C.byref(params), int(shadow), dst_ptr, hits_ptr,
                                    colors_ptr, rays_ptr, stream), "vxrt_render_interleaved")


def trace_stats(accel, rays_ptr, n, hits_ptr, mode=0, tmax_ptr=None, stream=None):
    import torch
    cnt = torch.zeros(8, dtype=torch.int64, device="cuda:%d" % torch.cuda.current_device())
    L = _lib()
    L.vxrt_trace_stats.restype = C.c_int
    L.vxrt_trace_stats.argtypes = [C.c_void_p, C.c_void_p, C.c_uint64, C.c_void_p, C.c_void_p, C.c_int, C.c_void_p, C.c_void_p]
    check(L.vxrt_trace_stats(accel, rays_ptr, n, tmax_ptr, hits_ptr, mode, cnt.data_ptr(), stream), "vxrt_trace_stats")
    torch.cuda.synchronize()
    r, nn, ni, nt = (int(v) for v in cnt.tolist()[:4])
    total = 24 * r + 52 * (nn + ni) + 36 * nt + 24 * r
    return {"rays": r, "node_fetches": nn, "inst_fetches": ni, "tri_fetches": nt, "bytes": total, "bytes_per_ray": total / max(r, 1)}


class RcScene(C.Structure):
    _fields_ = [(k, C.c_void_p) for k in ("tlas", "blas", "bvh", "tri", "triEx", "triIdx", "tex")] + \
               [(k, C.c_uint32) for k in ("n_tlas_nodes", "n_blas", "n_bvh_nodes", "n_tris", "n_tri_idx", "tlas_root")] + \
               [("tex_bytes", C.c_uint64)]


class RcParams(C.Structure):
    _fields_ = [("camera_pos", C.c_float * 3), ("camera_forward", C.c_float * 3), ("camera_right", C.c_float * 3),
                ("camera_up", C.c_float * 3), ("viewplane", C.c_float * 2),
                ("samples_per_pixel", C.c_uint32), ("max_depth", C.c_uint32),
                ("light_pos", C.c_float * 3), ("light_color", C.c_float * 3), ("ambient_color", C.c_float * 3),
                ("background_color", C.c_float * 3)]


def rc_params(cam14, light12, spp=1, max_depth=1):
    p = RcParams()
    c = [float(v) for v in cam14]
    p.camera_pos[:] = c[0:3]; p.camera_forward[:] = c[3:6]; p.camera_right[:] = c[6:9]; p.camera_up[:] = c[9:12]; p.viewplane[:] = c[12:14]
    l = [float(v) for v in light12]
    p.light_pos[:] = l[0:3]; p.light_color[:] = l[3:6]; p.ambient_color[:] = l[6:9]; p.background_color[:] = l[9:12]
    p.samples_per_pixel, p.max_depth = int(spp), int(max_depth)
    return p


def rc_render(scene, width, height, y0, y1, params, dst_ptr, colors_ptr=None, stream=None):
    L = _lib()
    L.vxrc_render.restype = C.c_int
    L.vxrc_render.argtypes = [C.POINTER(RcScene), C.c_uint32, C.c_uint32, C.c_uint32, C.c_uint32, C.POINTER(RcParams),
                              C.c_void_p, C.c_void_p, C.c_void_p]
    check(L.vxrc_render(C.byref(scene), width, height, y0, y1, C.byref(params), dst_ptr, colors_ptr, stream), "vxrc_render")


def rc_accel_build(scene, stream=None):
    L = _lib()
    L.vxrc_accel_build.restype = C.c_int
    L.vxrc_accel_build.argtypes = [C.POINTER(RcScene), C.c_void_p, C.POINTER(C.c_void_p)]
    h = C.c_void_p()
    check(L.vxrc_accel_build(C.byref(scene), stream, C.byref(h)), "vxrc_accel_build")
    return h


def wire_pack(frames_ptr, frame_stride, width, tile_rows_per_rank, world, rank, n_frames, wire_ptr, stream=None):
    L = _lib()
    L.vxrt_wire_pack.restype = C.c_int
    L.vxrt_wire_pack.argtypes = [C.c_void_p, C.c_uint64, C.c_uint32, C.c_uint32, C.c_uint32, C.c_uint32, C.c_uint32, C.c_void_p, C.c_void_p]
    check(L.vxrt_wire_pack(frames_ptr, frame_stride, width, tile_rows_per_rank, world, rank, n_frames, wire_ptr, stream), "vxrt_wire_pack")


def wire_unpack(wire_all_ptr, wire_stride_bytes, width, tile_rows_per_rank, world, n_frames, frames_ptr, frame_stride, stream=None):
    L = _lib()
    L.vxrt_wire_unpack.restype = C.c_int
    L.vxrt_wire_unpack.argtypes = [C.c_void_p, C.c_uint64, C.c_uint32, C.c_uint32, C.c_uint32, C.c_uint32, C.c_void_p, C.c_uint64, C.c_void_p]
    check(L.vxrt_wire_unpack(wire_all_ptr, wire_stride_bytes, width, tile_rows_per_rank, world, n_frames, frames_ptr, frame_stride, stream), "vxrt_wire_unpack")


def accel_info(accel, which):
    L = _lib()
    L.vxrt_accel_info.restype = C.c_int
    L.vxrt_accel_info.argtypes = [C.c_void_p, C.c_uint32, C.POINTER(C.c_uint64)]
    v = C.c_uint64()
    check(L.vxrt_accel_info(accel, which, C.byref(v)), "vxrt_accel_info")
    return int(v.value)


def rc_accel_info(accel, which):
    L = _lib()
    L.vxrc_accel_info.restype = C.c_int
    L.vxrc_accel_info.argtypes = [C.c_void_p, C.c_uint32, C.POINTER(C.c_uint64)]
    v = C.c_uint64()
    check(L.vxrc_accel_info(accel, which, C.byref(v)), "vxrc_accel_info")
    return int(v.value)


def rc_accel_destroy(accel):
    if accel:
        L = _lib()
        L.vxrc_accel_destroy.restype = C.c_int
        L.vxrc_accel_destroy.argtypes = [C.c_void_p]
        check(L.vxrc_accel_destroy(accel), "vxrc_accel_destroy")


def rc_render_accel(accel, width, height, y0, y1, params, dst_ptr, colors_ptr=None, stream=None):
    L = _lib()
    L.vxrc_render_accel.restype = C.c_int
    L.vxrc_render_accel.argtypes = [C.c_void_p, C.c_uint32, C.c_uint32, C.c_uint32, C.c_uint32, C.POINTER(RcParams), C.c_void_p, C.c_void_p, C.c_void_p]
    check(L.vxrc_render_accel(accel, width, height, y0, y1, C.byref(params), dst_ptr, colors_ptr, stream), "vxrc_render_accel")


class AoParams(C.Structure):
    _fields_ = [("spp", C.c_uint32), ("radius", C.c_float), ("seed", C.c_uint32), ("reserved", C.c_uint32)]


def render_ao(accel, width, height, y0, y1, params, spp, radius, dst_ptr, seed=0, colors_ptr=None, unoccluded_ptr=None,
              rays_ptr=None, stream=None):
    ao = AoParams(int(spp), float(radius), int(seed), 0)
    check(_lib().vxrt_render_ao(accel, width, height, y0, y1, C.byref(params), C.byref(ao), dst_ptr, colors_ptr,
                                unoccluded_ptr, rays_ptr, stream), "vxrt_render_ao")


def render_diffuse_bounce(accel, width, height, y0, y1, params, dst_ptr, seed=0, colors_ptr=None, rays_ptr=None, stream=None):
    L = _lib()
    L.vxrt_render_diffuse_bounce.restype = C.c_int
    L.vxrt_render_diffuse_bounce.argtypes = [C.c_void_p, C.c_uint32, C.c_uint32, C.c_uint32, C.c_uint32, C.POINTER(ShadeParams), C.c_uint32,
                                             C.c_void_p, C.c_void_p, C.c_void_p, C.c_void_p]
    check(L.vxrt_render_diffuse_bounce(accel, width, height, y0, y1, C.byref(params), int(seed), dst_ptr, colors_ptr, rays_ptr, stream),
          "vxrt_render_diffuse_bounce")


STAT_KEYS = ("rays", "node_fetches", "inst_fetches", "tri_fetches", "shaded_hits", "textured_hits", "pixels")


def algorithmic_bytes(c):
    return (52 * (c["node_fetches"] + c["inst_fetches"]) + 36 * c["tri_fetches"]
            + (64 + 88) * c["shaded_hits"] + 4 * c["textured_hits"] + 4 * c["pixels"])


def render_interleaved_batch(accel, width, height, phase, stride, params_list, dst_ptr, dst_frame_stride, shadow=0, rays_ptr=None, stream=None):
    L = _lib()
    L.vxrt_render_interleaved_batch.restype = C.c_int
    L.vxrt_render_interleaved_batch.argtypes = [C.c_void_p, C.c_uint32, C.c_uint32, C.c_uint32, C.c_uint32, C.c_uint32, C.POINTER(ShadeParams), C.c_int,
                                                C.c_void_p, C.c_uint64, C.c_void_p, C.c_void_p]
    arr = (ShadeParams * len(params_list))(*params_list)
    check(L.vxrt_render_interleaved_batch(accel, width, height, phase, stride, len(params_list), arr, int(shadow), dst_ptr, dst_frame_stride, rays_ptr, stream),
          "vxrt_render_interleaved_batch")


def render_rows_batch(accel, width, height, y0, y1, params_list, dst_ptr, dst_frame_stride, shadow=0, rays_ptr=None, stream=None):
    L = _lib()
    L.vxrt_render_rows_batch.restype = C.c_int
    L.vxrt_render_rows_batch.argtypes = [C.c_void_p, C.c_uint32, C.c_uint32, C.c_uint32, C.c_uint32, C.c_uint32, C.POINTER(ShadeParams), C.c_int,
                                         C.c_void_p, C.c_uint64, C.c_void_p, C.c_void_p]
    arr = (ShadeParams * len(params_list))(*params_list)
    check(L.vxrt_render_rows_batch(accel, width, height, y0, y1, len(params_list), arr, int(shadow), dst_ptr, dst_frame_stride, rays_ptr, stream),
          "vxrt_render_rows_batch")


def render_batch(accel, width, height, params_list, dst_ptr, dst_frame_stride, shadow=0, rays_ptr=None, stream=None):
    L = _lib()
    L.vxrt_render_batch.restype = C.c_int
    L.vxrt_render_batch.argtypes = [C.c_void_p, C.c_uint32, C.c_uint32, C.c_uint32, C.POINTER(ShadeParams), C.c_int, C.c_void_p, C.c_uint64, C.c_void_p, C.c_void_p]
    arr = (ShadeParams * len(params_list))(*params_list)
    check(L.vxrt_render_batch(accel, width, height, len(params_list), arr, int(shadow), dst_ptr, dst_frame_stride, rays_ptr, stream), "vxrt_render_batch")


def render_stats(accel, width, height, y0, y1, params, dst_ptr, shadow=0, stream=None, timed=False):
    import torch
    cnt = torch.zeros(8, dtype=torch.int64, device="cuda:%d" % torch.cuda.current_device())
    L = _lib()
    fn = L.vxrt_render_stats_timed if timed else L.vxrt_render_stats
    fn.restype = C.c_int
    fn.argtypes = [C.c_void_p, C.c_uint32, C.c_uint32, C.c_uint32, C.c_uint32, C.POINTER(ShadeParams), C.c_int, C.c_void_p, C.c_void_p, C.c_void_p]
    check(fn(accel, width, height, y0, y1, C.byref(params), int(shadow), dst_ptr, cnt.data_ptr(), stream), "vxrt_render_stats")
    torch.cuda.synchronize()
    c = dict(zip(STAT_KEYS, [int(v) for v in cnt[:7].tolist()]))
    c["bytes"] = algorithmic_bytes(c)
    return c


def trace(accel, rays_ptr, n, hits_ptr, mode=MODE_CLOSEST, tmax_ptr=None, stream=None):
    check(_lib().vxrt_trace(accel, rays_ptr, n, tmax_ptr, hits_ptr, mode, stream), "vxrt_trace")


def shade_rays(accel, rays_ptr, hits_ptr, n, params, colors_ptr=None, rgb8_ptr=None, stream=None):
    L = _lib()
    L.vxrt_shade_rays.restype = C.c_int
    L.vxrt_shade_rays.argtypes = [C.c_void_p, C.c_void_p, C.c_void_p, C.c_uint64, C.POINTER(ShadeParams), C.c_void_p, C.c_void_p, C.c_void_p]
    check(L.vxrt_shade_rays(accel, rays_ptr, hits_ptr, n, C.byref(params), colors_ptr, rgb8_ptr, stream), "vxrt_shade_rays")


def status(stream=None):
    st = C.c_uint32()
    check(_lib().vxrt_status(stream, C.byref(st)), "vxrt_status")
    return st.value


def version():
    return _lib().vxrt_version().decode()


class Camera(C.Structure):
    _fields_ = [("pos", C.c_float * 3), ("forward", C.c_float * 3), ("right", C.c_float * 3), ("up", C.c_float * 3),
                ("viewplane", C.c_float * 2)]

    @classmethod
    def from_cam14(cls, cam14):
        c = cls()
        v = [float(x) for x in cam14]
        if len(v) != 14:
            raise ValueError("a camera is 14 floats (pos, forward, right, up, viewplane)")
        c.pos[:] = v[0:3]; c.forward[:] = v[3:6]; c.right[:] = v[6:9]; c.up[:] = v[9:12]; c.viewplane[:] = v[12:14]
        return c

    def cam14(self):
        return list(self.pos) + list(self.forward) + list(self.right) + list(self.up) + list(self.viewplane)


def _camera(cam):
    return cam if isinstance(cam, Camera) else Camera.from_cam14(cam)


def look_at(eye, target, up, vfov_deg, width, height):
    import numpy as np
    f32 = np.float32
    e, t, u = (np.asarray(v, np.float32) for v in (eye, target, up))

    def normalize(v):
        inv = f32(1.0) / np.sqrt(f32(v[0] * v[0] + v[1] * v[1] + v[2] * v[2]))
        return (v * inv).astype(np.float32)

    def cross(a, b):
        return np.array([a[1] * b[2] - a[2] * b[1], a[2] * b[0] - a[0] * b[2], a[0] * b[1] - a[1] * b[0]], np.float32)

    fwd = normalize((t - e).astype(np.float32))
    right = normalize(cross(fwd, u))
    up2 = cross(right, fwd)
    aspect = f32(width) / f32(height)
    vh = f32(2.0) * np.tan(f32(vfov_deg) * f32(0.5))
# ... 32 lines not shown
```

Measured before the change: 11150 Mrays/s.

## Pack per-pixel hit records into 16-byte slim records for timed renders

Adds a slim pixel-record format for timed render frames that have no AO or mirror bounces. The record stores dist, bx and by plus a single 32-bit id that packs the BLAS index, the triangle index and the occlusion bit. bz is recomputed in the shade pass instead of being stored. The aim is to cut hit-buffer write and read traffic between the traversal and shade kernels. The cost is extra template instantiations, bit-packing logic, and a fallback to the full record when the id bits do not fit.

```diff
diff --git a/include/vortex_hip.h b/include/vortex_hip.h
--- a/include/vortex_hip.h
+++ b/include/vortex_hip.h
@@ -260,6 +260,8 @@
                                 const float* rays, uint64_t n, const float* tmax, vxrt_hit_t* hits, int mode, void* stream);
 
 int vxrt_debug_read_control(vxrt_accel_t* accel, uint32_t ctx, uint32_t* out, uint32_t n_dwords, void* stream);
+int vxrt_debug_pixel_record_bits(vxrt_accel_t* accel, uint32_t id_bits);
+int vxrt_debug_pixel_record_roundtrip(const vxrt_hit_t* in, uint64_t n, uint32_t tri_bits, vxrt_hit_t* out);
 int vxrt_debug_end_log(vxrt_accel_t* accel, unsigned long long* log);
 int vxrt_debug_trace_wave_log(vxrt_accel_t* accel, unsigned long long* log);
 int vxrt_debug_read_lpt(vxrt_accel_t* accel, uint32_t ctx, uint32_t batch, uint32_t* cost, uint32_t cost_cap, uint32_t* order, uint32_t order_cap,
diff --git a/vortex-raytracing_amd/csrc/rt_accel.hip b/vortex-raytracing_amd/csrc/rt_accel.hip
--- a/vortex-raytracing_amd/csrc/rt_accel.hip
+++ b/vortex-raytracing_amd/csrc/rt_accel.hip
@@ -400,6 +400,11 @@
   delete p;
 }
 
+static uint32_t pixrec_budget_env() {
+  static const uint32_t bits = [] { const char* e = getenv("VXRT_PIXREC_BITS"); return e ? (uint32_t)atoi(e) : PIXREC_ID_BITS; }();
+  return bits;
+}
+
 static void accel_free(vxrt_accel* a) {
   if (!a) return;
   (void)hipDeviceSynchronize();
@@ -523,6 +528,7 @@
   static const int shallow_env = [] { const char* e = getenv("VXRT_SHALLOW"); return e ? atoi(e) : -1; }();
   a->levels = levels;
   a->shallow = levels <= RT_SHALLOW_LEVELS && shallow_env != 0;
+  a->pix_tri_bits = pixrec_tri_bits(s->n_blas, s->n_tris, pixrec_budget_env());
   a->dev.nodes_c = (const uint4*)a->nodes_c; a->dev.ref_tlas = (const uint32_t*)s->tlas; a->dev.n_tlas = s->n_tlas_nodes; a->dev.tri_w = (const float4*)a->tri_w;
   a->dev.blas_root = (const uint32_t*)a->blas_root; a->dev.tlas_root = troot;
   a->dev.ident_root = 0u;
@@ -565,8 +571,30 @@
   case 1: *value = a->shallow ? 1u : 0u; return 0;
   case 2: *value = a->dev.ident_root; return 0;
   case 3: *value = a->dev.exact_decode; return 0;
+  case 4: *value = a->pix_tri_bits >= 0 ? 1u : 0u; return 0;
+  case 5: *value = a->pix_tri_bits >= 0 ? (uint64_t)a->pix_tri_bits : 0u; return 0;
   }
   return -1;
+}
+
+int vxrt_debug_pixel_record_bits(vxrt_accel_t* a, uint32_t id_bits) {
+  if (!a || id_bits > PIXREC_ID_BITS || hipDeviceSynchronize() != hipSuccess) return -2;
+  a->pix_tri_bits = id_bits ? pixrec_tri_bits(a->ref.n_blas, a->ref.n_tris, id_bits) : -1;
+  return a->pix_tri_bits;
+}
+
+int vxrt_debug_pixel_record_roundtrip(const vxrt_hit_t* in, uint64_t n, uint32_t tri_bits, vxrt_hit_t* out) {
+  if (!in || !out || tri_bits > PIXREC_ID_BITS) return -1;
+  const HitRec* src = (const HitRec*)in; HitRec* dst = (HitRec*)out;
+  for (uint64_t i = 0; i < n; ++i) {
+    const HitRec h = src[i];
+    if ((uint64_t)h.triIdx >> tri_bits || (uint64_t)(h.blasIdx & ~PIXREC_OCC) >> (PIXREC_ID_BITS - tri_bits)) return -1;
+    rt_pixrec_t q; q.dist = h.dist; q.bx = h.bx; q.by = h.by; q.id = pixrec_id(h.blasIdx, h.triIdx, tri_bits);
+    HitRec o; o.dist = q.dist; o.bx = q.bx; o.by = q.by; o.bz = pixrec_bz(q.dist, q.bx, q.by);
+    o.blasIdx = pixrec_blas24(q.id, tri_bits); o.triIdx = pixrec_tri(q.id, tri_bits);
+    dst[i] = o;
+  }
+  return 0;
 }
 
 int vxrt_accel_frames_in_flight(vxrt_accel_t* a, uint32_t n) {
diff --git a/vortex-raytracing_amd/csrc/rt_internal.h b/vortex-raytracing_amd/csrc/rt_internal.h
--- a/vortex-raytracing_amd/csrc/rt_internal.h
+++ b/vortex-raytracing_amd/csrc/rt_internal.h
@@ -83,6 +83,7 @@
   unsigned long long* end_log = nullptr;
   uint32_t levels = 0;
   bool shallow = false;
+  int pix_tri_bits = -1;
   int device = 0;
   struct RefitPlan* refit = nullptr;
   uint32_t blas_status = 0;
diff --git a/vortex-raytracing_amd/csrc/rt_kernels.hip b/vortex-raytracing_amd/csrc/rt_kernels.hip
--- a/vortex-raytracing_amd/csrc/rt_kernels.hip
+++ b/vortex-raytracing_amd/csrc/rt_kernels.hip
@@ -429,6 +429,7 @@
   uint32_t total;
   const uint32_t* total_dev;
   HitRec* hits;
+  uint32_t id_shift;
   const float* rays; const float* tmax; int any_hit;
   const uint32_t* order;
   unsigned long long* counters;
@@ -460,7 +461,7 @@
 #define F_WORLD 16u
 #define F_RESUMED 32u
 
-template <int JOB, int STATS, bool LDEXP, bool EXACT, bool PACKED = false, bool SHALLOW = false>
+template <int JOB, int STATS, bool LDEXP, bool EXACT, bool PACKED = false, bool SHALLOW = false, bool SLIM = false>
 __global__ __launch_bounds__(EXACT ? 256 : RT_WG_THREADS, EXACT ? 4 : (is_trace_job(JOB) ? RT_WAVES_TRACE : (JOB == JOB_RENDER_GI ? RT_WAVES_GI : (PACKED ? RT_WAVES_RENDER_PACKED : RT_WAVES_RENDER)))) void rt_persistent_kernel(SceneDev sc, ShadeParams p, PersistArgs A) {
   constexpr int LSTK = EXACT ? LDS_STACK : (is_trace_job(JOB) ? RT_LDS_STACK_TRACE : (JOB == JOB_RENDER_GI ? RT_LDS_STACK_GI : (PACKED ? RT_LDS_STACK_RENDER_PACKED : RT_LDS_STACK_RENDER)));
   constexpr int WG_WAVES = EXACT ? 4 : RT_WG_WAVES;
@@ -534,6 +535,20 @@
     uint32_t j = job;
     asm volatile("" : "+v"(j));
     return A.hits + j;
+  };
+  auto pix_slot = [&]() -> uint4* {
+    uint32_t j = job;
+    asm volatile("" : "+v"(j));
+    return (uint4*)A.hits + j;
+  };
+  auto store_pixel = [&](bool hit, float dist, float bx, float by, uint32_t blasIdx24, uint32_t triIdx) {
+    if constexpr (SLIM) {
+      *pix_slot() = make_uint4(__float_as_uint(dist), __float_as_uint(bx), __float_as_uint(by), pixrec_id(blasIdx24, triIdx, A.id_shift));
+    } else {
+      HitRec h;
+      h.dist = dist; h.bx = bx; h.by = by; h.bz = hit ? 1 - bx - by : 0.0f;
+      *hit_slot() = h;
+    }
   };
   auto pixel_ray = [&](uint32_t x, uint32_t y, float& ox, float& oy, float& oz, float& dx, float& dy, float& dz) {
     if constexpr (is_cam_job(JOB)) {
@@ -573,10 +588,7 @@
     if (JOB == JOB_RENDER_GI && (flags & F_SHADOW)) nrays--;
     if (slot < A.defer_cap) A.defer_list[slot] = job | ((flags & F_SHADOW) && JOB != JOB_RENDER_GI ? 0x80000000u : 0u);
     if (job_base(JOB) == JOB_RENDER_SHADOW && (flags & F_SHADOW)) {
-      HitRec h;
-      h.bx = __uint_as_float(CTX(3)); h.by = __uint_as_float(CTX(4)); h.bz = 1 - h.bx - h.by;
-      h.dist = __uint_as_float(CTX(5)); h.blasIdx = CTX(6); h.triIdx = CTX(7);
-      *hit_slot() = h;
+      store_pixel(true, __uint_as_float(CTX(5)), __uint_as_float(CTX(3)), __uint_as_float(CTX(4)), CTX(6), CTX(7));
     }
     if (counted) nrays--;
     cur = DESC_IDLE;
@@ -721,7 +733,7 @@
             if (EXACT) {
               const uint32_t wd = A.defer_list[job];
               job = wd & 0x7fffffffu;
-              if (wd >> 31) { flags = F_SHADOW | F_RESUMED; if (job_base(JOB) == JOB_RENDER_SHADOW) CTX(5) = __float_as_uint(hit_slot()->dist); }
+              if (wd >> 31) { flags = F_SHADOW | F_RESUMED; if (job_base(JOB) == JOB_RENDER_SHADOW) CTX(5) = SLIM ? pix_slot()->x : __float_as_uint(hit_slot()->dist); }
             }
             float ox, oy, oz, dx, dy, dz, tm;
             if (is_trace_job(JOB)) {
@@ -974,19 +986,17 @@
           start_ray(sox, soy, soz, sdx, sdy, sdz, sdist, true);
         } else {
           if (found) {
-            h.dist = hitd; h.bx = __uint_as_float(CTX(3)); h.by = __uint_as_float(CTX(4)); h.bz = 1 - h.bx - h.by;
+            h.dist = hitd; h.bx = __uint_as_float(CTX(3)); h.by = __uint_as_float(CTX(4));
             h.blasIdx = CTX(6); h.triIdx = CTX(7);
           }
-          *hit_slot() = h;
+          store_pixel(found, h.dist, h.bx, h.by, h.blasIdx, h.triIdx);
           cur = DESC_IDLE;
         }
       } else if (EXACT && (flags & F_RESUMED)) {
-        if (found) hit_slot()->blasIdx |= 0x80000000u;
+        if (found) { if constexpr (SLIM) ((uint32_t*)pix_slot())[3] |= PIXREC_OCC; else hit_slot()->blasIdx |= 0x80000000u; }
         cur = DESC_IDLE;
       } else {
-        h.bx = __uint_as_float(CTX(3)); h.by = __uint_as_float(CTX(4)); h.bz = 1 - h.bx - h.by;
-        h.dist = __uint_as_float(CTX(5)); h.blasIdx = CTX(6) | (found ? 0x80000000u : 0u); h.triIdx = CTX(7);
-        *hit_slot() = h;
+        store_pixel(true, __uint_as_float(CTX(5)), __uint_as_float(CTX(3)), __uint_as_float(CTX(4)), CTX(6) | (found ? 0x80000000u : 0u), CTX(7));
         cur = DESC_IDLE;
       }
     }
@@ -1066,7 +1076,7 @@
   }
 }
 
-template <bool STATS, bool CAM>
+template <bool STATS, bool CAM, bool SLIM>
 __device__ __forceinline__ void shade_pass(SceneDev sc, ShadeParams p, uint32_t W, uint32_t H, uint32_t y0, uint32_t y1, uint32_t row_step,
                                            uint32_t n_rows, const float* __restrict__ utab, const float* __restrict__ vtab,
                                            const HitRec* __restrict__ hb, uint32_t* __restrict__ dst,
@@ -1075,7 +1085,7 @@
                                            uint32_t lpt_blocks, const uint32_t* __restrict__ lpt_cost, uint32_t* __restrict__ lpt_order,
                                            uint32_t lpt_tiles, uint32_t lpt_per_shard,
                                            uint32_t batch, const ShadeParams* __restrict__ pbatch, uint64_t dst_frame_stride,
-                                           const uint32_t* __restrict__ lpt_base) {
+                                           const uint32_t* __restrict__ lpt_base, uint32_t id_shift) {
   __shared__ uint32_t s_hist[2048 + 8];
   if (blockIdx.x < lpt_blocks) { lpt_order_block(blockIdx.x, lpt_cost, lpt_order, lpt_tiles, lpt_per_shard, s_hist, lpt_base); return; }
   const uint32_t blk = blockIdx.x - lpt_blocks;
@@ -1089,7 +1099,12 @@
   if (batch > 1 && t < n) { p = pbatch[frame]; dst += (size_t)frame * dst_frame_stride; }
   if (t < n && y < y1) {
     const size_t idx = (size_t)x + (size_t)y * W;
-    HitRec h = hb[hit_index(x, vr, (W + 7u) >> 3)];
+    HitRec h;
+    if constexpr (SLIM) {
+      const uint4 q = ((const uint4*)hb)[hit_index(x, vr, (W + 7u) >> 3)];
+      h.dist = __uint_as_float(q.x); h.bx = __uint_as_float(q.y); h.by = __uint_as_float(q.z); h.bz = pixrec_bz(h.dist, h.bx, h.by);
+      h.blasIdx = pixrec_blas24(q.w, id_shift); h.triIdx = pixrec_tri(q.w, id_shift);
+    } else h = hb[hit_index(x, vr, (W + 7u) >> 3)];
     const uint32_t occ_bit = h.blasIdx & 0x80000000u;
     const bool occ = occ_bit != 0u;
     h.blasIdx &= 0x7fffffffu;
@@ -1114,7 +1129,7 @@
     }
   }
 }
-template <bool STATS>
+template <bool STATS, bool SLIM = false>
 __global__ __launch_bounds__(256) void rt_shade_kernel(SceneDev sc, ShadeParams p, uint32_t W, uint32_t H, uint32_t y0, uint32_t y1, uint32_t row_step,
                                                       uint32_t n_rows, const float* __restrict__ utab, const float* __restrict__ vtab,
                                                       const HitRec* __restrict__ hb, uint32_t* __restrict__ dst,
@@ -1123,11 +1138,11 @@
                                                       uint32_t lpt_blocks, const uint32_t* __restrict__ lpt_cost, uint32_t* __restrict__ lpt_order,
                                                       uint32_t lpt_tiles, uint32_t lpt_per_shard,
                                                       uint32_t batch = 1, const ShadeParams* __restrict__ pbatch = nullptr, uint64_t dst_frame_stride = 0,
-                                                      const uint32_t* __restrict__ lpt_base = nullptr) {
-  shade_pass<STATS, false>(sc, p, W, H, y0, y1, row_step, n_rows, utab, vtab, hb, dst, hits, colors, counters, ctl_reset, lpt_blocks, lpt_cost, lpt_order,
-                           lpt_tiles, lpt_per_shard, batch, pbatch, dst_frame_stride, lpt_base);
-}
-template <bool BATCH>
+                                                      const uint32_t* __restrict__ lpt_base = nullptr, uint32_t id_shift = 0) {
+  shade_pass<STATS, false, SLIM>(sc, p, W, H, y0, y1, row_step, n_rows, utab, vtab, hb, dst, hits, colors, counters, ctl_reset, lpt_blocks, lpt_cost, lpt_order,
+                                 lpt_tiles, lpt_per_shard, batch, pbatch, dst_frame_stride, lpt_base, id_shift);
+}
+template <bool BATCH, bool SLIM>
 __global__ __launch_bounds__(256) void rt_shade_camera_kernel(SceneDev sc, ShadeParams p, uint32_t W, uint32_t H, uint32_t y0, uint32_t y1, uint32_t row_step,
                                                              uint32_t n_rows, const float* __restrict__ cam,
                                                              const HitRec* __restrict__ hb, uint32_t* __restrict__ dst,
@@ -1135,9 +1150,9 @@
                                                              uint32_t lpt_blocks, const uint32_t* __restrict__ lpt_cost, uint32_t* __restrict__ lpt_order,
                                                              uint32_t lpt_tiles, uint32_t lpt_per_shard,
                                                              uint32_t batch, const ShadeParams* __restrict__ pbatch, uint64_t dst_frame_stride,
-                                                             const uint32_t* __restrict__ lpt_base) {
-  shade_pass<false, true>(sc, p, W, H, y0, y1, row_step, n_rows, cam, cam + CAM_TAB, hb, dst, hits, colors, nullptr, ctl_reset, lpt_blocks, lpt_cost, lpt_order,
-                          lpt_tiles, lpt_per_shard, BATCH ? batch : 1u, pbatch, dst_frame_stride, lpt_base);
+                                                             const uint32_t* __restrict__ lpt_base, uint32_t id_shift) {
+  shade_pass<false, true, SLIM>(sc, p, W, H, y0, y1, row_step, n_rows, cam, cam + CAM_TAB, hb, dst, hits, colors, nullptr, ctl_reset, lpt_blocks, lpt_cost, lpt_order,
+                                lpt_tiles, lpt_per_shard, BATCH ? batch : 1u, pbatch, dst_frame_stride, lpt_base, id_shift);
 }
 
 __global__ __launch_bounds__(256) void rt_shade_rays_kernel(SceneDev sc, ShadeParams p, uint64_t n, const float* __restrict__ rays,
@@ -2029,6 +2044,9 @@
 
 static bool mirror_frame(const vxrt_accel* a, const vxrt_shade_params_t& params) { return params.max_depth > 1 && a->max_reflectivity > 0.0f; }
 static bool gi_fused_frame(const RenderRequest& r) { return r.ao && r.ao->reserved == VXRT_AO_MODE_DIFFUSE_BOUNCE; }
+static bool slim_frame(const vxrt_accel* a, const RenderRequest& r) {
+  return a->pix_tri_bits >= 0 && r.counting == Counting::TIMED && !r.ao && !mirror_frame(a, r.params[0]);
+}
 
 static int check_request(const vxrt_accel* a, const RenderRequest& r) {
   const bool stats = r.counting != Counting::TIMED;
@@ -2151,7 +2169,7 @@
   if (!r.cams && !ensure_uv_tables(a, r.width, r.height, s)) return false;
   A.W = r.width; A.H = r.height; A.y0 = r.y0; A.y1 = r.y1; A.tiles_x = t.x; A.row_step = t.row_step; A.total = n_tiles * 64u;
   A.div_tiles_x = fast_div_make(t.x); A.div_frame_tiles = fast_div_make(t.per_frame); A.frame_tiles = t.per_frame;
-  A.hits = (HitRec*)c->hitbuf; A.counters = r.counters; A.wave_log = r.wave_log; A.end_log = a->end_log;
+  A.hits = (HitRec*)c->hitbuf; A.id_shift = a->pix_tri_bits >= 0 ? (uint32_t)a->pix_tri_bits : 0u; A.counters = r.counters; A.wave_log = r.wave_log; A.end_log = a->end_log;
   A.utab = a->uvtab; A.vtab = a->uvtab + r.width;
   if (r.cams) {
     if (!upload_cameras(c, r, s)) return false;
@@ -2207,20 +2225,25 @@
   PersistArgs A, X, X0;
 };
 
-template <int JOB, int STATS, bool PACKED>
+template <int JOB, int STATS, bool PACKED, bool SLIM = false>
 static void launch_traversal(const FrameLaunch& l) {
   static_assert(!(PACKED && (JOB == JOB_RENDER_GI || STATS != 0)), "only the timed render jobs have a packed form");
+  static_assert(!(SLIM && (JOB == JOB_RENDER_GI || STATS != 0)), "only the timed render jobs write pixel records");
   with_decode_and_depth<STATS == 0>(l.a, [&](auto ld, auto sh) {
-    const auto k_main = rt_persistent_kernel<JOB, STATS, decltype(ld)::value, false, PACKED, decltype(sh)::value>;
-    const auto k_exact = rt_persistent_kernel<JOB, STATS, decltype(ld)::value, true>;
+    const auto k_main = rt_persistent_kernel<JOB, STATS, decltype(ld)::value, false, PACKED, decltype(sh)::value, SLIM>;
+    const auto k_exact = rt_persistent_kernel<JOB, STATS, decltype(ld)::value, true, false, false, SLIM>;
     if (l.plan.side_launch) hipLaunchKernelGGL(k_exact, dim3(l.plan.side_wgs), dim3(256), 0, l.c->side, l.a->dev, l.p, l.X0);
     hipLaunchKernelGGL(k_main, dim3(main_grid(k_main, l.plan, l.A.total)), dim3(RT_WG_THREADS), 0, l.s, l.a->dev, l.p, l.A);
     hipLaunchKernelGGL(k_exact, dim3(EXACT_GRID), dim3(256), 0, l.s, l.a->dev, l.p, l.X);
   });
 }
-template <int STATS, bool PACKED, int CAM = 0>
+template <int STATS, bool PACKED, int CAM = 0, bool SLIM = false>
 static void launch_render(bool shadow, const FrameLaunch& l) {
-  if (shadow) launch_traversal<JOB_RENDER_SHADOW | CAM, STATS, PACKED>(l); else launch_traversal<JOB_RENDER | CAM, STATS, PACKED>(l);
+  if (shadow) launch_traversal<JOB_RENDER_SHADOW | CAM, STATS, PACKED, SLIM>(l); else launch_traversal<JOB_RENDER | CAM, STATS, PACKED, SLIM>(l);
+}
+template <bool PACKED, int CAM>
+static void launch_timed_render(bool slim, bool shadow, const FrameLaunch& l) {
+  if (slim) launch_render<0, PACKED, CAM, true>(shadow, l); else launch_render<0, PACKED, CAM, false>(shadow, l);
 }
 
 static bool traverse_frame(vxrt_accel* a, FrameCtx* c, const RenderRequest& r, const LaunchPlan& plan, const ShadeParams& p, const PersistArgs& A, hipStream_t s) {
@@ -2240,9 +2263,9 @@
   }
   else if (r.counting == Counting::TIMED_TRAVERSAL) launch_render<2, false>(r.shadow != 0, l);
   else if (r.counting == Counting::REFERENCE_ORDER) launch_render<1, false>(r.shadow != 0, l);
-  else if (r.cams)      launch_render<0, false, JOB_CAM>(r.shadow != 0, l);
-  else if (plan.packed) launch_render<0, true>(r.shadow != 0, l);
-  else                  launch_render<0, false>(r.shadow != 0, l);
+  else if (r.cams)      launch_timed_render<false, JOB_CAM>(slim_frame(a, r), r.shadow != 0, l);
+  else if (plan.packed) launch_timed_render<true, 0>(slim_frame(a, r), r.shadow != 0, l);
+  else                  launch_timed_render<false, 0>(slim_frame(a, r), r.shadow != 0, l);
   return !plan.side_launch || (hipEventRecord(c->ev_side, c->side) == hipSuccess && hipStreamWaitEvent(s, c->ev_side, 0) == hipSuccess);
 }
 
@@ -2253,16 +2276,20 @@
   const uint32_t lpt_blocks = lpt_sort ? QUEUE_SHARDS : 0u;
   const dim3 sgrid((uint32_t)((npx + 255) / 256) + lpt_blocks), block(256);
   const uint32_t* base_order = r.batch > 1 ? (const uint32_t*)a->batch_order[r.batch] : (const uint32_t*)nullptr;
+  const bool slim = slim_frame(a, r);
   if (r.cams) {
-    hipLaunchKernelGGL(r.batch > 1 ? rt_shade_camera_kernel<true> : rt_shade_camera_kernel<false>, sgrid, block, 0, s, a->dev, p, r.width, r.height, r.y0, r.y1, t.row_step,
+    const auto k = slim ? (r.batch > 1 ? rt_shade_camera_kernel<true, true> : rt_shade_camera_kernel<false, true>)
+                        : (r.batch > 1 ? rt_shade_camera_kernel<true, false> : rt_shade_camera_kernel<false, false>);
+    hipLaunchKernelGGL(k, sgrid, block, 0, s, a->dev, p, r.width, r.height, r.y0, r.y1, t.row_step,
                        n_rows, (const float*)A.utab, (const HitRec*)c->hitbuf, r.dst, (HitRec*)r.hits, r.colors, c->ctl, lpt_blocks, (const uint32_t*)L.cost,
-                       L.order, n_tiles, A.per_shard >> 6, r.batch, (const ShadeParams*)c->pbatch, r.dst_frame_stride, base_order);
+                       L.order, n_tiles, A.per_shard >> 6, r.batch, (const ShadeParams*)c->pbatch, r.dst_frame_stride, base_order, A.id_shift);
   } else {
     const bool stats = r.counting != Counting::TIMED;
-    hipLaunchKernelGGL(stats ? rt_shade_kernel<true> : rt_shade_kernel<false>, sgrid, block, 0, s, a->dev, p, r.width, r.height, r.y0, r.y1, t.row_step,
+    const auto k = stats ? rt_shade_kernel<true, false> : (slim ? rt_shade_kernel<false, true> : rt_shade_kernel<false, false>);
+    hipLaunchKernelGGL(k, sgrid, block, 0, s, a->dev, p, r.width, r.height, r.y0, r.y1, t.row_step,
                        n_rows, A.utab, A.vtab, (const HitRec*)c->hitbuf, r.dst, (HitRec*)r.hits, r.colors, r.counters, c->ctl, lpt_blocks, (const uint32_t*)L.cost,
                        L.order, n_tiles, A.per_shard >> 6, stats ? 1u : r.batch, stats ? (const ShadeParams*)nullptr : (const ShadeParams*)c->pbatch,
-                       stats ? (uint64_t)0 : r.dst_frame_stride, base_order);
+                       stats ? (uint64_t)0 : r.dst_frame_stride, base_order, A.id_shift);
   }
   return hipGetLastError() == hipSuccess;
 }
diff --git a/vortex-raytracing_amd/csrc/rt_types.h b/vortex-raytracing_amd/csrc/rt_types.h
--- a/vortex-raytracing_amd/csrc/rt_types.h
+++ b/vortex-raytracing_amd/csrc/rt_types.h
@@ -82,6 +82,27 @@
 #endif
 #define RT_TOP_MAX 1024
 static_assert(RT_TOP_NODES <= RT_TOP_MAX, "top-of-tree image");
+struct rt_pixrec_t { float dist, bx, by; uint32_t id; };
+static_assert(sizeof(rt_pixrec_t) == 16, "pixel record layout");
+#define PIXREC_OCC 0x80000000u
+#define PIXREC_ID_BITS 31u
+#ifdef __HIPCC__
+#define RT_HD __host__ __device__ inline
+#else
+#define RT_HD inline
+#endif
+RT_HD uint32_t pixrec_bits_for(uint32_t count) { uint32_t b = 0; while (b < 32u && ((uint64_t)1 << b) < (uint64_t)count) ++b; return b; }
+RT_HD int pixrec_tri_bits(uint32_t n_blas, uint32_t n_tris, uint32_t budget) {
+  const uint32_t tb = pixrec_bits_for(n_tris), bb = pixrec_bits_for(n_blas);
+  return (budget <= PIXREC_ID_BITS && tb + bb <= budget) ? (int)tb : -1;
+}
+RT_HD uint32_t pixrec_id(uint32_t blasIdx24, uint32_t triIdx, uint32_t tri_bits) {
+  return triIdx | ((blasIdx24 & ~PIXREC_OCC) << tri_bits) | (blasIdx24 & PIXREC_OCC);
+}
+RT_HD float pixrec_bz(float dist, float bx, float by) { return dist != RT_LARGE_FLOAT ? 1 - bx - by : 0.0f; }
+RT_HD uint32_t pixrec_tri(uint32_t id, uint32_t tri_bits) { return id & (uint32_t)(((uint64_t)1 << tri_bits) - 1u); }
+RT_HD uint32_t pixrec_blas24(uint32_t id, uint32_t tri_bits) { return ((id & ~PIXREC_OCC) >> tri_bits) | (id & PIXREC_OCC); }
+
 #ifdef __HIPCC__
 __device__ __forceinline__ bool is_node_desc(uint32_t d) { return d < 0x80000000u; }
 __device__ __forceinline__ bool is_leaf_desc(uint32_t d) { return (d >> 30) == DK_LEAF; }
diff --git a/vortex-raytracing_amd/rtapi.py b/vortex-raytracing_amd/rtapi.py
--- a/vortex-raytracing_amd/rtapi.py
+++ b/vortex-raytracing_amd/rtapi.py
@@ -240,6 +240,16 @@
     return int(v.value)
 
 
+def debug_pixel_record_bits(accel, id_bits):
+    L = _lib()
+    L.vxrt_debug_pixel_record_bits.restype = C.c_int
+    L.vxrt_debug_pixel_record_bits.argtypes = [C.c_void_p, C.c_uint32]
+    rc = L.vxrt_debug_pixel_record_bits(accel, id_bits)
+    if rc < -1:
+        raise RuntimeError("vxrt_debug_pixel_record_bits failed")
+    return rc
+
+
 def rc_accel_info(accel, which):
     L = _lib()
     L.vxrc_accel_info.restype = C.c_int
```

After: 11230 Mrays/s, median of 6. About the same (+0.7%).
